# juno181/Ex4DGS

Measured on AMD Instinct MI355X. Metric: fwd+bwd ms/frame @1M Gaussians 1352x1014; achieved HBM GB/s vs peak, lower is better.
Workload: dtype f32; 1 GPU; cfg3: 1.0M static+dynamic (K=35), 1352x1014; P=1000000, HW=1370928, sh_degree=3, step=GaussianRasterizer forward + backward on a resident frame, parallelism=frame-sharded x1

## Files before the change

### ex4dgs_amd/_C.py

```python
import ctypes as C

import torch

from . import _abi
from ._abi import ALLOC_FN, BinningLayout, Ex4dParams, Ex4dSplitSH, GeomLayout, ImgLayout, library_path, load

NUM_CHANNELS = 3
EXPORTS = _abi.exports("ex4d_rasterizer.h")


class PendingFrame:
    __slots__ = ("capacity", "assumed_no_flow", "_status", "_event", "_pool")

    def __init__(self, capacity, assumed_no_flow, status, event, pool):
        self.capacity, self.assumed_no_flow, self._status, self._event, self._pool = int(capacity), bool(assumed_no_flow), status, event, pool

    def done(self):
        return self._event is not None and self._event.query()

    def wait(self):
        if self._event is not None:
            self._event.synchronize()
        else:
            torch.cuda.synchronize()
# ... 40 lines not shown
        except Exception:
            pass


_status_pool = []
_status_parked = []


def _recycle_parked():
    if _status_parked:
        still = []
        for ev, st in _status_parked:
            if ev.query():
                _status_pool.append(st)
            else:
                still.append((ev, st))
        _status_parked[:] = still


def _pinned_status():
    _recycle_parked()
    if not _status_pool:
        if torch.cuda.is_current_stream_capturing():
            raise RuntimeError("no pinned status buffer left during graph capture: run one asynchronous forward before capturing")
        block = torch.zeros(16, 8, dtype=torch.int32).pin_memory()
        _status_pool.extend(block[i] for i in range(16))
    return _status_pool.pop()


class SplitSH(tuple):
    def __new__(cls, dc_static, rest_static, dc_dynamic, rest_dynamic):
        return super().__new__(cls, (dc_static, rest_static, dc_dynamic, rest_dynamic))

    @property
    def n_static(self):
        return self[0].shape[0]

    @property
    def n_dynamic(self):
        return self[2].shape[0]

    def numel(self):
        return sum(t.numel() for t in self)

    def size(self, dim):
        return (self.n_static + self.n_dynamic, 16, 3)[dim]


def _split_struct(split, device, what):
    keep, ptrs = [], []
    for t, shape1 in zip(split, (1, 15, 1, 15)):
        if t.dim() != 3 or t.shape[1] != shape1 or t.shape[2] != 3:
            raise RuntimeError(f"{what}: expected [n,{shape1},3] tensors (dc/rest, static then dynamic)")
        kt, pt = _dev_f32(t, what, device)
        keep.append(kt); ptrs.append(pt)
    if split[0].shape[0] != split[1].shape[0] or split[2].shape[0] != split[3].shape[0]:
        raise RuntimeError(f"{what}: dc and rest must have the same number of rows")
    st = Ex4dSplitSH((C.c_void_p * 2)(ptrs[0], ptrs[2]), (C.c_void_p * 2)(ptrs[1], ptrs[3]), int(split[0].shape[0]))
    return keep, st


def _dev_f32(t, name, device):
    if t is None or t.numel() == 0:
        return None, None
    if t.device != device:
        raise RuntimeError(f"{name} must be on {device}, got {t.device}")
    if t.dtype != torch.float32:
        raise RuntimeError(f"{name} must be float32, got {t.dtype}")
    t = t.contiguous()
    return t, t.data_ptr()


def _rows(t, name, rows, cols=None):
    if t is None or t.numel() == 0:
        return
    if t.size(0) != rows or (cols is not None and t.numel() != rows * cols):
        raise RuntimeError(f"{name} has shape {tuple(t.shape)}, expected {rows} rows" + (f" of {cols} values" if cols else ""))


def _numel(t, name, n):
    if t is not None and t.numel() not in (0, n):
        raise RuntimeError(f"{name} has {t.numel()} elements, expected {n}")


def _require_rocm(t, name):
    if not t.is_cuda:
        raise RuntimeError(f"{name} is on {t.device}: the ex4dgs_amd rasterizer only runs on a ROCm GPU (no CPU fallback)")


def _params(P, D, M, W, H, tanfovx, tanfovy, kernel_size, scale_modifier, min_depth, max_depth, prefiltered, debug, prepare_backward=False,
            instance_capacity=0, assume_no_flow=False):
    return Ex4dParams(P, D, M, W, H, tanfovx, tanfovy, kernel_size, scale_modifier, min_depth, max_depth, int(bool(prefiltered)), int(bool(debug)),
                      int(bool(prepare_backward)), int(instance_capacity), int(bool(assume_no_flow)), 0)


def _resizer(t):
    def fn(_user, nbytes):
        t.resize_(int(nbytes))
        return t.data_ptr()
    return ALLOC_FN(fn)


def rasterize_gaussians(background, means3D, dir3D, colors, opacity, scales, rotations, scale_modifier, cov3D_precomp,
                        viewmatrix, projmatrix, tan_fovx, tan_fovy, kernel_size, subpixel_offset, image_height, image_width,
                        sh, degree, campos, prefiltered, min_depth, max_depth, debug, prepare_backward=False,
                        instance_capacity=0, assume_no_flow=False):
    load()
    if means3D.ndimension() != 2 or means3D.size(1) != 3:
        raise RuntimeError("means3D must have dimensions (num_points, 3)")
    _require_rocm(means3D, "means3D")
    dev = means3D.device
    P, H, W = means3D.size(0), int(image_height), int(image_width)
    f32 = dict(dtype=torch.float32, device=dev)
    i32 = dict(dtype=torch.int32, device=dev)
    geomBuffer = torch.empty(0, dtype=torch.uint8, device=dev)
    binningBuffer = torch.empty(0, dtype=torch.uint8, device=dev)
    imgBuffer = torch.empty(0, dtype=torch.uint8, device=dev)
    if P == 0:
        return (0, torch.zeros(NUM_CHANNELS, H, W, **f32), torch.zeros(P, **i32), geomBuffer, binningBuffer, imgBuffer,
                torch.zeros(1, H, W, **f32), torch.zeros(1, H, W, **f32), torch.zeros(3, H, W, **f32), torch.full((1, H, W), -1, **i32))
    out_color = torch.empty(NUM_CHANNELS, H, W, **f32)
    radii = torch.empty(P, **i32)
    out_depth = torch.empty(1, H, W, **f32)
    out_acc = torch.empty(1, H, W, **f32)
    out_flow = torch.empty(3, H, W, **f32)
    out_idx = torch.empty(1, H, W, **i32)

    split = sh if isinstance(sh, SplitSH) else None
    if split is not None:
        if split.n_static + split.n_dynamic != P:
            raise RuntimeError("SplitSH rows do not add up to the number of Gaussians")
        sh = torch.empty(0, **f32)
    M = 16 if split is not None else (sh.size(1) if sh.numel() != 0 else 0)
    for name, t, cols in (("dir3D", dir3D, 3), ("colors", colors, NUM_CHANNELS), ("opacity", opacity, 1), ("scales", scales, 3),
                          ("rotations", rotations, 4), ("cov3D_precomp", cov3D_precomp, 6), ("sh", sh, 3 * M)):
        _rows(t, name, P, cols)
    _numel(subpixel_offset, "subpixel_offset", 2 * H * W)
    _numel(background, "background", NUM_CHANNELS)
    for name, t in (("viewmatrix", viewmatrix), ("projmatrix", projmatrix)):
        _numel(t, name, 16)
    _numel(campos, "campos", 3)
    keep = []
    ptr = {}
    for name, t in (("background", background), ("means3D", means3D), ("dir3D", dir3D), ("sh", sh), ("colors", colors),
                    ("opacity", opacity), ("scales", scales), ("rotations", rotations), ("cov3D_precomp", cov3D_precomp),
                    ("viewmatrix", viewmatrix), ("projmatrix", projmatrix), ("campos", campos), ("subpixel_offset", subpixel_offset)):
        kt, ptr[name] = _dev_f32(t, name, dev)
        keep.append(kt)
    prm = _params(P, int(degree), M, W, H, tan_fovx, tan_fovy, kernel_size, scale_modifier, min_depth, max_depth, prefiltered, debug, prepare_backward,
                  instance_capacity, assume_no_flow)
    cbs = [_resizer(geomBuffer), _resizer(binningBuffer), _resizer(imgBuffer)]
    num_rendered = C.c_int32(0)
    count_ref = C.byref(num_rendered)
    status = None
    if instance_capacity > 0:
        status = torch.zeros(8, dtype=torch.int32, device=dev) if torch.cuda.is_current_stream_capturing() else _pinned_status()
        count_ref = C.cast(status.data_ptr(), C.POINTER(C.c_int32))
    entry, sh_args = "ex4d_forward", (ptr["sh"], ptr["colors"])
    if split is not None:
        if colors.numel() != 0:
            raise RuntimeError("Please provide excatly one of either SHs or precomputed colors!")
        kp, st = _split_struct(split, dev, "sh")
        keep.append(kp)
        entry, sh_args = "ex4d_forward_split_sh", (C.byref(st),)
    with _abi.stream(dev) as stream:
        _abi.call(entry, C.byref(prm), ptr["background"], ptr["means3D"], ptr["dir3D"], *sh_args, ptr["opacity"],
                  ptr["scales"], ptr["rotations"], ptr["cov3D_precomp"], ptr["viewmatrix"], ptr["projmatrix"], ptr["campos"],
                  ptr["subpixel_offset"], cbs[0], None, cbs[1], None, cbs[2], None,
                  out_color.data_ptr(), radii.data_ptr(), out_depth.data_ptr(), out_acc.data_ptr(), out_flow.data_ptr(), out_idx.data_ptr(),
                  stream, count_ref)
        ev = None
        if status is not None and not torch.cuda.is_current_stream_capturing():
            ev = torch.cuda.Event()
            ev.record(torch.cuda.current_stream())
    if status is not None:
        return (PendingFrame(instance_capacity, assume_no_flow, status, ev, _status_pool), out_color, radii, geomBuffer, binningBuffer, imgBuffer,
                out_depth, out_acc, out_flow, out_idx)
    return (int(num_rendered.value), out_color, radii, geomBuffer, binningBuffer, imgBuffer, out_depth, out_acc, out_flow, out_idx)


def rasterize_gaussians_backward(background, means3D, radii, colors, scales, rotations, acc_depth, acc, min_depth, max_depth,
                                 scale_modifier, cov3D_precomp, viewmatrix, projmatrix, tan_fovx, tan_fovy, kernel_size,
                                 subpixel_offset, dL_dout_color, dL_dout_depth, dL_grad_out_flow, dL_grad_out_acc, sh, degree,
                                 campos, geomBuffer, R, binningBuffer, imageBuffer, debug, need_colors=True, need_cov3D=True, prepared=False):
    lib = load()
    _require_rocm(means3D, "means3D")
    dev = means3D.device
    P = means3D.size(0)
    if isinstance(R, PendingFrame):
        R = R.capacity
    H, W = acc_depth.size(1), acc_depth.size(2)
    f32 = dict(dtype=torch.float32, device=dev)
    split = sh if isinstance(sh, SplitSH) else None
    if split is not None:
        sh = torch.empty(0, **f32)
    M = 16 if split is not None else (sh.size(1) if sh.numel() != 0 else 0)
    shapes = [(P, 3), (P, NUM_CHANNELS), (P, 1), (P, 3), (P, 6), (P, M, 3) if split is None else (0,), (P, 3), (P, 4), (P, 3)]
    for name, t, cols in (("radii", radii, 1), ("colors", colors, NUM_CHANNELS), ("scales", scales, 3), ("rotations", rotations, 4),
                          ("cov3D_precomp", cov3D_precomp, 6), ("sh", sh, 3 * M)):
        _rows(t, name, P, cols)
    if split is not None and split.n_static + split.n_dynamic != P:
        raise RuntimeError("SplitSH rows do not add up to the number of Gaussians")
    _numel(subpixel_offset, "subpixel_offset", 2 * H * W)
    for name, t, n in (("acc", acc, H * W), ("dL_dout_color", dL_dout_color, NUM_CHANNELS * H * W), ("dL_dout_depth", dL_dout_depth, H * W),
                       ("dL_grad_out_flow", dL_grad_out_flow, 3 * H * W), ("dL_grad_out_acc", dL_grad_out_acc, H * W),
                       ("viewmatrix", viewmatrix, 16), ("projmatrix", projmatrix, 16), ("campos", campos, 3)):
        _numel(t, name, n)
    if P == 0:
        outs0 = [torch.zeros(*s, **f32) for s in shapes]
        if split is not None:
            outs0[5] = SplitSH(*[torch.zeros_like(t) for t in split])
        return tuple(outs0)
    outs = [torch.empty(*s, **f32) for s in shapes]
    if not need_colors:
        outs[1] = torch.empty(0, **f32)
    if not need_cov3D:
        outs[4] = torch.empty(0, **f32)
    if split is not None:
        outs[5] = SplitSH(*[torch.empty_like(t, memory_format=torch.contiguous_format) for t in split])
    keep = []
    ptr = {}
    for name, t in (("background", background), ("means3D", means3D), ("sh", sh), ("colors", colors), ("scales", scales),
                    ("rotations", rotations), ("cov3D_precomp", cov3D_precomp), ("viewmatrix", viewmatrix), ("projmatrix", projmatrix),
                    ("campos", campos), ("subpixel_offset", subpixel_offset), ("acc_depth", acc_depth), ("acc", acc),
                    ("dL_dout_color", dL_dout_color), ("dL_dout_depth", dL_dout_depth), ("dL_grad_out_flow", dL_grad_out_flow),
                    ("dL_grad_out_acc", dL_grad_out_acc)):
        kt, ptr[name] = _dev_f32(t, name, dev)
        keep.append(kt)
    radii_c = radii.contiguous()
    scratch = torch.empty(lib.ex4d_backward_scratch_bytes(P), dtype=torch.uint8, device=dev)
    prm = _params(P, int(degree), M, W, H, tan_fovx, tan_fovy, kernel_size, scale_modifier, min_depth, max_depth, False, debug, prepared)
    if split is None:
        entry, sh_args, g_sh = "ex4d_backward", (ptr["sh"], ptr["colors"]), (outs[5].data_ptr() if M > 0 else None)
    else:
        kp, st = _split_struct(split, dev, "sh")
        kg, gst = _split_struct(outs[5], dev, "dL_dsh")
        keep += [kp, kg]
        entry, sh_args, g_sh = "ex4d_backward_split_sh", (C.byref(st),), C.byref(gst)
    with _abi.stream(dev) as stream:
        _abi.call(entry, C.byref(prm), int(R), ptr["background"], ptr["means3D"], radii_c.data_ptr(), *sh_args,
                  ptr["scales"], ptr["rotations"], ptr["cov3D_precomp"], ptr["viewmatrix"], ptr["projmatrix"], ptr["campos"],
                  ptr["subpixel_offset"], ptr["acc_depth"], ptr["acc"],
                  geomBuffer.data_ptr(), binningBuffer.data_ptr(), imageBuffer.data_ptr(),
                  ptr["dL_dout_color"], ptr["dL_dout_depth"], ptr["dL_grad_out_flow"], ptr["dL_grad_out_acc"],
                  outs[0].data_ptr(), _abi.ptr(outs[1]), outs[2].data_ptr(), outs[3].data_ptr(), _abi.ptr(outs[4]),
                  g_sh, outs[6].data_ptr(), outs[7].data_ptr(), outs[8].data_ptr(), scratch.data_ptr(), stream)
    rasterize_gaussians_backward.last_scratch = scratch
    return tuple(outs)


def mark_visible(means3D, viewmatrix, projmatrix, min_depth, max_depth=3.4028234663852886e38):
    load()
    _require_rocm(means3D, "means3D")
    dev = means3D.device
    P = means3D.size(0)
    present = torch.zeros(P, dtype=torch.bool, device=dev)
    if P == 0:
        return present
    if means3D.ndimension() != 2 or means3D.size(1) != 3:
        raise RuntimeError("means3D must have dimensions (num_points, 3)")
    (m, _), (v, _), (p, _) = _dev_f32(means3D, "means3D", dev), _dev_f32(viewmatrix, "viewmatrix", dev), _dev_f32(projmatrix, "projmatrix", dev)
    if v is None or p is None or v.numel() != 16 or p.numel() != 16:
        raise RuntimeError("viewmatrix and projmatrix must be 4x4 float32 tensors")
    with _abi.stream(dev) as stream:
        _abi.call("ex4d_mark_visible", P, m.data_ptr(), v.data_ptr(), p.data_ptr(), min_depth, max_depth, present.data_ptr(), stream)
    return present


def geom_views(geomBuffer, P):
    lay = GeomLayout()
    load().ex4d_geom_layout(P, C.byref(lay))
    g = geomBuffer
    v = lambda off, n, dt: g[off: off + n * torch.empty(0, dtype=dt).element_size()].view(dt)
    rec = v(lay.records, 16 * P, torch.float32).view(P, 16)
    return dict(records=rec, depths=rec[:, 8], means2D=rec[:, 0:2], conic_opacity=rec[:, [2, 3, 4, 15]], rgb=rec[:, 9:12], dir3D=rec[:, 12:15],
                cov3D=v(lay.cov3D, 6 * P, torch.float32).view(P, 6), clamped=v(lay.clamped, P, torch.uint8),
                tiles_touched=v(lay.tiles_touched, P, torch.int32), depth_order=v(lay.depth_order, P, torch.int32),
                rects=v(lay.rects, 2 * P, torch.int32).view(P, 2))


def binning_views(binningBuffer, R, W, H):
    if isinstance(R, PendingFrame):
        R = R.capacity
    lay = BinningLayout()
    load().ex4d_binning_layout(R, W, H, C.byref(lay))
    b = binningBuffer
    T = ((W + 15) // 16) * ((H + 15) // 16)
    return dict(point_list=b[lay.point_list: lay.point_list + 4 * R].view(torch.int32),
                tile_ids=b[lay.tile_ids: lay.tile_ids + 4 * R].view(torch.int32),
                qlist=b[lay.qlist: lay.qlist + 16 * max(R, 1)].view(torch.int32),
                qcount=b[lay.qcount: lay.qcount + 16 * T].view(torch.int32).view(T, 4))


def img_views(imgBuffer, W, H):
    lay = ImgLayout()
    load().ex4d_img_layout(W, H, C.byref(lay))
    T = ((W + 15) // 16) * ((H + 15) // 16)
    i = imgBuffer
    return dict(final_T=i[lay.final_T: lay.final_T + 4 * W * H].view(torch.float32).view(H, W),
                n_contrib=i[lay.n_contrib: lay.n_contrib + 4 * W * H].view(torch.int32).view(H, W),
                ranges=i[lay.ranges: lay.ranges + 8 * T].view(torch.int32).view(T, 2))


def set_option(name, value):
    _abi.call("ex4d_set_option", name.encode(), int(value))


def get_option(name):
    return int(load().ex4d_get_option(name.encode()))


SAMPLE_SORT_STATS = ("empty", "skipped", "packed", "pairs", "memory", "memory_gaussians", "largest", "distinct_splitters")


def sample_sort_stats(reset=True):
    buf = (C.c_ulonglong * 8)()
    _abi.call("ex4d_debug_sample_sort", buf, int(bool(reset)))
    return dict(zip(SAMPLE_SORT_STATS, (int(x) for x in buf)))


def bwd_stats(reset=True, extended=False):
    n = 16 if extended else 8
    buf = (C.c_ulonglong * n)()
    _abi.call("ex4d_debug_bwd_stats16" if extended else "ex4d_debug_bwd_stats", buf, int(bool(reset)))
    return [int(x) for x in buf]


def profile_enable(on=True):
    load().ex4d_profile_enable(int(bool(on)))


def profile_read(which):
    ms = (C.c_float * 16)()
    names = (C.c_char_p * 16)()
    n = load().ex4d_profile_read(int(which), ms, names, 16)
    return [(names[i].decode(), float(ms[i])) for i in range(n)]
```

### ex4dgs_amd/_abi.py

```python
import contextlib
import ctypes as C
import os

import torch

_CSRC = os.path.join(os.path.dirname(os.path.abspath(__file__)), "csrc")
_LIB_PATH = os.environ.get("EX4D_HIP_LIB") or os.path.join(_CSRC, "libex4d_hip.so")
_lib = None

RADAM_MAX_WINDOWS = 8
TRAINER_PARAMS = 15


def _all(ctype, *names):
    return [(n, ctype) for n in names]


i32, i64, f32, f64, vp, cint, size, text = C.c_int32, C.c_int64, C.c_float, C.c_double, C.c_void_p, C.c_int, C.c_size_t, C.c_char_p
P = C.POINTER


class Ex4dParams(C.Structure):
    _fields_ = [*_all(i32, "P", "D", "M", "W", "H"),
                *_all(f32, "tanfovx", "tanfovy", "kernel_size", "scale_modifier", "min_depth", "max_depth"),
                *_all(i32, "prefiltered", "debug", "prepare_backward", "instance_capacity", "assume_no_flow", "reserved")]


ALLOC_FN = C.CFUNCTYPE(vp, vp, size)


class Ex4dSplitSH(C.Structure):
    _fields_ = [("dc", vp * 2), ("rest", vp * 2), ("n_static", i32)]


Ex4dSplitSHGrad = Ex4dSplitSH


class Ex4dGeomLayout(C.Structure):
    _fields_ = _all(size, "records", "cov3D", "clamped", "tiles_touched", "depth_order", "sorted_offsets", "rects", "total")


class Ex4dBinningLayout(C.Structure):
    _fields_ = _all(size, "point_list", "tile_ids", "qlist", "qcount", "total")


class Ex4dImgLayout(C.Structure):
    _fields_ = _all(size, "final_T", "n_contrib", "ranges", "total")


GeomLayout, BinningLayout, ImgLayout = Ex4dGeomLayout, Ex4dBinningLayout, Ex4dImgLayout


class Ex4dAttrParams(C.Structure):
    _fields_ = [*_all(i32, "Ns", "Nd", "K", "k"), *_all(f32, "t", "duration", "delta", "h00", "h10", "h01", "h11", "tau", "var_min")]


class Ex4dRadamTensor(C.Structure):
    _fields_ = [*_all(vp, "param", "grad", "exp_avg", "exp_avg_sq"), ("numel", i64), ("lr", f64), ("step", i64),
                ("nan_to_num", i32), ("reserved", i32)]


class Ex4dRadamSlicedTensor(C.Structure):
    _fields_ = [*_all(vp, "param", "exp_avg", "exp_avg_sq"), ("rows", i64), ("K", i32), ("C", i32), ("lr", f64), ("step", i64),
                ("n_windows", i32), ("first", i32 * RADAM_MAX_WINDOWS), ("count", i32 * RADAM_MAX_WINDOWS),
                ("grad", vp * RADAM_MAX_WINDOWS), ("first_dev", vp)]


class Ex4dRadamSlicedRegTensor(C.Structure):
    _fields_ = [("t", Ex4dRadamSlicedTensor), ("reg_kind", i32), ("reserved", i32), ("reg_weight", f64), ("reg_rows", i64)]


class Ex4dDensifyPlanGroup(C.Structure):
    _fields_ = [("n", i64), *_all(vp, "stats", "scaling", "opacity", "xyz"), ("xyz_width", i32), ("use_screen", i32),
                *_all(f32, "grad_thr", "dense_scale", "big_scale", "screen_size", "min_opacity", "l1_thres", "max_ssim"),
                ("reserved", i32), *_all(vp, "map", "counts", "scratch")]


class Ex4dDensifyTensor(C.Structure):
    _fields_ = [("src", vp), ("dst", vp), ("rows", i64), ("dst_rows", i64), *_all(i32, "width", "planes", "rule", "group"),
                ("aux0", vp), ("aux1", vp), ("value", f32), ("reserved", i32)]


class Ex4dDensifyApplyGroup(C.Structure):
    _fields_ = [("map", vp), ("child_stride", i64), ("n_split", i64), *_all(vp, "split_z", "split_c1", "split_c0", "clone_c1", "clone_c0"),
                *_all(f32, "min_len", "center_lo", "center_hi", "split_div")]


class Ex4dGrowthClassify(C.Structure):
    _fields_ = [("n", i64), *_all(vp, "score", "result", "disp", "stats"), ("motion_abs", f32), ("min_abs", f32),
                *_all(vp, "map", "counts", "selected", "counts_out", "scratch")]


class Ex4dGrowthTensor(C.Structure):
    _fields_ = [*_all(vp, "old", "dst", "src0", "src1"), ("old_rows", i64), ("width", i32), ("rule", i32)]


class Ex4dGrowthAppend(C.Structure):
    _fields_ = [("selected", vp), ("n_new", i64), ("n_static", i64), ("stats", vp), ("K", i32),
                *_all(f32, "interval", "max_dur", "b_scale", "time_shift", "time_pad", "center_lo", "center_hi")]


class Ex4dTrainerConfig(C.Structure):
    _fields_ = [*_all(i32, "Ns", "Nd", "K", "W", "H", "sh_degree"), *_all(f32, "tanfovx", "tanfovy", "kernel_size", "min_depth", "max_depth"),
                *_all(f64, "duration", "interval", "time_shift", "var_pad"), ("lambda_dssim", f32), ("window", f32 * 11),
                ("lr", f64 * TRAINER_PARAMS), *_all(f64, "beta1", "beta2", "eps"), ("optimizer", i32)]


class Ex4dTrainerStepOptions(C.Structure):
    _fields_ = [*_all(i32, "l1_accum", "skip_optimizer", "stats_flags", "nan_census"), *_all(vp, "stats_s", "stats_d")]


class Ex4dTrainerReport(C.Structure):
    _fields_ = [("loss", f32), *_all(i32, "nan_static", "nan_dynamic", "reserved")]


def _status(name, *argtypes):
    return name, cint, argtypes, True


def _value(name, restype, *argtypes):
    return name, restype, argtypes, False


_fwd_tail = (ALLOC_FN, vp) * 3 + (vp,) * 6 + (vp, P(i32))
PROTOTYPES = {
    "ex4d_rasterizer.h": ("ex4d_last_error", (
        _value("ex4d_last_error", text),
        _value("ex4d_abi_version", cint),
        _value("ex4d_target_arch", text),
        _status("ex4d_forward", P(Ex4dParams), *[vp] * 13, *_fwd_tail),
        _status("ex4d_backward", P(Ex4dParams), i32, *[vp] * 32),
        _value("ex4d_backward_scratch_bytes", size, i32),
        _status("ex4d_forward_split_sh", P(Ex4dParams), *[vp] * 3, P(Ex4dSplitSH), *[vp] * 8, *_fwd_tail),
        _status("ex4d_backward_split_sh", P(Ex4dParams), i32, *[vp] * 3, P(Ex4dSplitSH), *[vp] * 21, P(Ex4dSplitSHGrad), *[vp] * 5),
        _status("ex4d_mark_visible", i32, vp, vp, vp, f32, f32, vp, vp),
        _value("ex4d_geom_bytes", size, i32),
        _value("ex4d_binning_bytes", size, i32, i32, i32),
        _value("ex4d_img_bytes", size, i32, i32),
        _value("ex4d_geom_layout", None, i32, P(Ex4dGeomLayout)),
        _value("ex4d_binning_layout", None, i32, i32, i32, P(Ex4dBinningLayout)),
        _value("ex4d_img_layout", None, i32, i32, P(Ex4dImgLayout)),
        _status("ex4d_set_option", text, cint),
        _value("ex4d_get_option", cint, text),
        _status("ex4d_debug_bwd_stats", P(C.c_ulonglong), cint),
        _status("ex4d_debug_bwd_stats16", P(C.c_ulonglong), cint),
        _status("ex4d_debug_rows_prof", P(C.c_ulonglong), cint),
        _status("ex4d_debug_sample_sort", P(C.c_ulonglong), cint),
        _value("ex4d_profile_enable", None, cint),
        _value("ex4d_profile_read", cint, cint, P(f32), P(text), cint))),
    "ex4d_attributes.h": ("ex4d_attributes_last_error", (
        _value("ex4d_attributes_last_error", text),
        _status("ex4d_attributes_forward", P(Ex4dAttrParams), *[vp] * 21),
        _status("ex4d_attributes_backward", P(Ex4dAttrParams), *[vp] * 28),
        _status("ex4d_attributes_backward_sliced", P(Ex4dAttrParams), *[vp] * 27, P(i32), vp),
        _status("ex4d_attr_time_scalars", i32, f64, f64, f64, f64, i32, i32, i32, f64, P(Ex4dAttrParams)),
        _status("ex4d_attributes_forward_ex", P(Ex4dAttrParams), i32, *[vp] * 21),
        _status("ex4d_attributes_backward_ex", P(Ex4dAttrParams), i32, *[vp] * 29),
        _status("ex4d_attributes_backward_sliced_ex", P(Ex4dAttrParams), i32, *[vp] * 28, P(i32), vp))),
    "ex4d_loss.h": ("ex4d_loss_last_error", (
        _value("ex4d_loss_last_error", text),
        _value("ex4d_l1_ssim_scratch_floats", size, i32, i32),
        _status("ex4d_l1_ssim_forward", i32, i32, i32, vp, vp, f32, *[vp] * 7),
        _status("ex4d_l1_ssim_backward", i32, i32, i32, vp, vp, f32, *[vp] * 5),
        _status("ex4d_l1_ssim_forward_u8", i32, i32, vp, vp, i32, vp, f32, *[vp] * 7),
        _status("ex4d_l1_ssim_backward_u8", i32, i32, vp, vp, i32, vp, f32, *[vp] * 5),
        _value("ex4d_frame_metrics_scratch_floats", size, i32, i32),
        _status("ex4d_frame_metrics", i32, i32, vp, vp, vp, i32, *[vp] * 4),
        _status("ex4d_frame_metrics_u8", i32, i32, vp, vp, i32, vp, vp, i32, *[vp] * 4),
        _value("ex4d_resize_u8_table_words", size, i32, i32, i32),
        _status("ex4d_resize_u8_table", i32, i32, i32, vp),
        _value("ex4d_resize_u8_scratch_bytes", size, i32, i32, i32, i32),
        _status("ex4d_resize_u8", i32, i32, i32, i32, i32, *[vp] * 6),
        _value("ex4d_frame_skssim_scratch_floats", size, i32, i32),
        _status("ex4d_frame_skssim", i32, i32, vp, vp, i32, *[vp] * 3),
        _status("ex4d_frame_skssim_u8", i32, i32, vp, vp, i32, vp, i32, *[vp] * 3))),
    "ex4d_optim.h": ("ex4d_optim_last_error", (
        _value("ex4d_optim_last_error", text),
        _status("ex4d_radam_step", P(Ex4dRadamTensor), i32, f64, f64, f64, vp),
        _status("ex4d_radam_step_sliced", P(Ex4dRadamSlicedTensor), i32, f64, f64, f64, vp),
        _status("ex4d_radam_step_sliced_reg", P(Ex4dRadamSlicedRegTensor), i32, f64, f64, f64, vp),
        _value("ex4d_radam_sliced_reg_rows", i32, i32, i32))),
    "ex4d_knn.h": ("ex4d_knn_last_error", (
        _value("ex4d_knn_last_error", text),
        _value("ex4d_dist2_scratch_bytes", size, i32),
        _status("ex4d_dist2", i32, vp, vp, vp, vp))),
    "ex4d_densify.h": ("ex4d_densify_last_error", (
        _status("ex4d_densify_stats", vp, i64, vp, i64, vp, vp, vp, f32, i32, vp),
        _status("ex4d_densify_stats_merge", vp, vp, i32, i64, vp, vp),
        _status("ex4d_nan_any", vp, i64, vp, i64, vp, vp),
        _value("ex4d_densify_scratch_bytes", size, i64),
        _status("ex4d_densify_plan", i32, P(Ex4dDensifyPlanGroup), vp),
        _status("ex4d_densify_apply", P(Ex4dDensifyTensor), i32, P(Ex4dDensifyApplyGroup), vp),
        _value("ex4d_densify_last_error", text),
        _status("ex4d_growth_scores", vp, vp, vp, vp, i64, vp, vp),
        _value("ex4d_growth_select_scratch_bytes", size),
        _status("ex4d_growth_select", vp, i64, f32, vp, vp, vp),
        _status("ex4d_growth_classify", P(Ex4dGrowthClassify), vp),
        _status("ex4d_growth_append", P(Ex4dGrowthTensor), i32, P(Ex4dGrowthAppend), vp),
        _status("ex4d_growth_extrapolate", vp, vp, i64, i32, i32, i32, i32, vp),
        _status("ex4d_growth_expand_opacity", vp, vp, vp, vp, i64, f32, f32, f32, vp),
        _status("ex4d_growth_adjust_opacity", vp, vp, vp, vp, i64, f32, f32, vp))),
    "ex4d_regularizers.h": ("ex4d_reg_last_error", (
        _value("ex4d_reg_last_error", text),
        _value("ex4d_reg_scratch_bytes", size),
        _status("ex4d_reg_forward", vp, i64, vp, vp, i64, i32, f64, f64, f64, vp, vp, vp),
        _status("ex4d_reg_backward", vp, vp, i64, vp, vp, vp, vp, i64, i32, f64, f64, f64, vp, i32, vp),
        _status("ex4d_reg_backward_range", i32, vp, i64, i32, i64, i64, vp, f64, i32, vp))),
    "ex4d_trainer.h": ("ex4d_trainer_last_error", (
        _value("ex4d_trainer_last_error", text),
        _value("ex4d_trainer_create", vp, P(Ex4dTrainerConfig), P(vp)),
        _value("ex4d_trainer_destroy", None, vp),
        _value("ex4d_trainer_time_scalars", None, P(Ex4dTrainerConfig), f64, P(Ex4dAttrParams)),
        _status("ex4d_trainer_step", vp, f64, *[vp] * 6, P(i32)),
        _status("ex4d_trainer_step_ex", vp, f64, *[vp] * 6, P(i32), P(Ex4dTrainerStepOptions)),
        _status("ex4d_trainer_step_u8", vp, f64, *[vp] * 5, i32, vp, vp, P(i32), P(Ex4dTrainerStepOptions)),
        _status("ex4d_trainer_report", vp, P(Ex4dTrainerReport)),
        _status("ex4d_trainer_set_lr", vp, P(f64)),
        _status("ex4d_trainer_set_sh_degree", vp, i32),
        _status("ex4d_trainer_set_async", vp, i32),
        _value("ex4d_trainer_replays", i64, vp),
        _status("ex4d_trainer_set_interp", vp, i32),
        _status("ex4d_trainer_set_regularizers", vp, f64, f64, f64),
        _value("ex4d_trainer_output", vp, vp, i32),
        _value("ex4d_trainer_grad", vp, vp, i32, P(i32)),
        _status("ex4d_trainer_read", vp, i32, vp, size, vp),
        _status("ex4d_trainer_write", vp, i32, vp, size, vp),
        _status("ex4d_trainer_get_step", vp, P(i64)),
        _status("ex4d_trainer_set_step", vp, i64),
        _value("ex4d_trainer_bytes", size, vp))),
}
_LAST_ERROR = {name: err for err, protos in PROTOTYPES.values() for name, _, _, is_status in protos if is_status}


def exports(header):
    return tuple(name for name, _, _, _ in PROTOTYPES[header][1])


def library_path():
    return _LIB_PATH


def load():
    global _lib
    if _lib is not None:
        return _lib
    if not os.path.exists(_LIB_PATH):
        raise RuntimeError(f"{_LIB_PATH} not found: build it with `python -m ex4dgs_amd.build` "
                           "(there is no CPU / PyTorch fallback for the rasterizer)")
    lib = C.CDLL(_LIB_PATH)
    for _, protos in PROTOTYPES.values():
        for name, restype, argtypes, _ in protos:
            fn = getattr(lib, name)
            fn.restype, fn.argtypes = restype, list(argtypes)
    _lib = lib
    return lib


def call(name, *args):
    err = _LAST_ERROR[name]
    lib = load()
    rc = getattr(lib, name)(*args)
    if rc != 0:
        raise RuntimeError(getattr(lib, err)().decode() or f"{name} failed with status {rc}")


def ptr(t):
    return None if t is None or t.numel() == 0 else t.data_ptr()


@contextlib.contextmanager
def stream(device):
    with torch.cuda.device(device):
        yield C.c_void_p(torch.cuda.current_stream().cuda_stream)
```

### ex4dgs_amd/csrc/ex4d_api.hip

```cpp
#include "ex4d_internal.h"
#include <atomic>
#include <cstdarg>
#include <cstdio>
#include <cstdlib>
#include <cstring>
#include <mutex>

namespace {

std::atomic<bool> g_prof_on{false};
std::atomic<int> g_bwd_variant{4};
std::atomic<int> g_tile_ids{0};
std::atomic<int> g_tile_rows{1};
std::atomic<int> g_depth_msd{3};
struct DepthSortWatch {
    std::mutex mu;
    uint32_t *word = nullptr;
    bool tried = false;
    std::atomic<int> hold{0}, backoff{64}, trips{0};
    uint32_t *get()
    {
        std::lock_guard<std::mutex> lock(mu);
        if (!tried) {
            tried = true;
            if (hipHostMalloc((void **)&word, 64, hipHostMallocPortable) != hipSuccess) { (void)hipGetLastError(); word = nullptr; }
            else memset(word, 0, 64);
        }
        return word;
    }
    void reset()
    {
        std::lock_guard<std::mutex> lock(mu);
        hold.store(0); backoff.store(64); trips.store(0);
        if (word) __atomic_store_n(word, 0u, __ATOMIC_RELAXED);
    }
} g_depth_watch;
bool depth_sort_auto_msd(hipStream_t stream, bool async, uint32_t **watch)
{
    *watch = nullptr;
    if (async) {
        hipStreamCaptureStatus st = hipStreamCaptureStatusNone;
        if (hipStreamIsCapturing(stream, &st) != hipSuccess) { (void)hipGetLastError(); return false; }
        if (st != hipStreamCaptureStatusNone) return false;
    }
    uint32_t *w = g_depth_watch.get();
    if (!w) return false;
    if (__atomic_load_n(w, __ATOMIC_RELAXED) != 0u && __atomic_exchange_n(w, 0u, __ATOMIC_RELAXED) != 0u) {
        const int b = g_depth_watch.backoff.load();
        g_depth_watch.hold.store(b);
        g_depth_watch.backoff.store(b < (1 << 20) ? 2 * b : b);
        g_depth_watch.trips.fetch_add(1);
    }
    for (int h = g_depth_watch.hold.load(); h > 0; )
        if (g_depth_watch.hold.compare_exchange_weak(h, h - 1)) return false;
    *watch = w;
    return true;
}
std::atomic<int> g_depth_msd_bits{0};
std::atomic<int> g_readback_side{1};
std::atomic<int> g_depth_local_cap{0};
std::atomic<int> g_depth_local_threads{0};
std::atomic<int> g_depth_sample{0};
std::atomic<int> g_depth_sample_frames{0};
std::atomic<int> g_depth_sample_stats{0};
std::atomic<int> g_geom_debug{0};
thread_local char g_err[512] = "";

int fail(int code, const char *fmt, ...)
{
    va_list ap;
    va_start(ap, fmt);
    vsnprintf(g_err, sizeof(g_err), fmt, ap);
    va_end(ap);
    return code;
}

#define HIP_TRY(expr)                                                                              \
    do {                                                                                           \
        hipError_t e_ = (expr);                                                                    \
        if (e_ != hipSuccess) return fail(EX4D_ERR_HIP, "%s failed: %s", #expr, hipGetErrorString(e_)); \
    } while (0)

#define STAGE(expr, prm, stream)                                                                   \
    do {                                                                                           \
        HIP_TRY(expr);                                                                             \
        if ((prm)->debug) HIP_TRY(hipStreamSynchronize(stream));                                   \
    } while (0)
#define MARK(which, name) g_prof.mark(which, name, stream)

struct StageProfiler {
    static const int kMax = 16;
    hipEvent_t ev[2][kMax + 1];
    const char *names[2][kMax];
    int n[2] = { 0, 0 };
    bool created = false;
    int device = -1;
    std::mutex mu;
    void begin(int which, hipStream_t s)
    {
        if (!g_prof_on.load(std::memory_order_relaxed)) return;
        std::lock_guard<std::mutex> lock(mu);
        int dev = -1;
        (void)hipGetDevice(&dev);
        if (created && dev != device) {
            for (int w = 0; w < 2; w++) for (int i = 0; i <= kMax; i++) (void)hipEventDestroy(ev[w][i]);
            created = false; n[0] = n[1] = 0;
        }
        if (!created) { for (int w = 0; w < 2; w++) for (int i = 0; i <= kMax; i++) (void)hipEventCreate(&ev[w][i]); created = true; device = dev; }
        n[which] = 0;
        (void)hipEventRecord(ev[which][0], s);
    }
    void mark(int which, const char *name, hipStream_t s)
    {
        if (!g_prof_on.load(std::memory_order_relaxed)) return;
        std::lock_guard<std::mutex> lock(mu);
        if (!created || n[which] >= kMax) return;
        names[which][n[which]] = name;
        n[which]++;
        (void)hipEventRecord(ev[which][n[which]], s);
    }
};
StageProfiler g_prof;

struct Readback {
    uint32_t *host = nullptr;
    size_t words = 0;
    hipEvent_t ev;
    hipEvent_t ev_pre;
    hipStream_t side = nullptr;
    bool have_ev = false;
    int device = -1;
    bool init(size_t need_words)
    {
        int dev = -1;
        if (hipGetDevice(&dev) != hipSuccess) return false;
        if (have_ev && dev != device) { (void)hipEventDestroy(ev); (void)hipEventDestroy(ev_pre); (void)hipStreamDestroy(side); side = nullptr; have_ev = false; }
        if (!have_ev) {
            if (hipEventCreateWithFlags(&ev, hipEventDisableTiming) != hipSuccess) return false;
            if (hipEventCreateWithFlags(&ev_pre, hipEventDisableTiming) != hipSuccess) { (void)hipEventDestroy(ev); return false; }
            if (hipStreamCreateWithFlags(&side, hipStreamNonBlocking) != hipSuccess) { (void)hipEventDestroy(ev); (void)hipEventDestroy(ev_pre); side = nullptr; return false; }
            have_ev = true; device = dev;
        }
        if (need_words > words) {
            if (host) (void)hipHostFree(host);
            host = nullptr; words = 0;
            if (hipHostMalloc((void **)&host, need_words * sizeof(uint32_t), hipHostMallocDefault) != hipSuccess) return false;
            words = need_words;
        }
        return true;
    }
};
thread_local Readback g_readback;

struct Carver {
    char *base; size_t off;
    explicit Carver(void *b) : base((char *)b), off(0) {}
    template <typename T> T *take(size_t count)
    {
        T *p = base ? (T *)(base + off) : nullptr;
        off = ex4d_align_up(off + count * sizeof(T));
        return p;
    }
};

GeomState carve_geom(void *buf, int P, Ex4dGeomLayout *lay, size_t *total)
{
    Carver c(buf);
    GeomState g;
    Ex4dGeomLayout l;
    l.records = c.off;        g.records = c.take<float4>(4 * (size_t)P);
    l.cov3D = c.off;          g.cov3D = c.take<float>(6 * (size_t)P);
    l.clamped = c.off;        g.clamped = c.take<uint8_t>(P);
    l.tiles_touched = c.off;  g.tiles_touched = c.take<uint32_t>(P);
    l.rects = c.off;          g.rects = c.take<uint2>(P);
    g.sorted_rects = c.take<uint2>(P);
    g.rects4 = c.take<uint32_t>(P);
    l.depth_order = c.off;    g.depth_order = c.take<uint32_t>(P);
    l.sorted_offsets = c.off; g.sorted_offsets = c.take<uint32_t>(P);
    g.sort_keys_a = c.take<uint32_t>(P);
    g.sort_keys_b = c.take<uint32_t>(P);
    g.sort_vals_b = c.take<uint32_t>(P);
    g.sort_vals_a = c.take<uint32_t>(P);
    g.rects4_b = c.take<uint32_t>(P);
    g.bucket_starts = c.take<uint32_t>((size_t)1 << EX4D_DLS_MSD_BITS);
    g.key_ranges = c.take<uint2>(((size_t)P + 63) / 64);
    g.bucket_sums = c.take<uint32_t>((size_t)1 << EX4D_DLS_MSD_BITS);
    g.scan_block_sums = c.take<uint32_t>((P + SCAN_CHUNK - 1) / SCAN_CHUNK + 1);
    g.sort_hist = c.take<uint32_t>(ex4d_radix_hist_words((uint32_t)P));
    g.total = c.take<uint32_t>(EX4D_FLAG_WORDS);
    g.block_totals = c.take<uint32_t>(2 * (((size_t)P + 63) / 64));
    g.row_hist = c.take<uint32_t>(ex4d_tile_sort_rows_geom_words((uint32_t)P));
    g.sh_dsums = c.take<float>(9 * (size_t)P);
    l.total = c.off;
    if (lay) *lay = l;
    if (total) *total = c.off;
    return g;
}

int tile_bits(int T)
{
    int b = 1;
    while ((1 << b) < T) b++;
    return b;
}

BinState carve_binning(void *buf, uint32_t R, int W, int H, Ex4dBinningLayout *lay, size_t *total)
{
    const int T = ((W + EX4D_TILE - 1) / EX4D_TILE) * ((H + EX4D_TILE - 1) / EX4D_TILE);
    Carver c(buf);
    BinState b;
    Ex4dBinningLayout l;
    const size_t n = R ? R : 1;
    l.point_list = c.off; b.point_list = c.take<uint32_t>(n);
    l.tile_ids = c.off;   b.tile_ids = c.take<uint32_t>(n);
    const int tb = tile_bits(T);
    const int cgx = (W + EX4D_TILE - 1) / EX4D_TILE, cgy = (H + EX4D_TILE - 1) / EX4D_TILE;
    const size_t hw = ex4d_radix_hist_words(R), hw2 = ex4d_tile_sort_hist_words(R, tb);
    const size_t hw3 = (cgx <= 255 && cgy <= 255) ? ex4d_tile_sort_rows_hist_words(R) : 0;
    const size_t hwm = hw > hw2 ? hw : hw2;
    b.sort_hist = c.take<uint32_t>(hwm > hw3 ? hwm : hw3);
    l.qlist = c.off;  b.qlist = c.take<uint32_t>(4 * n);
    b.vals_tmp = b.qlist;
    b.keys_tmp = b.qlist ? b.vals_tmp + ex4d_align_up(n * sizeof(uint32_t)) / sizeof(uint32_t) : nullptr;
    l.qcount = c.off; b.qcount = c.take<uint32_t>(4 * (size_t)T);
    l.total = c.off;
    if (lay) *lay = l;
    if (total) *total = c.off;
    return b;
}

ImgState carve_img(void *buf, int W, int H, Ex4dImgLayout *lay, size_t *total)
{
    Carver c(buf);
    ImgState s;
    Ex4dImgLayout l;
    const size_t HW = (size_t)W * H;
    const int T = ((W + EX4D_TILE - 1) / EX4D_TILE) * ((H + EX4D_TILE - 1) / EX4D_TILE);
    l.final_T = c.off;   s.final_T = c.take<float>(HW);
    l.n_contrib = c.off; s.n_contrib = c.take<uint32_t>(HW);
    l.ranges = c.off;    s.ranges = c.take<uint2>(T);
    l.total = c.off;
    if (lay) *lay = l;
    if (total) *total = c.off;
    return s;
}

}

extern "C" {

const char *ex4d_last_error(void) { return g_err; }
int ex4d_abi_version(void) { return 5; }
const char *ex4d_target_arch(void) { return "gfx950"; }

size_t ex4d_geom_bytes(int32_t P) { size_t t; carve_geom(nullptr, P, nullptr, &t); return t; }
size_t ex4d_binning_bytes(int32_t R, int32_t W, int32_t H) { size_t t; carve_binning(nullptr, (uint32_t)R, W, H, nullptr, &t); return t; }
size_t ex4d_img_bytes(int32_t W, int32_t H) { size_t t; carve_img(nullptr, W, H, nullptr, &t); return t; }
void ex4d_geom_layout(int32_t P, Ex4dGeomLayout *out) { carve_geom(nullptr, P, out, nullptr); }
void ex4d_binning_layout(int32_t R, int32_t W, int32_t H, Ex4dBinningLayout *out) { carve_binning(nullptr, (uint32_t)R, W, H, out, nullptr); }
void ex4d_img_layout(int32_t W, int32_t H, Ex4dImgLayout *out) { carve_img(nullptr, W, H, out, nullptr); }
size_t ex4d_backward_scratch_bytes(int32_t P) { return ex4d_align_up((size_t)P * 16 * sizeof(float)); }

static int forward_impl(
    const Ex4dParams *prm, ShSplit split,
    const float *background, const float *means3D, const float *dir3D, const float *shs, const float *colors_precomp,
    const float *opacities, const float *scales, const float *rotations, const float *cov3D_precomp,
    const float *viewmatrix, const float *projmatrix, const float *campos, const float *subpixel_offset,
    ex4d_alloc_fn geom_alloc, void *geom_user, ex4d_alloc_fn binning_alloc, void *binning_user,
    ex4d_alloc_fn img_alloc, void *img_user,
    float *out_color, int32_t *radii, float *out_depth, float *out_acc, float *out_flow, int32_t *out_idx,
    void *stream_, int32_t *num_rendered)
{
    g_err[0] = 0;
    hipStream_t stream = (hipStream_t)stream_;
    if (!prm || !num_rendered) return fail(EX4D_ERR_ARG, "null params");
    const int P = prm->P, W = prm->W, H = prm->H;
    if (P <= 0 || W <= 0 || H <= 0) return fail(EX4D_ERR_ARG, "P, W, H must be positive (P == 0 is handled by the caller)");
    if (!means3D || !opacities || !background || !viewmatrix || !projmatrix || !campos)
        return fail(EX4D_ERR_ARG, "means3D, opacities, background, viewmatrix, projmatrix, campos are required");
    const bool is_split = split.rest[0] != nullptr || split.rest[1] != nullptr;
    if (((shs != nullptr || is_split) ? 1 : 0) + (colors_precomp != nullptr ? 1 : 0) != 1 || (shs != nullptr && is_split))
        return fail(EX4D_ERR_ARG, "Please provide excatly one of either SHs or precomputed colors!");
    if (is_split && prm->M != 16) return fail(EX4D_ERR_ARG, "split SH needs M == 16 (dc [n,1,3] + rest [n,15,3])");
    if (((scales == nullptr || rotations == nullptr) && cov3D_precomp == nullptr) ||
        ((scales != nullptr || rotations != nullptr) && cov3D_precomp != nullptr))
        return fail(EX4D_ERR_ARG, "Please provide exactly one of either scale/rotation pair or precomputed 3D covariance!");
    if (shs && prm->M < (prm->D + 1) * (prm->D + 1)) return fail(EX4D_ERR_ARG, "sh has fewer coefficients than the active degree needs");
    if (!out_color || !radii || !out_depth || !out_acc || !out_flow || !out_idx) return fail(EX4D_ERR_ARG, "null output");
    const int gx = (W + EX4D_TILE - 1) / EX4D_TILE, gy = (H + EX4D_TILE - 1) / EX4D_TILE;
    const int T = gx * gy;
    const bool async = prm->instance_capacity > 0;
    if (prm->instance_capacity < 0) return fail(EX4D_ERR_ARG, "instance_capacity must be >= 0");
    if (async && prm->debug) return fail(EX4D_ERR_ARG, "debug (synchronise after every stage) and instance_capacity > 0 (asynchronous forward) exclude each other");

    void *geom_buf = geom_alloc(geom_user, ex4d_geom_bytes(P));
    if (!geom_buf) return fail(EX4D_ERR_ALLOC, "geometry buffer allocation failed");
    GeomState g = carve_geom(geom_buf, P, nullptr, nullptr);
    void *img_buf = img_alloc(img_user, ex4d_img_bytes(W, H));
    if (!img_buf) return fail(EX4D_ERR_ALLOC, "image buffer allocation failed");
    ImgState im = carve_img(img_buf, W, H, nullptr, nullptr);

    uint32_t key_base = 0, key_invisible = 0xFFFFFFFFu;
    int key_bits = 32;
    if (prm->min_depth >= 0.0f && prm->max_depth > prm->min_depth && prm->max_depth < 3.0e38f) {
        uint32_t lo, hi;
        memcpy(&lo, &prm->min_depth, 4); memcpy(&hi, &prm->max_depth, 4);
        key_base = lo;
        key_invisible = hi - lo + 1u;
        key_bits = 1;
        while (key_bits < 32 && (key_invisible >> key_bits) != 0u) key_bits++;
    }
    const bool packed_rects = gx <= 255 && gy <= 255;
    int msd_mode = g_depth_msd.load(std::memory_order_relaxed);
    uint32_t *msd_watch = nullptr;
    const bool sample_depth = g_depth_sample.load(std::memory_order_relaxed) != 0 && packed_rects && ex4d_depth_sort_msd_applies((uint32_t)P, key_bits);
    if (!(packed_rects && ex4d_depth_sort_msd_applies((uint32_t)P, key_bits))) msd_mode = 0;
    else if (sample_depth) msd_mode = 1;
    else if (msd_mode == 3) msd_mode = depth_sort_auto_msd(stream, async, &msd_watch) ? 2 : 0;
    const bool msd_depth = msd_mode != 0;
    int msd_bits = ex4d_depth_sort_msd_bits((uint32_t)P, key_bits);
    {
        const int forced = g_depth_msd_bits.load(std::memory_order_relaxed);
        if (forced == EX4D_DLS_MSD_BITS || (forced == EX4D_DLS_MSD_BITS - 1 && ex4d_depth_sort_msd_bits(1u, key_bits) == forced)) msd_bits = forced;
    }
    const bool start_in_b = (ex4d_radix_passes((uint32_t)P, key_bits) & 1) != 0;
    uint32_t *keys0 = start_in_b ? g.sort_keys_b : g.sort_keys_a, *vals0 = start_in_b ? g.sort_vals_b : g.depth_order;
    uint32_t *keys1 = start_in_b ? g.sort_keys_a : g.sort_keys_b, *vals1 = start_in_b ? g.depth_order : g.sort_vals_b;
    if (msd_depth) { keys0 = g.sort_keys_a; vals0 = g.sort_vals_a; }

    HIP_TRY(ex4d_prepare_rank_lds(stream));
    g_prof.begin(0, stream);
    if (async) HIP_TRY(ex4d_launch_zero(g.total, 8 * sizeof(uint32_t), stream));
    GeomState gw = g;
    if (!g_geom_debug.load(std::memory_order_relaxed)) {
        gw.cov3D = nullptr; gw.tiles_touched = nullptr;
        if (packed_rects) gw.rects = nullptr;
    }
    STAGE(ex4d_launch_preprocess_fwd(*prm, means3D, dir3D, scales, rotations, opacities, shs, cov3D_precomp, colors_precomp,
                                     viewmatrix, projmatrix, campos, radii, gw, g.total + 1, split,
                                     keys0, (uint32_t *)nullptr, key_base, key_invisible, packed_rects ? g.rects4 : nullptr, stream,
                                     (msd_depth && !sample_depth) ? reinterpret_cast<uint32_t *>(g.key_ranges) : nullptr, async), prm, stream);
    MARK(0, "preprocess_fwd");
    const size_t nblk = (size_t)(P + 63) / 64;
    const size_t rb_words = (size_t)(g.block_totals - g.total) + 2 * nblk;
    if (!async) {
        if (!g_readback.init(rb_words)) return fail(EX4D_ERR_HIP, "pinned read-back buffer allocation failed");
        if (g_readback_side.load(std::memory_order_relaxed)) {
            HIP_TRY(hipEventRecord(g_readback.ev_pre, stream));
            HIP_TRY(hipStreamWaitEvent(g_readback.side, g_readback.ev_pre, 0));
            HIP_TRY(hipMemcpyAsync(g_readback.host, g.total, rb_words * sizeof(uint32_t), hipMemcpyDeviceToHost, g_readback.side));
            HIP_TRY(hipEventRecord(g_readback.ev, g_readback.side));
        } else {
            HIP_TRY(hipMemcpyAsync(g_readback.host, g.total, rb_words * sizeof(uint32_t), hipMemcpyDeviceToHost, stream));
            HIP_TRY(hipEventRecord(g_readback.ev, stream));
        }
    }
    const bool rows_sort = g_tile_rows.load(std::memory_order_relaxed) != 0 && ex4d_tile_sort_rows_applies(P, gx, gy);
    const bool fused_scan = msd_mode == 2 && !rows_sort;
    const bool lsd_gather = !msd_depth && rows_sort && packed_rects;
    if (msd_depth) {
        if (sample_depth) {
            g_depth_sample_frames.fetch_add(1);
            STAGE(ex4d_depth_sort_sample(g.sort_keys_a, g.sort_vals_a, g.rects4, g.sort_keys_b, g.depth_order, g.rects4_b, (uint32_t)P, key_invisible, key_bits,
                                         g.sort_hist, g.bucket_starts, g.bucket_sums, (uint32_t)g_depth_local_cap.load(std::memory_order_relaxed), stream,
                                         T, rows_sort ? im.ranges : nullptr, g_depth_local_threads.load(std::memory_order_relaxed),
                                         g_depth_sample_stats.load(std::memory_order_relaxed) != 0), prm, stream);
        } else {
            STAGE(ex4d_depth_sort_msd(g.sort_keys_a, g.sort_vals_a, g.rects4, g.sort_keys_b, g.depth_order, g.rects4_b, (uint32_t)P, key_invisible,
                                      g.total, g.key_ranges, g.sort_hist, g.bucket_starts, (uint32_t)g_depth_local_cap.load(std::memory_order_relaxed), stream,
                                      fused_scan ? g.sorted_offsets : nullptr, fused_scan ? g.bucket_sums : nullptr, T, (fused_scan || rows_sort) ? im.ranges : nullptr,
                                      g_depth_local_threads.load(std::memory_order_relaxed), msd_watch, msd_bits), prm, stream);
        }
        MARK(0, "depth_sort");
        if (!fused_scan && !rows_sort) {
            STAGE(ex4d_launch_scan_tiles(P, nullptr, g.rects4_b, nullptr, nullptr, g.sorted_offsets, g.scan_block_sums, T, im.ranges, async ? g.total : nullptr, stream), prm, stream);
            MARK(0, "scan_tiles");
        }
    } else {
        bool in_first = true;
        STAGE(ex4d_radix_sort_pairs(keys0, vals0, keys1, vals1, (uint32_t)P, key_bits, g.sort_hist, &in_first, stream, nullptr, true,
                                    lsd_gather ? g.rects4 : nullptr, lsd_gather ? g.rects4_b : nullptr, lsd_gather ? im.ranges : nullptr, T), prm, stream);
        if (in_first == start_in_b) return fail(EX4D_ERR_HIP, "internal: depth sort ended in the wrong buffer");
        MARK(0, "depth_sort");
        if (!lsd_gather) {
            STAGE(ex4d_launch_scan_tiles(P, g.rects, packed_rects ? g.rects4 : nullptr, g.depth_order, g.sorted_rects, g.sorted_offsets, g.scan_block_sums, T, im.ranges, async ? g.total : nullptr, stream), prm, stream);
            MARK(0, "scan_tiles");
        }
    }
    const uint2 *dup_rects = (msd_depth || lsd_gather) ? nullptr : g.sorted_rects;
    const uint32_t *dup_rects4 = (msd_depth || lsd_gather) ? g.rects4_b : nullptr;
    uint32_t R = 0;
    uint32_t segment_sum = 0;
    const uint32_t *n_dev = nullptr;
    bool has_flow;
    if (async) {
        static_assert(sizeof(Ex4dFrameStatus) == 8 * sizeof(uint32_t), "Ex4dFrameStatus mirrors the first eight frame-flag words");
        const bool count_later = fused_scan || (rows_sort && msd_depth) || lsd_gather;
        if (!count_later) HIP_TRY(hipMemcpyAsync(num_rendered, g.total, sizeof(Ex4dFrameStatus), hipMemcpyDefault, stream));
        R = (uint32_t)prm->instance_capacity;
        segment_sum = 0;
        n_dev = g.total;
        has_flow = prm->assume_no_flow == 0;
    } else {
        {
            static const bool spin = []{ const char *e = getenv("EX4D_READBACK_SPIN"); return e ? atoi(e) != 0 : true; }();
            if (spin) {
                hipError_t q = hipErrorNotReady;
                for (int i = 0; i < 20000 && (q = hipEventQuery(g_readback.ev)) == hipErrorNotReady; i++) { }
                if (q == hipErrorNotReady) q = hipEventSynchronize(g_readback.ev);
                HIP_TRY(q);
            } else HIP_TRY(hipEventSynchronize(g_readback.ev));
        }
        uint32_t instance_sum = 0;
        uint32_t chunk_flags = 0;
        for (size_t i = 0; i < nblk; i++) {
            const uint32_t seg = g_readback.host[(size_t)(g.block_totals - g.total) + 2 * i + 1];
            instance_sum += g_readback.host[(size_t)(g.block_totals - g.total) + 2 * i];
            segment_sum += seg & 0x3FFFFFFFu;
            chunk_flags |= seg;
        }
        has_flow = (chunk_flags & EX4D_CHUNK_FLOW) != 0u;
        if (prm->prefiltered && (chunk_flags & EX4D_CHUNK_FILTERED))
            return fail(EX4D_ERR_PREFILTERED, "Point is filtered although prefiltered is set. This shouldn't happen!");
        R = instance_sum;
        if (R > 0x7FFFFFFFu) return fail(EX4D_ERR_ARG, "more than 2^31-1 tile instances");
        *num_rendered = (int32_t)R;
    }

    void *bin_buf = binning_alloc(binning_user, ex4d_binning_bytes((int32_t)R, W, H));
    if (!bin_buf) return fail(EX4D_ERR_ALLOC, "binning buffer allocation failed");
    BinState b = carve_binning(bin_buf, R, W, H, nullptr, nullptr);

    const int passes = ex4d_radix_passes(R, tile_bits(T));
    uint32_t *k0 = (passes % 2 == 0) ? b.tile_ids : b.keys_tmp;
    uint32_t *v0 = (passes % 2 == 0) ? b.point_list : b.vals_tmp;
    uint32_t *k1 = (passes % 2 == 0) ? b.keys_tmp : b.tile_ids;
    uint32_t *v1 = (passes % 2 == 0) ? b.vals_tmp : b.point_list;
    if (rows_sort) {
        if (R > 0) {
            STAGE(ex4d_tile_sort_rows(P, gx, gy, g.depth_order, dup_rects4, dup_rects, b.keys_tmp, b.point_list,
                                      g_tile_ids.load(std::memory_order_relaxed) ? b.tile_ids : nullptr, R, segment_sum, g.row_hist, b.sort_hist, im.ranges,
                                      (async && (msd_depth || lsd_gather)) ? g.total : nullptr, stream), prm, stream);
        }
        if (async && (msd_depth || lsd_gather)) HIP_TRY(hipMemcpyAsync(num_rendered, g.total, sizeof(Ex4dFrameStatus), hipMemcpyDefault, stream));
        MARK(0, "tile_sort");
    } else if (R > 0 && ex4d_tile_sort_msd_applies(P, tile_bits(T))) {
        STAGE(ex4d_launch_duplicate(P, W, H, g.depth_order, g.sorted_offsets, g.scan_block_sums, dup_rects, dup_rects4, b.tile_ids, b.vals_tmp, R, stream,
                                    fused_scan ? g.sort_keys_b : nullptr, g.total + EX4D_FLAG_DPARAMS, g.bucket_sums, g.total, msd_bits), prm, stream);
        if (async && fused_scan) HIP_TRY(hipMemcpyAsync(num_rendered, g.total, sizeof(Ex4dFrameStatus), hipMemcpyDefault, stream));
        MARK(0, "duplicate");
        STAGE(ex4d_tile_sort_msd(b.tile_ids, b.vals_tmp, b.keys_tmp, b.point_list, g_tile_ids.load(std::memory_order_relaxed) ? b.tile_ids : nullptr,
                                 R, tile_bits(T), b.sort_hist, im.ranges, stream, n_dev), prm, stream);
        MARK(0, "tile_sort");
        MARK(0, "tile_ranges");
    } else {
        if (R > 0) {
            STAGE(ex4d_launch_duplicate(P, W, H, g.depth_order, g.sorted_offsets, g.scan_block_sums, dup_rects, dup_rects4, k0, v0, R, stream,
                                        fused_scan ? g.sort_keys_b : nullptr, g.total + EX4D_FLAG_DPARAMS, g.bucket_sums, g.total, msd_bits), prm, stream);
            if (async && fused_scan) HIP_TRY(hipMemcpyAsync(num_rendered, g.total, sizeof(Ex4dFrameStatus), hipMemcpyDefault, stream));
            MARK(0, "duplicate");
            bool res_a = true;
            STAGE(ex4d_radix_sort_pairs(k0, v0, k1, v1, R, tile_bits(T), b.sort_hist, &res_a, stream, n_dev), prm, stream);
        }
        MARK(0, "tile_sort");
        STAGE(ex4d_launch_tile_ranges(R, T, b.tile_ids, im.ranges, stream, n_dev), prm, stream);
        MARK(0, "tile_ranges");
    }
    STAGE(ex4d_launch_composite_fwd(*prm, im.ranges, b.point_list, subpixel_offset, g.records, background, im.final_T, im.n_contrib,
                                    out_color, out_depth, out_acc, out_flow, out_idx, b.qlist, b.qcount, has_flow, stream), prm, stream);
    MARK(0, "composite_fwd");
    return EX4D_OK;
}

static int backward_impl(
    const Ex4dParams *prm, ShSplit split, ShSplitGrad gsplit, int32_t num_rendered,
    const float *background, const float *means3D, const int32_t *radii,
    const float *shs, const float *colors_precomp, const float *scales, const float *rotations,
    const float *cov3D_precomp, const float *viewmatrix, const float *projmatrix, const float *campos,
    const float *subpixel_offset, const float *out_depth, const float *out_acc,
    const void *geom_buffer, const void *binning_buffer, const void *img_buffer,
    const float *dL_dout_color, const float *dL_dout_depth, const float *dL_dout_flow, const float *dL_dout_acc,
    float *dL_dmeans2D, float *dL_dcolors, float *dL_dopacity, float *dL_dmeans3D, float *dL_dcov3D, float *dL_dsh,
    float *dL_dscales, float *dL_drotations, float *dL_ddir, void *bwd_scratch, void *stream_)
{
    g_err[0] = 0;
    hipStream_t stream = (hipStream_t)stream_;
    if (!prm) return fail(EX4D_ERR_ARG, "null params");
    const int P = prm->P, W = prm->W, H = prm->H;
    if (P <= 0 || W <= 0 || H <= 0) return fail(EX4D_ERR_ARG, "P, W, H must be positive (P == 0 is handled by the caller)");
    if (!geom_buffer || !binning_buffer || !img_buffer || !bwd_scratch) return fail(EX4D_ERR_ARG, "null state buffer");
    if ((size_t)P * 64 > 0xFFFFFFFFull) return fail(EX4D_ERR_ARG, "more than 2^26 Gaussians: the accumulator rows are addressed with 32-bit byte offsets");
    if (!dL_dmeans2D || !dL_dopacity || !dL_dmeans3D || !dL_dscales || !dL_drotations || !dL_ddir || (prm->M > 0 && !dL_dsh && !(gsplit.rest[0] || gsplit.rest[1])))
        return fail(EX4D_ERR_ARG, "null gradient output");
    GeomState g = carve_geom((void *)geom_buffer, P, nullptr, nullptr);
    BinState b = carve_binning((void *)binning_buffer, (uint32_t)num_rendered, W, H, nullptr, nullptr);
    ImgState im = carve_img((void *)img_buffer, W, H, nullptr, nullptr);
    float *acc16 = (float *)bwd_scratch;

    const int variant = g_bwd_variant.load(std::memory_order_relaxed);
    g_prof.begin(1, stream);
    HIP_TRY(ex4d_launch_zero(acc16, (size_t)P * 16 * sizeof(float), stream));
    MARK(1, "zero_accumulators");
    if (num_rendered > 0)
        STAGE(ex4d_launch_composite_bwd(*prm, im.ranges, b.point_list, subpixel_offset, background, g.records,
                                        out_depth, out_acc, im.final_T, im.n_contrib,
                                        dL_dout_color, dL_dout_depth, dL_dout_flow, dL_dout_acc, acc16, b.qlist, b.qcount, variant, stream), prm, stream);
    MARK(1, "composite_bwd");
    const float *cov3D_ptr = cov3D_precomp;
    STAGE(ex4d_launch_preprocess_bwd(*prm, means3D, radii, shs, scales, rotations, cov3D_ptr, viewmatrix, projmatrix, campos, g, acc16,
                                     dL_dmeans2D, dL_dcolors, dL_dopacity, dL_dmeans3D, dL_dcov3D, dL_dsh, dL_dscales, dL_drotations, dL_ddir,
                                     split, gsplit, stream), prm, stream);
    MARK(1, "preprocess_bwd");
    return EX4D_OK;
}

static const ShSplit kNoSplit = { { nullptr, nullptr }, { nullptr, nullptr }, 0 };
static const ShSplitGrad kNoSplitGrad = { { nullptr, nullptr }, { nullptr, nullptr }, 0 };

int ex4d_forward(
    const Ex4dParams *prm,
    const float *background, const float *means3D, const float *dir3D, const float *shs, const float *colors_precomp,
    const float *opacities, const float *scales, const float *rotations, const float *cov3D_precomp,
    const float *viewmatrix, const float *projmatrix, const float *campos, const float *subpixel_offset,
    ex4d_alloc_fn geom_alloc, void *geom_user, ex4d_alloc_fn binning_alloc, void *binning_user,
    ex4d_alloc_fn img_alloc, void *img_user,
    float *out_color, int32_t *radii, float *out_depth, float *out_acc, float *out_flow, int32_t *out_idx,
    void *stream_, int32_t *num_rendered)
{
    return forward_impl(prm, kNoSplit, background, means3D, dir3D, shs, colors_precomp, opacities, scales, rotations, cov3D_precomp,
                        viewmatrix, projmatrix, campos, subpixel_offset, geom_alloc, geom_user, binning_alloc, binning_user,
                        img_alloc, img_user, out_color, radii, out_depth, out_acc, out_flow, out_idx, stream_, num_rendered);
}

static bool split_ok(const Ex4dParams *prm, const float *const dc[2], const float *const rest[2], int n_static)
{
    if (!prm || n_static < 0 || n_static > prm->P) return false;
    if (n_static > 0 && (!dc[0] || !rest[0])) return false;
    if (n_static < prm->P && (!dc[1] || !rest[1])) return false;
    return true;
}

int ex4d_forward_split_sh(
    const Ex4dParams *prm, const float *background, const float *means3D, const float *dir3D, const Ex4dSplitSH *shs,
    const float *opacities, const float *scales, const float *rotations, const float *cov3D_precomp,
    const float *viewmatrix, const float *projmatrix, const float *campos, const float *subpixel_offset,
    ex4d_alloc_fn geom_alloc, void *geom_user, ex4d_alloc_fn binning_alloc, void *binning_user,
    ex4d_alloc_fn img_alloc, void *img_user,
    float *out_color, int32_t *radii, float *out_depth, float *out_acc, float *out_flow, int32_t *out_idx,
    void *stream_, int32_t *num_rendered)
{
    g_err[0] = 0;
    if (!shs || !split_ok(prm, shs->dc, shs->rest, shs->n_static)) return fail(EX4D_ERR_ARG, "split SH: null tensor or n_static outside [0, P]");
    const ShSplit sp = { { shs->dc[0], shs->dc[1] }, { shs->rest[0], shs->rest[1] }, shs->n_static };
    return forward_impl(prm, sp, background, means3D, dir3D, nullptr, nullptr, opacities, scales, rotations, cov3D_precomp,
                        viewmatrix, projmatrix, campos, subpixel_offset, geom_alloc, geom_user, binning_alloc, binning_user,
                        img_alloc, img_user, out_color, radii, out_depth, out_acc, out_flow, out_idx, stream_, num_rendered);
}

int ex4d_backward(
    const Ex4dParams *prm, int32_t num_rendered,
    const float *background, const float *means3D, const int32_t *radii,
    const float *shs, const float *colors_precomp, const float *scales, const float *rotations,
    const float *cov3D_precomp, const float *viewmatrix, const float *projmatrix, const float *campos,
    const float *subpixel_offset, const float *out_depth, const float *out_acc,
    const void *geom_buffer, const void *binning_buffer, const void *img_buffer,
    const float *dL_dout_color, const float *dL_dout_depth, const float *dL_dout_flow, const float *dL_dout_acc,
    float *dL_dmeans2D, float *dL_dcolors, float *dL_dopacity, float *dL_dmeans3D, float *dL_dcov3D, float *dL_dsh,
    float *dL_dscales, float *dL_drotations, float *dL_ddir, void *bwd_scratch, void *stream_)
{
    return backward_impl(prm, kNoSplit, kNoSplitGrad, num_rendered, background, means3D, radii, shs, colors_precomp, scales, rotations,
                         cov3D_precomp, viewmatrix, projmatrix, campos, subpixel_offset, out_depth, out_acc, geom_buffer, binning_buffer,
                         img_buffer, dL_dout_color, dL_dout_depth, dL_dout_flow, dL_dout_acc, dL_dmeans2D, dL_dcolors, dL_dopacity,
                         dL_dmeans3D, dL_dcov3D, dL_dsh, dL_dscales, dL_drotations, dL_ddir, bwd_scratch, stream_);
}

int ex4d_backward_split_sh(
    const Ex4dParams *prm, int32_t num_rendered,
    const float *background, const float *means3D, const int32_t *radii,
    const Ex4dSplitSH *shs, const float *scales, const float *rotations,
    const float *cov3D_precomp, const float *viewmatrix, const float *projmatrix, const float *campos,
    const float *subpixel_offset, const float *out_depth, const float *out_acc,
    const void *geom_buffer, const void *binning_buffer, const void *img_buffer,
    const float *dL_dout_color, const float *dL_dout_depth, const float *dL_dout_flow, const float *dL_dout_acc,
    float *dL_dmeans2D, float *dL_dcolors, float *dL_dopacity, float *dL_dmeans3D, float *dL_dcov3D, const Ex4dSplitSHGrad *dL_dsh,
    float *dL_dscales, float *dL_drotations, float *dL_ddir, void *bwd_scratch, void *stream_)
{
    g_err[0] = 0;
    if (!shs || !dL_dsh || !split_ok(prm, shs->dc, shs->rest, shs->n_static) || dL_dsh->n_static != shs->n_static ||
        !split_ok(prm, (const float *const *)dL_dsh->dc, (const float *const *)dL_dsh->rest, dL_dsh->n_static))
        return fail(EX4D_ERR_ARG, "split SH: null tensor, n_static outside [0, P] or mismatching gradient split");
    if (prm->M != 16) return fail(EX4D_ERR_ARG, "split SH needs M == 16 (dc [n,1,3] + rest [n,15,3])");
    const ShSplit sp = { { shs->dc[0], shs->dc[1] }, { shs->rest[0], shs->rest[1] }, shs->n_static };
    const ShSplitGrad gsp = { { dL_dsh->dc[0], dL_dsh->dc[1] }, { dL_dsh->rest[0], dL_dsh->rest[1] }, dL_dsh->n_static };
    return backward_impl(prm, sp, gsp, num_rendered, background, means3D, radii, nullptr, nullptr, scales, rotations,
                         cov3D_precomp, viewmatrix, projmatrix, campos, subpixel_offset, out_depth, out_acc, geom_buffer, binning_buffer,
                         img_buffer, dL_dout_color, dL_dout_depth, dL_dout_flow, dL_dout_acc, dL_dmeans2D, dL_dcolors, dL_dopacity,
                         dL_dmeans3D, dL_dcov3D, nullptr, dL_dscales, dL_drotations, dL_ddir, bwd_scratch, stream_);
}

int ex4d_set_option(const char *name, int value)
{
    if (name && !strcmp(name, "composite_bwd_variant") && (value == 4 || value == 8)) { g_bwd_variant.store(value); return EX4D_OK; }
    if (name && !strcmp(name, "composite_fwd_asm") && (value == 0 || value == 1)) { ex4d_set_fwd_asm(value); return EX4D_OK; }
    if (name && !strcmp(name, "binning_tile_ids") && (value == 0 || value == 1)) { g_tile_ids.store(value); return EX4D_OK; }
    if (name && !strcmp(name, "composite_clamp_always") && (value == 0 || value == 1)) { ex4d_set_clamp_always(value); return EX4D_OK; }
    if (name && !strcmp(name, "composite_bwd_pairs") && (value == 0 || value == 1)) { ex4d_set_bwd_pairs(value); return EX4D_OK; }
    if (name && !strcmp(name, "tile_sort_rows") && (value == 0 || value == 1)) { g_tile_rows.store(value); return EX4D_OK; }
    if (name && !strcmp(name, "rank_lds_atomics") && value >= -1 && value <= 1) { ex4d_set_rank_lds(value); return EX4D_OK; }
    if (name && !strcmp(name, "rows_probe")) { ex4d_set_rows_probe(value); return EX4D_OK; }
    if (name && !strcmp(name, "preprocess_sh_predicate") && (value == 0 || value == 1)) { ex4d_set_preprocess_tune(value); return EX4D_OK; }
    if (name && !strcmp(name, "geom_debug_arrays") && (value == 0 || value == 1)) { g_geom_debug.store(value); return EX4D_OK; }
    if (name && !strcmp(name, "preprocess_fast_path") && (value == 0 || value == 1)) { ex4d_set_preprocess_fast(value); return EX4D_OK; }
    if (name && !strcmp(name, "depth_sort_msd") && value >= 0 && value <= 3) { g_depth_msd.store(value); g_depth_watch.reset(); return EX4D_OK; }
    if (name && !strcmp(name, "depth_sort_sample") && (value == 0 || value == 1)) { g_depth_sample.store(value); g_depth_sample_frames.store(0); return EX4D_OK; }
    if (name && !strcmp(name, "depth_sort_sample_stats") && (value == 0 || value == 1)) { g_depth_sample_stats.store(value); return EX4D_OK; }
    if (name && !strcmp(name, "depth_sort_local_cap") && value >= 0 && value <= 8192) { g_depth_local_cap.store(value); return EX4D_OK; }
    if (name && !strcmp(name, "readback_side_stream") && (value == 0 || value == 1)) { g_readback_side.store(value); return EX4D_OK; }
    if (name && !strcmp(name, "depth_sort_msd_bits") && (value == 0 || value == EX4D_DLS_MSD_BITS - 1 || value == EX4D_DLS_MSD_BITS)) { g_depth_msd_bits.store(value); return EX4D_OK; }
    if (name && !strcmp(name, "depth_sort_local_threads") && (value == 0 || value == 256 || value == 512)) { g_depth_local_threads.store(value); return EX4D_OK; }
    return fail(EX4D_ERR_ARG, "unknown option or value out of range");
}

int ex4d_debug_bwd_stats(unsigned long long *out8, int reset) { return ex4d_bwd_stats(out8, 8, reset) == hipSuccess ? EX4D_OK : EX4D_ERR_HIP; }
int ex4d_debug_rows_prof(unsigned long long *out8, int reset) { return ex4d_rows_prof(out8, reset) == hipSuccess ? EX4D_OK : EX4D_ERR_HIP; }
int ex4d_debug_sample_sort(unsigned long long *out8, int reset) { return ex4d_sample_sort_stats(out8, reset) == hipSuccess ? EX4D_OK : EX4D_ERR_HIP; }
int ex4d_debug_bwd_stats16(unsigned long long *out16, int reset) { return ex4d_bwd_stats(out16, 16, reset) == hipSuccess ? EX4D_OK : EX4D_ERR_HIP; }

int ex4d_get_option(const char *name)
{
    if (name && !strcmp(name, "composite_bwd_variant")) return g_bwd_variant.load();
    if (name && !strcmp(name, "composite_fwd_asm")) return ex4d_get_fwd_asm();
    if (name && !strcmp(name, "binning_tile_ids")) return g_tile_ids.load();
    if (name && !strcmp(name, "composite_clamp_always")) return ex4d_get_clamp_always();
    if (name && !strcmp(name, "composite_bwd_pairs")) return ex4d_get_bwd_pairs();
    if (name && !strcmp(name, "tile_sort_rows")) return g_tile_rows.load();
    if (name && !strcmp(name, "rank_lds_atomics")) return ex4d_get_rank_lds();
    if (name && !strcmp(name, "rank_lds_atomics_in_use")) return ex4d_rank_lds_in_use();
    if (name && !strcmp(name, "preprocess_sh_predicate")) return ex4d_get_preprocess_tune();
    if (name && !strcmp(name, "geom_debug_arrays")) return g_geom_debug.load();
    if (name && !strcmp(name, "preprocess_fast_path")) return ex4d_get_preprocess_fast();
    if (name && !strcmp(name, "depth_sort_msd")) return g_depth_msd.load();
    if (name && !strcmp(name, "depth_sort_hold")) return g_depth_watch.hold.load();
    if (name && !strcmp(name, "depth_sort_trips")) return g_depth_watch.trips.load();
    if (name && !strcmp(name, "depth_sort_sample")) return g_depth_sample.load();
    if (name && !strcmp(name, "depth_sort_sample_frames")) return g_depth_sample_frames.load();
    if (name && !strcmp(name, "depth_sort_sample_stats")) return g_depth_sample_stats.load();
    if (name && !strcmp(name, "depth_sort_local_cap")) return g_depth_local_cap.load();
    if (name && !strcmp(name, "readback_side_stream")) return g_readback_side.load();
    if (name && !strcmp(name, "depth_sort_msd_bits")) return g_depth_msd_bits.load();
    if (name && !strcmp(name, "depth_sort_local_threads")) return g_depth_local_threads.load();
    return -1;
}

void ex4d_profile_enable(int on) { g_prof_on.store(on != 0); }

int ex4d_profile_read(int which, float *ms, const char **names, int max_stages)
{
    std::lock_guard<std::mutex> lock(g_prof.mu);
    if (which < 0 || which > 1 || !g_prof.created) return 0;
    const int n = g_prof.n[which] < max_stages ? g_prof.n[which] : max_stages;
    if (n == 0) return 0;
    if (hipEventSynchronize(g_prof.ev[which][g_prof.n[which]]) != hipSuccess) return 0;
    for (int i = 0; i < n; i++) {
        float t = 0.f;
        (void)hipEventElapsedTime(&t, g_prof.ev[which][i], g_prof.ev[which][i + 1]);
        ms[i] = t;
        if (names) names[i] = g_prof.names[which][i];
    }
    return n;
}

int ex4d_mark_visible(int32_t P, const float *means3D, const float *viewmatrix, const float *projmatrix,
                      float min_depth, float max_depth, uint8_t *present, void *stream_)
{
    g_err[0] = 0;
    if (P <= 0) return EX4D_OK;
    if (!means3D || !viewmatrix || !projmatrix || !present) return fail(EX4D_ERR_ARG, "null argument");
    HIP_TRY(ex4d_launch_mark_visible(P, means3D, viewmatrix, projmatrix, min_depth, max_depth, present, (hipStream_t)stream_));
    return EX4D_OK;
}

}
```

### ex4dgs_amd/csrc/ex4d_binning.hip

```cpp
#include "ex4d_internal.h"
#include <atomic>
#include <mutex>

__device__ int ex4d_g_rank_lds = 0;

namespace {

__global__ __launch_bounds__(256) void lds_rank_probe_kernel(uint32_t seed, int trials, int ndigits, uint32_t *__restrict__ bad)
{
    __shared__ uint32_t cnt[4][256];
    const int lane = threadIdx.x & 63, wave = threadIdx.x >> 6;
    uint32_t x = seed ^ (blockIdx.x * 0x9E3779B9u) ^ (threadIdx.x * 0x85EBCA6Bu);
    uint32_t nb = 0;
    for (int t = 0; t < trials; t++) {
        for (int i = lane; i < 256; i += 64) cnt[wave][i] = 0;
        __builtin_amdgcn_fence(__ATOMIC_RELEASE, "wavefront"); __builtin_amdgcn_wave_barrier(); __builtin_amdgcn_fence(__ATOMIC_ACQUIRE, "wavefront");
        x = x * 1664525u + 1013904223u;
        const uint32_t d = (x >> 16) % (uint32_t)ndigits;
        uint32_t expect = 0, same = 0;
        for (int l = 0; l < 64; l++) { const uint32_t dl = __shfl(d, l, 64); if (dl == d) { same++; if (l < lane) expect++; } }
        const uint32_t got = atomicAdd(&cnt[wave][d], 1u);
        const uint32_t got2 = atomicAdd(&cnt[wave][d], 1u);
        if (got != expect || got2 != same + expect) nb++;
    }
// ... 295 lines not shown
    }
    __syncthreads();
    {
        constexpr int BPT = BINS / RS_THREADS;
        uint32_t c[BPT][4], tot[BPT], gtot[BPT], pf[BPT];
        uint32_t tsum = 0, gsum = 0;
#pragma unroll
        for (int k = 0; k < BPT; k++) {
            const int d = tid * BPT + k;
            const bool live = d < nbins;
#pragma unroll
            for (int w = 0; w < 4; w++) c[k][w] = live ? wave_cnt[w][d] : 0u;
            tot[k] = c[k][0] + c[k][1] + c[k][2] + c[k][3];
            static_assert(BPT == BPT_PRE, "the prefetched histogram words follow the digit ownership of this phase");
            if (MODE == 2) {
                pf[k] = pre_pf[k];
                gtot[k] = live ? pre_gt[k] - pf[k] : 0u;
            } else {
                pf[k] = 0u;
                gtot[k] = pre_gt[k];
            }
            tsum += tot[k]; gsum += gtot[k];
        }
        uint32_t x = tsum, gx = gsum;
#pragma unroll
        for (int o = 1; o < 64; o <<= 1) {
            const uint32_t y = __shfl_up(x, o, 64), gy = __shfl_up(gx, o, 64);
            if (lane >= o) { x += y; gx += gy; }
        }
        if (lane == 63) { scan_tmp[wave] = x; scan_tmp[4 + wave] = gx; }
        __syncthreads();
        uint32_t ls = x - tsum, gb = gx - gsum;
        for (int w = 0; w < wave; w++) { ls += scan_tmp[w]; gb += scan_tmp[4 + w]; }
        if (MODE == 2) gb += tb.bucket_start;
#pragma unroll
        for (int k = 0; k < BPT; k++) {
            const int d = tid * BPT + k;
            if (d < nbins) {
                local_start[d] = ls;
                global_base[d] = gb + pre_hb[k] - pf[k];
                if (MODE == 2 && blockIdx.x == tb.fb_first && gtot[k] != 0u) {
                    const uint32_t e = gb + gtot[k];
                    ranges[(size_t)bucket * (range_stride ? range_stride : (1u << nbits)) + d] = make_uint2(gb < out_cap ? gb : out_cap, e < out_cap ? e : out_cap);
                }
                if (MODE == 3 && blockIdx.x == 0) bucket_starts[d] = gb;
                wave_cnt[0][d] = ls; wave_cnt[1][d] = ls + c[k][0]; wave_cnt[2][d] = ls + c[k][0] + c[k][1]; wave_cnt[3][d] = ls + c[k][0] + c[k][1] + c[k][2];
            }
            ls += tot[k]; gb += gtot[k];
        }
    }
    __syncthreads();
#pragma unroll
    for (int it = 0; it < ITEMS; it++) {
        const uint32_t i = base + it * 64 + lane;
        if (i < block_end) {
            const uint32_t d = digit_of(key[it]);
            if constexpr (MODE == 2) stage_w[wave_cnt[wave][d] + pos[it]] = key[it];
            else stage[wave_cnt[wave][d] + pos[it]] = make_uint2(key[it], val[it]);
            if constexpr (MODE == 3) stage_r[wave_cnt[wave][d] + pos[it]] = rct[it];
        }
    }
    __syncthreads();
    const uint32_t count = (block_end - block_first) < CHUNK ? (block_end - block_first) : CHUNK;
#pragma unroll 4
    for (uint32_t p = tid; p < count; p += RS_THREADS) {
        uint2 kv;
        if constexpr (MODE == 2) kv = make_uint2(stage_w[p], 0u); else kv = stage[p];
        const uint32_t d = digit_of(kv.x);
        const uint32_t dst = global_base[d] + (p - local_start[d]);
        if (MODE == 0) { keys_out[dst] = kv.x; vals_out[dst] = kv.y; if (rects_in) rects_out[dst] = rects_in[kv.y]; }
        if constexpr (MODE == 3) { keys_out[dst] = kv.x; vals_out[dst] = kv.y; rects_out[dst] = stage_r[p]; }
        if (MODE == 1) keys_out[dst] = ((kv.x & ((1u << low_bits) - 1u)) << (32 - low_bits)) | kv.y;
        if (MODE == 2 && dst < out_cap) {
            vals_out[dst] = kv.x & (0xFFFFFFFFu >> nbits);
            if (keys_out) keys_out[dst] = bucket * (range_stride ? range_stride : (1u << nbits)) + d;
        }
    }
}

__global__ __launch_bounds__(RS_THREADS) void ts_histogram_kernel(const uint32_t *__restrict__ words, const uint32_t *__restrict__ bucket_totals,
    int nbuckets, int shift, uint32_t nblocks, uint32_t *__restrict__ hist, uint32_t cap = 0xFFFFFFFFu, const Ex4dTsBlock *__restrict__ block_table = nullptr)
{
    __shared__ uint32_t h[256];
    __shared__ TsLocateLds loc;
    h[threadIdx.x] = 0;
    TsBlock tb;
    if (block_table) { tb = ts_block_from_table(block_table, blockIdx.x); __syncthreads(); }
    else tb = ts_locate_block(bucket_totals, nbuckets, blockIdx.x, loc);
    if (tb.count != 0) {
        uint32_t k[RS_ITEMS];
#pragma unroll
        for (int it = 0; it < RS_ITEMS; it++) {
            const uint32_t i = it * RS_THREADS + threadIdx.x;
            const uint32_t gi = tb.start + (i < tb.count ? i : tb.count - 1);
            k[it] = words[gi < cap ? gi : cap - 1];
        }
#pragma unroll
        for (int it = 0; it < RS_ITEMS; it++) {
            const uint32_t i = it * RS_THREADS + threadIdx.x;
            if (i < tb.count && tb.start + i < cap) atomicAdd(&h[k[it] >> shift], 1u);
        }
    }
    __syncthreads();
    hist[(size_t)threadIdx.x * nblocks + blockIdx.x] = h[threadIdx.x];
}


#define DLS_ITEMS 16
#define DLS_MAX_CAP 8192
template <int THREADS> struct DlsLds {
    static constexpr int WAVES = THREADS / 64, CAP = THREADS * DLS_ITEMS, IDX_BITS = (THREADS == 512 ? 13 : 12);
    static_assert((1 << IDX_BITS) == CAP, "arrival index bits");
    uint32_t buf[CAP]; uint32_t cnt[WAVES][512]; uint32_t scan_tmp[WAVES];
};
#define DLS_IDX_BITS 13

__device__ __forceinline__ void dls_wave_sync()
{
    __builtin_amdgcn_fence(__ATOMIC_RELEASE, "wavefront");
    __builtin_amdgcn_wave_barrier();
    __builtin_amdgcn_fence(__ATOMIC_ACQUIRE, "wavefront");
}
template <int NBITS>
__device__ __forceinline__ uint64_t dls_peers(uint32_t d, int nbits, bool valid)
{
    const uint64_t vmask = __builtin_amdgcn_ballot_w64(valid);
    uint32_t plo = (uint32_t)vmask, phi = (uint32_t)(vmask >> 32);
    if (NBITS > 0) {
#pragma unroll
        for (int b = 0; b < NBITS; b++) {
            const uint64_t bal = __builtin_amdgcn_ballot_w64((d & (1u << b)) != 0u);
            uint32_t flip;
            asm("v_cndmask_b32_e64 %0, -1, 0, %1" : "=v"(flip) : "s"(bal));
            plo &= (uint32_t)bal ^ flip;
            phi &= (uint32_t)(bal >> 32) ^ flip;
        }
    } else {
        for (int b = 0; b < nbits; b++) {
            const uint32_t bit = (d >> b) & 1u;
            const uint64_t bal = __builtin_amdgcn_ballot_w64(bit != 0u);
            const uint32_t flip = bit - 1u;
            plo &= (uint32_t)bal ^ flip;
            phi &= (uint32_t)(bal >> 32) ^ flip;
        }
    }
    const uint64_t peers = ((uint64_t)phi << 32) | plo;
    return valid ? peers : 0ull;
}
template <int NBITS>
__device__ __forceinline__ uint32_t dls_rank(uint32_t *cnt, uint32_t d, int nbits, bool valid, int lane)
{
    if (ex4d_g_rank_lds != 0) return valid ? atomicAdd(&cnt[d], 1u) : 0u;
    const uint64_t peers = dls_peers<NBITS>(d, nbits, valid);
    const uint32_t rank = __popcll(peers & ((1ull << lane) - 1ull));
    const uint32_t before = cnt[valid ? d : 0u];
    if (valid && rank == 0) cnt[d] = before + (uint32_t)__popcll(peers);
    dls_wave_sync();
    return before + rank;
}
template <int THREADS>
__device__ __forceinline__ void dls_scan_counts(DlsLds<THREADS> &L, int nbits)
{
    constexpr int DLS_WAVES = THREADS / 64;
    const int tid = threadIdx.x, lane = tid & 63, wave = tid >> 6;
    constexpr int PER = 512 / THREADS;
    uint32_t c[PER][DLS_WAVES], tot = 0;
#pragma unroll
    for (int q = 0; q < PER; q++) {
        const bool live = tid * PER + q < (1 << nbits);
#pragma unroll
        for (int w = 0; w < DLS_WAVES; w++) { c[q][w] = live ? L.cnt[w][tid * PER + q] : 0u; tot += c[q][w]; }
    }
    uint32_t x = tot;
#pragma unroll
    for (int o = 1; o < 64; o <<= 1) { const uint32_t y = __shfl_up(x, o, 64); if (lane >= o) x += y; }
    if (lane == 63) L.scan_tmp[wave] = x;
    __syncthreads();
    uint32_t run = x - tot;
    for (int w = 0; w < wave; w++) run += L.scan_tmp[w];
#pragma unroll
    for (int q = 0; q < PER; q++) {
        if (tid * PER + q < (1 << nbits)) {
#pragma unroll
            for (int w = 0; w < DLS_WAVES; w++) { L.cnt[w][tid * PER + q] = run; run += c[q][w]; }
        }
    }
    __syncthreads();
}
__device__ __forceinline__ int dls_pass_bits(int rem, int lo, int npass, int pass) { return (rem - lo + (npass - pass) - 1) / (npass - pass); }

template <int THREADS>
__device__ __forceinline__ void dls_sort_through_memory(DlsLds<THREADS> &L, uint32_t *xk, uint32_t *xv, uint32_t *xr, uint32_t *yk, uint32_t *yv, uint32_t *yr,
    uint32_t n, int rem, uint32_t kmin)
{
    constexpr int DLS_WAVES = THREADS / 64, DLS_THREADS = THREADS;
    const int tid = threadIdx.x, lane = tid & 63, wave = tid >> 6;
    const int npass = (rem + 8) / 9;
    const uint32_t m = ((n + DLS_WAVES * 64 - 1) / (DLS_WAVES * 64)) * 64;
    const uint32_t wbase = wave * m < n ? wave * m : n, wend = (wbase + m) < n ? (wbase + m) : n;
    uint32_t *sk = xk, *sv = xv, *sr = xr, *dk = yk, *dv = yv, *dr = yr;
    for (int pass = 0, lo = 0; pass < npass; pass++) {
        const int nbits = dls_pass_bits(rem, lo, npass, pass);
        const uint32_t mask = (1u << nbits) - 1u;
        for (int i = lane; i < 512; i += 64) L.cnt[wave][i] = 0;
        dls_wave_sync();
        for (uint32_t i = wbase + lane; i < wend; i += 64) atomicAdd(&L.cnt[wave][((sk[i] - kmin) >> lo) & mask], 1u);
        __syncthreads();
        dls_scan_counts(L, nbits);
        for (uint32_t base = wbase; base < wend; base += 64) {
            const uint32_t i = base + lane;
            const bool valid = i < wend;
            const uint32_t k = valid ? sk[i] : 0u, v = valid ? sv[i] : 0u, r = valid ? sr[i] : 0u;
            const uint32_t d = ((k - kmin) >> lo) & mask;
            const uint32_t dst = dls_rank<0>(L.cnt[wave], d, nbits, valid, lane);
            if (valid) { dk[dst] = k; dv[dst] = v; dr[dst] = r; }
        }
        __threadfence();
        __syncthreads();
        uint32_t *t;
        t = sk; sk = dk; dk = t; t = sv; sv = dv; dv = t; t = sr; sr = dr; dr = t;
        lo += nbits;
    }
    if (sv != xv) {
        for (uint32_t i = tid; i < n; i += DLS_THREADS) { xv[i] = sv[i]; xr[i] = sr[i]; }
    }
}

__device__ __forceinline__ uint32_t rect4_count(uint32_t r) { return ((r >> 16) & 0xFFu) * (r >> 24); }
template <int THREADS>
__device__ __forceinline__ uint32_t dls_scan_chunk(DlsLds<THREADS> &L, uint32_t cn, uint32_t carry)
{
    constexpr int DLS_WAVES = THREADS / 64;
    const int tid = threadIdx.x, lane = tid & 63, wave = tid >> 6;
    uint32_t v[DLS_ITEMS], run = 0;
#pragma unroll
    for (int q = 0; q < DLS_ITEMS; q++) { const uint32_t i = tid * DLS_ITEMS + q; run += (i < cn) ? L.buf[i] : 0u; v[q] = run; }
    uint32_t x = run;
#pragma unroll
    for (int o = 1; o < 64; o <<= 1) { const uint32_t y = __shfl_up(x, o, 64); if (lane >= o) x += y; }
    if (lane == 63) L.scan_tmp[wave] = x;
    __syncthreads();
    uint32_t excl = carry + x - run, total = 0;
    for (int w = 0; w < DLS_WAVES; w++) { const uint32_t t = L.scan_tmp[w]; if (w < wave) excl += t; total += t; }
#pragma unroll
    for (int q = 0; q < DLS_ITEMS; q++) { const uint32_t i = tid * DLS_ITEMS + q; if (i < cn) L.buf[i] = excl + v[q]; }
    __syncthreads();
    return total;
}
template <int THREADS>
__device__ __forceinline__ uint32_t dls_scan_from_memory(DlsLds<THREADS> &L, const uint32_t *rects, uint32_t *local_incl, uint32_t n)
{
    constexpr int DLS_THREADS = THREADS, DLS_CAP = THREADS * DLS_ITEMS;
    const int tid = threadIdx.x;
    uint32_t carry = 0;
    for (uint32_t c0 = 0; c0 < n; c0 += DLS_CAP) {
        const uint32_t cn = (n - c0) < DLS_CAP ? (n - c0) : DLS_CAP;
        uint32_t r[DLS_ITEMS];
#pragma unroll
        for (int j = 0; j < DLS_ITEMS; j++) { const uint32_t p = tid + j * DLS_THREADS; r[j] = p < cn ? rects[c0 + p] : 0u; }
#pragma unroll
        for (int j = 0; j < DLS_ITEMS; j++) { const uint32_t p = tid + j * DLS_THREADS; if (p < cn) L.buf[p] = rect4_count(r[j]); }
        __syncthreads();
        carry += dls_scan_chunk(L, cn, carry);
#pragma unroll
        for (int j = 0; j < DLS_ITEMS; j++) { const uint32_t p = tid + j * DLS_THREADS; if (p < cn) local_incl[c0 + p] = L.buf[p]; }
        __syncthreads();
    }
    return carry;
}

template <int THREADS, int NBITS>
__device__ __forceinline__ void dls_lds_pass(DlsLds<THREADS> &L, uint32_t n, uint32_t m, int sh, int nbits)
{
    const int tid = threadIdx.x, lane = tid & 63, wave = tid >> 6;
    if (NBITS > 0) nbits = NBITS;
    const uint32_t mask = (1u << nbits) - 1u;
    const uint32_t wbase = wave * m;
    for (int i = lane; i < (1 << nbits); i += 64) L.cnt[wave][i] = 0;
    dls_wave_sync();
    uint32_t word[DLS_ITEMS], pos[DLS_ITEMS];
#pragma unroll
    for (int it = 0; it < DLS_ITEMS; it++) {
        word[it] = 0u; pos[it] = 0u;
        if ((uint32_t)(it * 64) < m) {
            const uint32_t i = wbase + it * 64 + lane;
            const bool valid = i < n;
            word[it] = valid ? L.buf[i] : 0u;
            pos[it] = dls_rank<NBITS>(L.cnt[wave], (word[it] >> sh) & mask, nbits, valid, lane);
        }
    }
    __syncthreads();
    dls_scan_counts(L, nbits);
#pragma unroll
    for (int it = 0; it < DLS_ITEMS; it++) {
        if ((uint32_t)(it * 64) < m) {
            const uint32_t i = wbase + it * 64 + lane;
            if (i < n) L.buf[L.cnt[wave][(word[it] >> sh) & mask] + pos[it]] = word[it];
        }
    }
    __syncthreads();
}

template <int THREADS>
__global__ __launch_bounds__(THREADS, THREADS == 512 ? 4 : 5) void depth_local_sort_kernel(uint32_t *kb, uint32_t *vb, uint32_t *rb, uint32_t *ka, uint32_t *va, uint32_t *ra,
    const uint32_t *__restrict__ starts, const uint32_t *__restrict__ totals, const uint32_t *__restrict__ dparams, uint32_t cap,
    uint32_t *__restrict__ local_incl, uint32_t *__restrict__ bucket_sums, int T, uint2 *__restrict__ ranges, uint32_t *__restrict__ watch)
{
    constexpr int DLS_THREADS = THREADS, DLS_WAVES = THREADS / 64, DLS_CAP = THREADS * DLS_ITEMS, IDX_BITS = DlsLds<THREADS>::IDX_BITS;
    __shared__ DlsLds<THREADS> L;
    const uint32_t b = blockIdx.x;
    const int tid = threadIdx.x;
    if (ranges) for (int i = b * DLS_THREADS + tid; i < T; i += gridDim.x * DLS_THREADS) ranges[i] = make_uint2(0u, 0u);
    const uint32_t n = totals[b], s = starts[b];
    const DlsParams dq = dls_params(dparams);
    const int rem = (int)dq.shift;
    const uint32_t inv_digit = gridDim.x - 1u;
    if (b == inv_digit || n == 0u) {
        if (bucket_sums && tid == 0) bucket_sums[b] = 0u;
        return;
    }
    const bool sorted_already = n < 2u || rem == 0;
    if (sorted_already || n > cap) {
        if (n > cap && watch && tid == 0) __hip_atomic_store(watch, 1u, __ATOMIC_RELAXED, __HIP_MEMORY_SCOPE_SYSTEM);
        if (!sorted_already) {
            dls_sort_through_memory(L, kb + s, vb + s, rb + s, ka + s, va + s, ra + s, n, rem, dq.kmin); __threadfence(); __syncthreads();
        }
        if (local_incl) {
            const uint32_t sum = dls_scan_from_memory(L, rb + s, local_incl + s, n);
            if (tid == 0) bucket_sums[b] = sum;
        }
        return;
    }
    const uint32_t remmask = (1u << rem) - 1u;
    {
        uint32_t k[DLS_ITEMS];
#pragma unroll
        for (int j = 0; j < DLS_ITEMS; j++) { const uint32_t p = tid + j * DLS_THREADS; k[j] = p < n ? kb[s + p] : 0u; }
#pragma unroll
        for (int j = 0; j < DLS_ITEMS; j++) { const uint32_t p = tid + j * DLS_THREADS; if (p < n) L.buf[p] = (((k[j] - dq.kmin) & remmask) << IDX_BITS) | p; }
    }
    __syncthreads();
    const int npass = (rem + 8) / 9;
    const uint32_t m = ((n + DLS_WAVES * 64 - 1) / (DLS_WAVES * 64)) * 64;
    if (rem == 16) { dls_lds_pass<THREADS, 8>(L, n, m, IDX_BITS, 8); dls_lds_pass<THREADS, 8>(L, n, m, IDX_BITS + 8, 8); }
    else if (rem == 17) { dls_lds_pass<THREADS, 9>(L, n, m, IDX_BITS, 9); dls_lds_pass<THREADS, 8>(L, n, m, IDX_BITS + 9, 8); }
    else {
        for (int pass = 0, lo = 0; pass < npass; pass++) {
            const int nbits = dls_pass_bits(rem, lo, npass, pass);
            dls_lds_pass<THREADS, 0>(L, n, m, IDX_BITS + lo, nbits);
            lo += nbits;
        }
    }
    uint32_t v[DLS_ITEMS], r[DLS_ITEMS];
#pragma unroll
    for (int j = 0; j < DLS_ITEMS; j++) {
        const uint32_t p = tid + j * DLS_THREADS;
        v[j] = 0u; r[j] = 0u;
        if (p < n) { const uint32_t idx = L.buf[p] & (DLS_CAP - 1u); v[j] = vb[s + idx]; r[j] = rb[s + idx]; }
    }
    asm volatile("s_waitcnt vmcnt(0)" ::: "memory");
    __syncthreads();
#pragma unroll
    for (int j = 0; j < DLS_ITEMS; j++) {
        const uint32_t p = tid + j * DLS_THREADS;
        if (p < n) { vb[s + p] = v[j]; rb[s + p] = r[j]; if (local_incl) L.buf[p] = rect4_count(r[j]); }
    }
    if (local_incl) {
        __syncthreads();
        const uint32_t sum = dls_scan_chunk(L, n, 0u);
#pragma unroll
        for (int j = 0; j < DLS_ITEMS; j++) { const uint32_t p = tid + j * DLS_THREADS; if (p < n) local_incl[s + p] = L.buf[p]; }
        if (tid == 0) bucket_sums[b] = sum;
    }
}

__device__ __forceinline__ uint2 unpack_rect(uint32_t p) { return make_uint2((p & 0xFFu) | (((p >> 8) & 0xFFu) << 16), ((p >> 16) & 0xFFu) | ((p >> 24) << 16)); }
__global__ __launch_bounds__(256) void scan_tiles_local_kernel(int P, const uint2 *__restrict__ rects, const uint32_t *__restrict__ rects4,
    const uint32_t *__restrict__ order, uint2 *__restrict__ sorted_rects, uint32_t *__restrict__ out, uint32_t *__restrict__ block_sums,
    int T, uint2 *__restrict__ ranges, uint32_t *__restrict__ frame_total)
{
    for (int i = blockIdx.x * 256 + threadIdx.x; i < T; i += gridDim.x * 256) ranges[i] = make_uint2(0u, 0u);
    __shared__ uint32_t cnt[SCAN_CHUNK];
    __shared__ uint32_t wave_sums[4];
    const int lane = threadIdx.x & 63, wave = threadIdx.x >> 6;
    const int block_first = blockIdx.x * SCAN_CHUNK;
#pragma unroll
    for (int it = 0; it < SCAN_CHUNK / 256; it++) {
        const int i = block_first + it * 256 + threadIdx.x;
        uint2 rc = make_uint2(0u, 0u);
        if (i < P) { rc = rects4 ? unpack_rect(rects4[order ? order[i] : (uint32_t)i]) : rects[order[i]]; if (sorted_rects) sorted_rects[i] = rc; }
        cnt[it * 256 + threadIdx.x] = (rc.y & 0xFFFFu) * (rc.y >> 16);
    }
    __syncthreads();
    uint32_t v[8];
    uint32_t run = 0;
#pragma unroll
    for (int k = 0; k < 8; k++) { run += cnt[threadIdx.x * 8 + k]; v[k] = run; }
    uint32_t x = run;
#pragma unroll
    for (int o = 1; o < 64; o <<= 1) { uint32_t y = __shfl_up(x, o, 64); if (lane >= o) x += y; }
    if (lane == 63) wave_sums[wave] = x;
    __syncthreads();
    uint32_t woff = 0;
    for (int w = 0; w < wave; w++) woff += wave_sums[w];
    const uint32_t excl = woff + x - run;
#pragma unroll
    for (int k = 0; k < 8; k++) cnt[threadIdx.x * 8 + k] = excl + v[k];
    __syncthreads();
#pragma unroll
    for (int it = 0; it < SCAN_CHUNK / 256; it++) {
        const int i = block_first + it * 256 + threadIdx.x;
        if (i < P) out[i] = cnt[it * 256 + threadIdx.x];
    }
    if (threadIdx.x == 255) {
        block_sums[blockIdx.x] = woff + x;
        if (frame_total) atomicAdd(frame_total, woff + x);
    }
}

template <int CTRL, int ROW_MASK>
__device__ __forceinline__ uint32_t dpp_max_u32(uint32_t x)
{
    const uint32_t y = (uint32_t)__builtin_amdgcn_update_dpp((int)x, (int)x, CTRL, ROW_MASK, 0xf, false);
    return y > x ? y : x;
}
__device__ __forceinline__ uint32_t wave_inclusive_max_u32(uint32_t x)
{
    x = dpp_max_u32<0x111, 0xf>(x);
    x = dpp_max_u32<0x112, 0xf>(x);
    x = dpp_max_u32<0x114, 0xf>(x);
    x = dpp_max_u32<0x118, 0xf>(x);
    x = dpp_max_u32<0x142, 0xa>(x);
    x = dpp_max_u32<0x143, 0xc>(x);
    return x;
}
struct DupRec { uint32_t off, gid, xy, w, magic; };
__global__ __launch_bounds__(256) void duplicate_kernel(int P, int gx, int gy, const uint32_t *__restrict__ order,
    const uint32_t *__restrict__ sorted_offsets, const uint32_t *__restrict__ block_sums,
    const uint2 *__restrict__ sorted_rects, const uint32_t *__restrict__ sorted_rects4,
    uint32_t *__restrict__ tile_keys, uint32_t *__restrict__ vals, uint32_t cap,
    const uint32_t *__restrict__ bucket_keys, const uint32_t *__restrict__ dparams, const uint32_t *__restrict__ bucket_sums, int nbuckets, uint32_t *__restrict__ frame_total)
{
    __shared__ DupRec s_rec[4][64];
    __shared__ uint32_t s_mark[4][64];
    __shared__ uint32_t s_base[1024];
    __shared__ uint32_t s_wsum[4];
    const int k = blockIdx.x * 256 + threadIdx.x;
    const int lane = threadIdx.x & 63, wave = threadIdx.x >> 6;
    if (bucket_keys) {
        const int per = nbuckets >> 8;
        uint32_t c[4], run = 0;
#pragma unroll
        for (int q = 0; q < 4; q++) { c[q] = q < per ? bucket_sums[threadIdx.x * per + q] : 0u; }
#pragma unroll
        for (int q = 0; q < 4; q++) { const uint32_t t = c[q]; c[q] = run; run += t; }
        uint32_t x = run;
#pragma unroll
        for (int o = 1; o < 64; o <<= 1) { const uint32_t y = __shfl_up(x, o, 64); if (lane >= o) x += y; }
        if (lane == 63) s_wsum[wave] = x;
        __syncthreads();
        uint32_t excl = x - run;
        for (int wv = 0; wv < wave; wv++) excl += s_wsum[wv];
#pragma unroll
        for (int q = 0; q < 4; q++) if (q < per) s_base[threadIdx.x * per + q] = excl + c[q];
        if (blockIdx.x == 0 && threadIdx.x == 255) *frame_total = excl + run;
        __syncthreads();
    }
    uint32_t gid = 0, off = 0, count = 0;
    int x0 = 0, y0 = 0, w = 1;
    if (k < P) {
        gid = order[k];
        const uint2 rc = sorted_rects4 ? unpack_rect(sorted_rects4[k]) : sorted_rects[k];
        x0 = (int)(rc.x & 0xFFFFu); y0 = (int)(rc.x >> 16);
        w = (int)(rc.y & 0xFFFFu);
        count = (uint32_t)w * (rc.y >> 16);
        if (w <= 0) w = 1;
        if (!bucket_keys) off = (k == 0) ? 0u : sorted_offsets[k - 1];
        else if (count != 0u) off = s_base[dls_digit(bucket_keys[k], dls_params(dparams), (uint32_t)nbuckets)] + sorted_offsets[k] - count;
    }
    if (!bucket_keys) {
        const int kf = blockIdx.x * 256 + (threadIdx.x & ~63) - 1;
        const int c0 = kf < 0 ? 0 : kf / SCAN_CHUNK;
        uint32_t part = 0;
        for (int j = lane; j < c0; j += 64) part += block_sums[j];
#pragma unroll
        for (int o = 32; o > 0; o >>= 1) part += __shfl_xor(part, o, 64);
        if (k > 0 && k < P) {
            const int c = (k - 1) / SCAN_CHUNK;
            off += part + (c > c0 ? block_sums[c0] : 0u);
        }
    }
    const uint32_t magic = 0xFFFFFFFFu / (uint32_t)w + 1u;
    uint32_t start = count != 0u ? off : 0xFFFFFFFFu, end = count != 0u ? off + count : 0u;
#pragma unroll
    for (int o = 32; o > 0; o >>= 1) {
        const uint32_t t = __shfl_xor(end, o, 64), u = __shfl_xor(start, o, 64);
        end = t > end ? t : end; start = u < start ? u : start;
    }
    s_rec[wave][lane] = { off, gid, (uint32_t)x0 | ((uint32_t)y0 << 16), (uint32_t)w, magic };
    uint32_t carry = 0;
    for (uint32_t tb = start; tb < end; tb += 64) {
        const uint32_t t = tb + lane;
        s_mark[wave][lane] = 0u;
        __builtin_amdgcn_fence(__ATOMIC_RELEASE, "wavefront"); __builtin_amdgcn_wave_barrier(); __builtin_amdgcn_fence(__ATOMIC_ACQUIRE, "wavefront");
        if (count != 0u && off - tb < 64u) s_mark[wave][off - tb] = (uint32_t)lane + 1u;
        __builtin_amdgcn_fence(__ATOMIC_RELEASE, "wavefront"); __builtin_amdgcn_wave_barrier(); __builtin_amdgcn_fence(__ATOMIC_ACQUIRE, "wavefront");
        uint32_t owner = wave_inclusive_max_u32(s_mark[wave][lane]);
        owner = owner > carry ? owner : carry;
        carry = (uint32_t)__builtin_amdgcn_readlane((int)owner, 63);
        if (t < end && t < cap) {
            const DupRec r = s_rec[wave][owner - 1u];
            const uint32_t local = t - r.off;
            uint32_t row = (r.w == 1u) ? local : __umulhi(local, r.magic);
            if (gx * gy > 65535) row = local / r.w;
            const uint32_t ty = (r.xy >> 16) + row, tx = (r.xy & 0xFFFFu) + (local - row * r.w);
            tile_keys[t] = ty * (uint32_t)gx + tx;
            vals[t] = r.gid;
        }
    }
}

__global__ __launch_bounds__(256) void zero_fill_kernel(uint4 *__restrict__ p, size_t n16, uint32_t tail_words)
{
    const uint4 z = make_uint4(0u, 0u, 0u, 0u);
    for (size_t i = (size_t)blockIdx.x * 256 + threadIdx.x; i < n16; i += (size_t)gridDim.x * 256) p[i] = z;
    if (blockIdx.x == 0 && threadIdx.x < tail_words) reinterpret_cast<uint32_t *>(p + n16)[threadIdx.x] = 0u;
}

__global__ __launch_bounds__(256) void tile_ranges_kernel(uint32_t R, const uint32_t *__restrict__ tile_ids, uint2 *__restrict__ ranges,
    const uint32_t *__restrict__ n_dev)
{
    if (n_dev) { const uint32_t nd = *n_dev; R = nd < R ? nd : R; }
    const uint32_t i = blockIdx.x * 256 + threadIdx.x;
    if (i >= R) return;
    const uint32_t cur = tile_ids[i];
    if (i == 0) ranges[cur].x = 0;
    else {
        const uint32_t prev = tile_ids[i - 1];
        if (cur != prev) { ranges[prev].y = i; ranges[cur].x = i; }
    }
    if (i == R - 1) ranges[cur].y = R;
}

#define SS_SAMPLE 8192
__device__ unsigned long long g_ss_stats[8];

template <int BINS>
__device__ __forceinline__ uint32_t ss_bucket_of(const uint32_t *ub, uint32_t key)
{
    const uint32_t K = 2u * key + 1u;
    uint32_t i = 0;
#pragma unroll
    for (uint32_t step = BINS / 2; step > 0; step >>= 1) if (ub[i + step - 1u] < K) i += step;
    return i;
}

template <int BINS>
__global__ __launch_bounds__(512) void ss_splitter_kernel(const uint32_t *__restrict__ keys, uint32_t n, uint32_t inv_key, int key_bits,
    uint32_t *__restrict__ table, unsigned long long *__restrict__ stats)
{
    __shared__ DlsLds<512> L;
    __shared__ uint32_t spl[BINS];
    const int tid = threadIdx.x, lane = tid & 63, wave = tid >> 6;
    const uint32_t stride = (n + SS_SAMPLE - 1u) / SS_SAMPLE;
    const uint32_t ns = (n + stride - 1u) / stride;
    {
        uint32_t k[DLS_ITEMS];
#pragma unroll
        for (int j = 0; j < DLS_ITEMS; j++) { const uint32_t p = tid + j * 512; k[j] = p < ns ? keys[p * stride] : 0u; }
#pragma unroll
        for (int j = 0; j < DLS_ITEMS; j++) { const uint32_t p = tid + j * 512; if (p < ns) L.buf[p] = k[j]; }
    }
    __syncthreads();
    const int npass = (key_bits + 8) / 9;
    const uint32_t m = ((ns + 8 * 64 - 1) / (8 * 64)) * 64;
    for (int pass = 0, lo = 0; pass < npass; pass++) {
        const int nbits = dls_pass_bits(key_bits, lo, npass, pass);
        dls_lds_pass<512, 0>(L, ns, m, lo, nbits);
        lo += nbits;
    }
    constexpr uint32_t NSPL = BINS - 2;
    for (uint32_t j = tid; j < (uint32_t)BINS; j += 512) spl[j] = j < NSPL ? L.buf[((j + 1u) * ns) / (NSPL + 1u)] : inv_key;
    __syncthreads();
    constexpr int PER = BINS / 512;
    uint32_t v[PER], c[PER], x = 0;
#pragma unroll
    for (int q = 0; q < PER; q++) {
        const uint32_t j = tid * PER + q;
        v[q] = spl[j];
        const bool first = j == 0u || spl[j - 1u] != v[q];
        const bool rep = first && j + 1u < (uint32_t)BINS && spl[j + 1u] == v[q];
        c[q] = first ? (rep ? 2u : 1u) : 0u;
        x += c[q] + (first ? 0x10000u : 0u);
    }
    const uint32_t own = x;
#pragma unroll
    for (int o = 1; o < 64; o <<= 1) { const uint32_t y = __shfl_up(x, o, 64); if (lane >= o) x += y; }
    if (lane == 63) L.scan_tmp[wave] = x;
    __syncthreads();
    uint32_t excl = x - own, total = 0;
    for (int w = 0; w < 8; w++) { const uint32_t t = L.scan_tmp[w]; if (w < wave) excl += t; total += t; }
    uint32_t off = excl & 0xFFFFu;
#pragma unroll
    for (int q = 0; q < PER; q++) {
        if (c[q] == 2u) { table[off] = 2u * v[q]; table[off + 1u] = 2u * v[q] + 1u; }
        else if (c[q] == 1u) table[off] = 2u * v[q] + 1u;
        off += c[q];
    }
    for (uint32_t j = (total & 0xFFFFu) + tid; j < (uint32_t)BINS; j += 512) table[j] = 0xFFFFFFFFu;
    if (stats && tid == 0) atomicAdd(&stats[7], (unsigned long long)(total >> 16));
}

template <int ITEMS, int BINS>
__global__ __launch_bounds__(RS_THREADS) void ss_histogram_kernel(const uint32_t *__restrict__ keys, uint32_t n, uint32_t nblocks,
    uint32_t *__restrict__ hist, const uint32_t *__restrict__ table)
{
    __shared__ uint32_t h[BINS];
    __shared__ uint32_t ub[BINS];
    for (int b = threadIdx.x; b < BINS; b += RS_THREADS) { h[b] = 0; ub[b] = table[b]; }
    const uint32_t base = blockIdx.x * (RS_THREADS * ITEMS);
    uint32_t k[ITEMS];
    if (base < n) {
#pragma unroll
        for (int it = 0; it < ITEMS; it++) {
            const uint32_t i = base + it * RS_THREADS + threadIdx.x;
            k[it] = keys[i < n ? i : n - 1];
        }
    }
    __syncthreads();
    if (base < n) {
#pragma unroll
        for (int it = 0; it < ITEMS; it++) {
            const uint32_t i = base + it * RS_THREADS + threadIdx.x;
            if (i < n) atomicAdd(&h[ss_bucket_of<BINS>(ub, k[it])], 1u);
        }
    }
    __syncthreads();
    for (int b = threadIdx.x; b < BINS; b += RS_THREADS) hist[(size_t)b * nblocks + blockIdx.x] = h[b];
}

template <int ITEMS, int BINS>
__global__ __launch_bounds__(RS_THREADS) void ss_scatter_kernel(const uint32_t *__restrict__ keys_in, const uint32_t *__restrict__ rects_in,
    uint32_t *__restrict__ keys_out, uint32_t *__restrict__ vals_out, uint32_t *__restrict__ rects_out, uint32_t n, uint32_t nblocks,
    const uint32_t *__restrict__ hist, const uint32_t *__restrict__ table, uint32_t *__restrict__ bucket_starts)
{
    constexpr uint32_t CHUNK = RS_THREADS * ITEMS;
    constexpr int NBITS = BINS == 512 ? 9 : 10, BPT = BINS / RS_THREADS;
    static_assert(BINS == 512 || BINS == 1024, "bucket counts of the sample sort");
    if (blockIdx.x * CHUNK >= n) return;
    __shared__ uint32_t wave_cnt[4][BINS];
    __shared__ uint32_t local_start[BINS];
    __shared__ uint32_t global_base[BINS];
    __shared__ uint32_t ub[BINS];
    __shared__ uint32_t scan_tmp[4];
    __shared__ uint2 stage[CHUNK];
    __shared__ uint32_t stage_r[CHUNK];
    static_assert(sizeof(uint32_t) * (7 * BINS + 4) + sizeof(uint32_t) * 3 * CHUNK <= 80 * 1024, "ss_scatter_kernel: static LDS beyond 80 KB");
    const int tid = threadIdx.x, lane = tid & 63, wave = tid >> 6;
    for (int i = tid; i < BINS; i += RS_THREADS) { ub[i] = table[i]; wave_cnt[0][i] = 0; wave_cnt[1][i] = 0; wave_cnt[2][i] = 0; wave_cnt[3][i] = 0; }
    const uint32_t block_first = blockIdx.x * CHUNK, block_end = n;
    const uint32_t base = block_first + wave * (CHUNK / 4);
    uint32_t pre_gt[BPT], pre_hb[BPT];
#pragma unroll
    for (int k = 0; k < BPT; k++) {
        const int d = tid * BPT + k;
        pre_gt[k] = hist[(size_t)BINS * nblocks + d];
        pre_hb[k] = hist[(size_t)d * nblocks + blockIdx.x];
    }
    uint32_t key[ITEMS], pos[ITEMS], rct[ITEMS], dig[ITEMS];
#pragma unroll
    for (int it = 0; it < ITEMS; it++) {
        const uint32_t i = base + it * 64 + lane;
        const uint32_t ic = i < block_end ? i : block_end - 1;
        key[it] = keys_in[ic];
        rct[it] = rects_in[ic];
    }
    __syncthreads();
#pragma unroll
    for (int it = 0; it < ITEMS; it++) {
        const uint32_t i = base + it * 64 + lane;
        dig[it] = ss_bucket_of<BINS>(ub, key[it]);
        pos[it] = dls_rank<NBITS>(wave_cnt[wave], dig[it], NBITS, i < block_end, lane);
    }
    __syncthreads();
    {
        uint32_t c[BPT][4], tot[BPT];
        uint32_t tsum = 0, gsum = 0;
#pragma unroll
        for (int k = 0; k < BPT; k++) {
            const int d = tid * BPT + k;
#pragma unroll
            for (int w = 0; w < 4; w++) c[k][w] = wave_cnt[w][d];
            tot[k] = c[k][0] + c[k][1] + c[k][2] + c[k][3];
            tsum += tot[k]; gsum += pre_gt[k];
        }
        uint32_t x = tsum, gx = gsum;
#pragma unroll
        for (int o = 1; o < 64; o <<= 1) {
            const uint32_t y = __shfl_up(x, o, 64), gy = __shfl_up(gx, o, 64);
            if (lane >= o) { x += y; gx += gy; }
        }
        if (lane == 63) { scan_tmp[wave] = x; local_start[wave] = gx; }
        __syncthreads();
        uint32_t ls = x - tsum, gb = gx - gsum;
        for (int w = 0; w < wave; w++) { ls += scan_tmp[w]; gb += local_start[w]; }
        __syncthreads();
#pragma unroll
        for (int k = 0; k < BPT; k++) {
            const int d = tid * BPT + k;
            local_start[d] = ls;
            global_base[d] = gb + pre_hb[k];
            if (blockIdx.x == 0) bucket_starts[d] = gb;
            wave_cnt[0][d] = ls; wave_cnt[1][d] = ls + c[k][0]; wave_cnt[2][d] = ls + c[k][0] + c[k][1]; wave_cnt[3][d] = ls + c[k][0] + c[k][1] + c[k][2];
            ls += tot[k]; gb += pre_gt[k];
        }
    }
    __syncthreads();
#pragma unroll
    for (int it = 0; it < ITEMS; it++) {
        const uint32_t i = base + it * 64 + lane;
        if (i < block_end) {
            const uint32_t slot = wave_cnt[wave][dig[it]] + pos[it];
            stage[slot] = make_uint2(key[it], i);
            stage_r[slot] = rct[it];
        }
    }
    __syncthreads();
    const uint32_t count = (block_end - block_first) < CHUNK ? (block_end - block_first) : CHUNK;
#pragma unroll 4
    for (uint32_t p = tid; p < count; p += RS_THREADS) {
        const uint2 kv = stage[p];
        const uint32_t d = ss_bucket_of<BINS>(ub, kv.x);
        const uint32_t dst = global_base[d] + (p - local_start[d]);
        keys_out[dst] = kv.x; vals_out[dst] = kv.y; rects_out[dst] = stage_r[p];
    }
}

template <int THREADS> struct SsLds { DlsLds<THREADS> L; uint16_t idx[THREADS * DLS_ITEMS]; };

template <int THREADS>
__device__ __forceinline__ void ss_pair_pass(SsLds<THREADS> &S, uint32_t n, uint32_t m, int lo, int nbits)
{
    DlsLds<THREADS> &L = S.L;
    const int tid = threadIdx.x, lane = tid & 63, wave = tid >> 6;
    const uint32_t mask = (1u << nbits) - 1u;
    const uint32_t wbase = wave * m;
    for (int i = lane; i < (1 << nbits); i += 64) L.cnt[wave][i] = 0;
    dls_wave_sync();
    uint32_t word[DLS_ITEMS], idx[DLS_ITEMS], pos[DLS_ITEMS];
#pragma unroll
    for (int it = 0; it < DLS_ITEMS; it++) {
        word[it] = 0u; idx[it] = 0u; pos[it] = 0u;
        if ((uint32_t)(it * 64) < m) {
            const uint32_t i = wbase + it * 64 + lane;
            const bool valid = i < n;
            word[it] = valid ? L.buf[i] : 0u;
            idx[it] = valid ? S.idx[i] : 0u;
            pos[it] = dls_rank<0>(L.cnt[wave], (word[it] >> lo) & mask, nbits, valid, lane);
        }
    }
    __syncthreads();
    dls_scan_counts(L, nbits);
#pragma unroll
    for (int it = 0; it < DLS_ITEMS; it++) {
        if ((uint32_t)(it * 64) < m) {
            const uint32_t i = wbase + it * 64 + lane;
            if (i < n) { const uint32_t dst = L.cnt[wave][(word[it] >> lo) & mask] + pos[it]; L.buf[dst] = word[it]; S.idx[dst] = (uint16_t)idx[it]; }
        }
    }
    __syncthreads();
}

template <int THREADS>
__global__ __launch_bounds__(THREADS) void ss_bucket_kernel(uint32_t *kb, uint32_t *vb, uint32_t *rb, uint32_t *ka, uint32_t *va, uint32_t *ra,
    const uint32_t *__restrict__ starts, const uint32_t *__restrict__ totals, const uint32_t *__restrict__ table, uint32_t cap,
    int T, uint2 *__restrict__ ranges, unsigned long long *__restrict__ stats)
{
    constexpr int DLS_THREADS = THREADS, DLS_WAVES = THREADS / 64, DLS_CAP = THREADS * DLS_ITEMS, IDX_BITS = DlsLds<THREADS>::IDX_BITS;
    __shared__ SsLds<THREADS> S;
    DlsLds<THREADS> &L = S.L;
    const uint32_t b = blockIdx.x;
    const int tid = threadIdx.x;
    if (ranges) for (int i = b * DLS_THREADS + tid; i < T; i += gridDim.x * DLS_THREADS) ranges[i] = make_uint2(0u, 0u);
    const uint32_t n = totals[b], s = starts[b];
    if (n == 0u) { if (stats && tid == 0) atomicAdd(&stats[0], 1ull); return; }
    const uint32_t ub_prev = b ? table[b - 1u] : 0u, ub_cur = table[b];
    const uint32_t klo = (ub_prev + 1u) >> 1, khi = (ub_cur - 1u) >> 1;
    const uint32_t span = khi - klo;
    const int rem = span ? 32 - __builtin_clz(span) : 0;
    if (stats && tid == 0 && span) atomicMax(&stats[6], (unsigned long long)n);
    if (n < 2u || span == 0u) { if (stats && tid == 0) atomicAdd(&stats[1], 1ull); return; }
    if (n > cap) {
        if (stats && tid == 0) { atomicAdd(&stats[4], 1ull); atomicAdd(&stats[5], (unsigned long long)n); }
        dls_sort_through_memory(L, kb + s, vb + s, rb + s, ka + s, va + s, ra + s, n, rem, klo);
        return;
    }
    const bool packed = rem + IDX_BITS <= 32;
    if (stats && tid == 0) atomicAdd(&stats[packed ? 2 : 3], 1ull);
    {
        uint32_t k[DLS_ITEMS];
#pragma unroll
        for (int j = 0; j < DLS_ITEMS; j++) { const uint32_t p = tid + j * DLS_THREADS; k[j] = p < n ? kb[s + p] : 0u; }
#pragma unroll
        for (int j = 0; j < DLS_ITEMS; j++) {
            const uint32_t p = tid + j * DLS_THREADS;
            if (p < n) { if (packed) L.buf[p] = ((k[j] - klo) << IDX_BITS) | p; else { L.buf[p] = k[j] - klo; S.idx[p] = (uint16_t)p; } }
        }
    }
    __syncthreads();
    const int npass = (rem + 8) / 9;
    const uint32_t m = ((n + DLS_WAVES * 64 - 1) / (DLS_WAVES * 64)) * 64;
    for (int pass = 0, lo = 0; pass < npass; pass++) {
        const int nbits = dls_pass_bits(rem, lo, npass, pass);
        if (packed) dls_lds_pass<THREADS, 0>(L, n, m, IDX_BITS + lo, nbits);
        else ss_pair_pass<THREADS>(S, n, m, lo, nbits);
        lo += nbits;
    }
    uint32_t v[DLS_ITEMS], r[DLS_ITEMS];
#pragma unroll
    for (int j = 0; j < DLS_ITEMS; j++) {
        const uint32_t p = tid + j * DLS_THREADS;
        v[j] = 0u; r[j] = 0u;
        if (p < n) { const uint32_t idx = packed ? (L.buf[p] & (DLS_CAP - 1u)) : S.idx[p]; v[j] = vb[s + idx]; r[j] = rb[s + idx]; }
    }
    asm volatile("s_waitcnt vmcnt(0)" ::: "memory");
    __syncthreads();
#pragma unroll
    for (int j = 0; j < DLS_ITEMS; j++) {
        const uint32_t p = tid + j * DLS_THREADS;
        if (p < n) { vb[s + p] = v[j]; rb[s + p] = r[j]; }
    }
}

}

static std::atomic<int> g_rank_lds_option{-1};
static std::mutex g_rank_lds_mu;
static int g_rank_lds_device = -1, g_rank_lds_value = 0;
void ex4d_set_rank_lds(int v) { std::lock_guard<std::mutex> lock(g_rank_lds_mu); g_rank_lds_option.store(v); g_rank_lds_device = -1; }
int ex4d_get_rank_lds() { return g_rank_lds_option.load(); }
int ex4d_rank_lds_in_use() { return g_rank_lds_value; }
hipError_t ex4d_prepare_rank_lds(hipStream_t stream)
{
    int dev = -1;
    if (hipGetDevice(&dev) != hipSuccess) return hipGetLastError();
    std::lock_guard<std::mutex> lock(g_rank_lds_mu);
    if (dev == g_rank_lds_device) return hipSuccess;
    hipStreamCaptureStatus st = hipStreamCaptureStatusNone;
    if (hipStreamIsCapturing(stream, &st) == hipSuccess && st != hipStreamCaptureStatusNone) return hipSuccess;
    (void)hipGetLastError();
    int want = g_rank_lds_option.load();
    if (want < 0) {
        uint32_t *bad = nullptr, h = 1;
        hipError_t e = hipMalloc((void **)&bad, sizeof(uint32_t));
        if (e != hipSuccess) return e;
        (void)hipMemset(bad, 0, sizeof(uint32_t));
        for (int nd : { 1, 3, 17, 64, 256 })
            hipLaunchKernelGGL(lds_rank_probe_kernel, dim3(256), dim3(256), 0, 0, 0x5EEDu + nd, 200, nd, bad);
        e = hipMemcpy(&h, bad, sizeof(uint32_t), hipMemcpyDeviceToHost);
        (void)hipFree(bad);
        if (e != hipSuccess) return e;
        want = h == 0u ? 1 : 0;
    }
    hipError_t e = hipMemcpyToSymbol(HIP_SYMBOL(ex4d_g_rank_lds), &want, sizeof(int));
    if (e != hipSuccess) return e;
    g_rank_lds_device = dev; g_rank_lds_value = want;
    return hipSuccess;
}

#define RS_SMALL_ITEMS 8
static inline int rs_items_for(uint32_t n) { return n <= (2u << 20) ? RS_SMALL_ITEMS : RS_ITEMS; }
static inline uint32_t rs_blocks_for(uint32_t n) { const uint32_t c = RS_THREADS * rs_items_for(n); return (n + c - 1) / c; }
static inline int rs_max_bits_for(uint32_t n) { return rs_items_for(n) == RS_SMALL_ITEMS ? 9 : 8; }
size_t ex4d_radix_hist_words(uint32_t n) { return (size_t)1024 * rs_blocks_for(n) + 1024; }
int ex4d_radix_passes(uint32_t n, int end_bit) { const int mb = rs_max_bits_for(n); return (end_bit + mb - 1) / mb; }

hipError_t ex4d_radix_sort_pairs(uint32_t *keys_a, uint32_t *vals_a, uint32_t *keys_b, uint32_t *vals_b,
    uint32_t n, int end_bit, uint32_t *hist, bool *result_in_a, hipStream_t stream, const uint32_t *n_dev, bool iota_values,
    const uint32_t *gather_in, uint32_t *gather_out, uint2 *zero_ranges, int num_ranges)
{
    *result_in_a = true;
    if (n == 0) return hipSuccess;
    const uint32_t nb = rs_blocks_for(n);
    const bool small = rs_items_for(n) == RS_SMALL_ITEMS;
    uint32_t *kin = keys_a, *vin = iota_values ? nullptr : vals_a, *kout = keys_b, *vout = vals_b;
    uint32_t *vnext = vals_a;
    const int npass = ex4d_radix_passes(n, end_bit);
    for (int pass = 0, shift = 0; pass < npass; pass++) {
        const int nbits = (end_bit - shift + (npass - pass) - 1) / (npass - pass);
        const uint32_t mask = (1u << nbits) - 1u;
        if (small) {
            hipLaunchKernelGGL((rs_histogram_kernel<RS_SMALL_ITEMS, 512, 1>), dim3(nb), dim3(RS_THREADS), 0, stream, kin, n, shift, mask, nb, hist, n_dev);
            hipLaunchKernelGGL(rs_scan_rows_kernel, dim3(1u << nbits), dim3(256), 0, stream, nb, hist, 512u);
            const bool last = pass == npass - 1;
#define RS_SMALL_SCATTER(NB) hipLaunchKernelGGL((rs_scatter_kernel<RS_SMALL_ITEMS, 512, 0, NB>), dim3(nb), dim3(RS_THREADS), 0, stream, kin, vin, kout, vout, n, shift, nbits, nb, hist, 0, nullptr, 0, \
                last ? zero_ranges : (uint2 *)nullptr, n_dev, last ? gather_in : (const uint32_t *)nullptr, last ? gather_out : (uint32_t *)nullptr, (uint32_t *)nullptr, (const uint32_t *)nullptr, (uint32_t)num_ranges)
            if (nbits == 9) RS_SMALL_SCATTER(9); else if (nbits == 8) RS_SMALL_SCATTER(8); else RS_SMALL_SCATTER(0);
#undef RS_SMALL_SCATTER
        } else {
            hipLaunchKernelGGL((rs_histogram_kernel<RS_ITEMS, 256, 1>), dim3(nb), dim3(RS_THREADS), 0, stream, kin, n, shift, mask, nb, hist, n_dev);
            hipLaunchKernelGGL(rs_scan_rows_kernel, dim3(1u << nbits), dim3(256), 0, stream, nb, hist, 256u);
            const bool last = pass == npass - 1;
            hipLaunchKernelGGL((rs_scatter_kernel<RS_ITEMS, 256, 0, 0>), dim3(nb), dim3(RS_THREADS), 0, stream, kin, vin, kout, vout, n, shift, nbits, nb, hist, 0, nullptr, 0,
                last ? zero_ranges : (uint2 *)nullptr, n_dev, last ? gather_in : (const uint32_t *)nullptr, last ? gather_out : (uint32_t *)nullptr, (uint32_t *)nullptr, (const uint32_t *)nullptr, (uint32_t)num_ranges);
        }
        uint32_t *t = kin; kin = kout; kout = t;
        t = (pass == 0) ? vnext : vin; vin = vout; vout = t;
        *result_in_a = !*result_in_a;
        shift += nbits;
    }
    return hipGetLastError();
}

bool ex4d_depth_sort_msd_applies(uint32_t n, int key_bits) { return n <= (1u << 26) && key_bits - (EX4D_DLS_MSD_BITS - 1) + DLS_IDX_BITS <= 32; }
int ex4d_depth_sort_msd_bits(uint32_t n, int key_bits)
{
    const int narrow = EX4D_DLS_MSD_BITS - 1;
    return (n <= 1300000u && key_bits - (narrow - 1) + DLS_IDX_BITS <= 32) ? narrow : EX4D_DLS_MSD_BITS;
}
template <int MB>
static hipError_t depth_sort_msd_launch(uint32_t *ka, uint32_t *va, uint32_t *ra, uint32_t *kb, uint32_t *vb, uint32_t *rb, uint32_t n, uint32_t inv_key,
    uint32_t *flags, const uint2 *wave_ranges, uint32_t *hist, uint32_t *starts, uint32_t local_cap, hipStream_t stream,
    uint32_t *local_incl, uint32_t *bucket_sums, int T, uint2 *ranges, int local_threads, uint32_t *watch)
{
    if (n == 0) return hipSuccess;
    constexpr int BINS = 1 << MB;
    const uint32_t nb = rs_blocks_for(n);
    const bool small = rs_items_for(n) == RS_SMALL_ITEMS;
    uint32_t *dparams = flags + EX4D_FLAG_DPARAMS;
    const uint32_t nranges = (n + 255u) / 256u;
    if (local_threads != 256 && local_threads != 512) local_threads = (MB < EX4D_DLS_MSD_BITS || n > 1200000u) ? 512 : 256;
    const uint32_t kcap = (uint32_t)local_threads * DLS_ITEMS;
    if (local_cap == 0 || local_cap > kcap) local_cap = kcap;
    if (small) {
        hipLaunchKernelGGL((dls_histogram_kernel<RS_SMALL_ITEMS, BINS>), dim3(nb), dim3(RS_THREADS), 0, stream, ka, n, nb, hist, dparams, wave_ranges, nranges, inv_key);
        hipLaunchKernelGGL(rs_scan_rows_kernel, dim3(BINS), dim3(256), 0, stream, nb, hist, (uint32_t)BINS);
        hipLaunchKernelGGL((rs_scatter_kernel<RS_SMALL_ITEMS, BINS, 3, MB>), dim3(nb), dim3(RS_THREADS), 0, stream, ka, (const uint32_t *)nullptr, kb, vb, n, 0, MB, nb, hist,
            0, (const uint32_t *)nullptr, 0, (uint2 *)nullptr, (const uint32_t *)nullptr, ra, rb, starts, (const uint32_t *)dparams);
    } else {
        hipLaunchKernelGGL((dls_histogram_kernel<RS_ITEMS, BINS>), dim3(nb), dim3(RS_THREADS), 0, stream, ka, n, nb, hist, dparams, wave_ranges, nranges, inv_key);
        hipLaunchKernelGGL(rs_scan_rows_kernel, dim3(BINS), dim3(256), 0, stream, nb, hist, (uint32_t)BINS);
        hipLaunchKernelGGL((rs_scatter_kernel<RS_ITEMS, BINS, 3, MB>), dim3(nb), dim3(RS_THREADS), 0, stream, ka, (const uint32_t *)nullptr, kb, vb, n, 0, MB, nb, hist,
            0, (const uint32_t *)nullptr, 0, (uint2 *)nullptr, (const uint32_t *)nullptr, ra, rb, starts, (const uint32_t *)dparams);
    }
    if (local_threads == 256)
        hipLaunchKernelGGL(depth_local_sort_kernel<256>, dim3(BINS), dim3(256), 0, stream, kb, vb, rb, ka, va, ra, starts, hist + (size_t)BINS * nb, (const uint32_t *)dparams, local_cap,
            local_incl, bucket_sums, T, ranges, watch);
    else
        hipLaunchKernelGGL(depth_local_sort_kernel<512>, dim3(BINS), dim3(512), 0, stream, kb, vb, rb, ka, va, ra, starts, hist + (size_t)BINS * nb, (const uint32_t *)dparams, local_cap,
            local_incl, bucket_sums, T, ranges, watch);
    return hipGetLastError();
}

hipError_t ex4d_depth_sort_msd(uint32_t *ka, uint32_t *va, uint32_t *ra, uint32_t *kb, uint32_t *vb, uint32_t *rb, uint32_t n, uint32_t inv_key,
    uint32_t *flags, const uint2 *wave_ranges, uint32_t *hist, uint32_t *starts, uint32_t local_cap, hipStream_t stream,
    uint32_t *local_incl, uint32_t *bucket_sums, int T, uint2 *ranges, int local_threads, uint32_t *watch, int msd_bits)
{
    if (msd_bits == EX4D_DLS_MSD_BITS - 1)
        return depth_sort_msd_launch<EX4D_DLS_MSD_BITS - 1>(ka, va, ra, kb, vb, rb, n, inv_key, flags, wave_ranges, hist, starts, local_cap, stream, local_incl, bucket_sums, T, ranges, local_threads, watch);
    return depth_sort_msd_launch<EX4D_DLS_MSD_BITS>(ka, va, ra, kb, vb, rb, n, inv_key, flags, wave_ranges, hist, starts, local_cap, stream, local_incl, bucket_sums, T, ranges, local_threads, watch);
}

template <int BINS>
static hipError_t depth_sort_sample_launch(uint32_t *ka, uint32_t *va, uint32_t *ra, uint32_t *kb, uint32_t *vb, uint32_t *rb, uint32_t n, uint32_t inv_key, int key_bits,
    uint32_t *hist, uint32_t *starts, uint32_t *table, uint32_t local_cap, hipStream_t stream, int T, uint2 *ranges, int local_threads, unsigned long long *stats)
{
    const uint32_t nb = rs_blocks_for(n);
    if (local_threads != 256 && local_threads != 512) local_threads = 512;
    const uint32_t kcap = (uint32_t)local_threads * DLS_ITEMS;
    if (local_cap == 0 || local_cap > kcap) local_cap = kcap;
    hipLaunchKernelGGL(ss_splitter_kernel<BINS>, dim3(1), dim3(512), 0, stream, (const uint32_t *)ka, n, inv_key, key_bits, table, stats);
    if (rs_items_for(n) == RS_SMALL_ITEMS) {
        hipLaunchKernelGGL((ss_histogram_kernel<RS_SMALL_ITEMS, BINS>), dim3(nb), dim3(RS_THREADS), 0, stream, (const uint32_t *)ka, n, nb, hist, (const uint32_t *)table);
        hipLaunchKernelGGL(rs_scan_rows_kernel, dim3(BINS), dim3(256), 0, stream, nb, hist, (uint32_t)BINS);
        hipLaunchKernelGGL((ss_scatter_kernel<RS_SMALL_ITEMS, BINS>), dim3(nb), dim3(RS_THREADS), 0, stream, (const uint32_t *)ka, (const uint32_t *)ra, kb, vb, rb, n, nb,
            (const uint32_t *)hist, (const uint32_t *)table, starts);
    } else {
        hipLaunchKernelGGL((ss_histogram_kernel<RS_ITEMS, BINS>), dim3(nb), dim3(RS_THREADS), 0, stream, (const uint32_t *)ka, n, nb, hist, (const uint32_t *)table);
        hipLaunchKernelGGL(rs_scan_rows_kernel, dim3(BINS), dim3(256), 0, stream, nb, hist, (uint32_t)BINS);
        hipLaunchKernelGGL((ss_scatter_kernel<RS_ITEMS, BINS>), dim3(nb), dim3(RS_THREADS), 0, stream, (const uint32_t *)ka, (const uint32_t *)ra, kb, vb, rb, n, nb,
            (const uint32_t *)hist, (const uint32_t *)table, starts);
    }
    if (local_threads == 256)
        hipLaunchKernelGGL(ss_bucket_kernel<256>, dim3(BINS), dim3(256), 0, stream, kb, vb, rb, ka, va, ra, (const uint32_t *)starts, (const uint32_t *)(hist + (size_t)BINS * nb),
            (const uint32_t *)table, local_cap, T, ranges, stats);
    else
        hipLaunchKernelGGL(ss_bucket_kernel<512>, dim3(BINS), dim3(512), 0, stream, kb, vb, rb, ka, va, ra, (const uint32_t *)starts, (const uint32_t *)(hist + (size_t)BINS * nb),
            (const uint32_t *)table, local_cap, T, ranges, stats);
    return hipGetLastError();
}

int ex4d_depth_sort_sample_bins(uint32_t n) { return n <= 1300000u ? 512 : 1024; }
hipError_t ex4d_depth_sort_sample(uint32_t *ka, uint32_t *va, uint32_t *ra, uint32_t *kb, uint32_t *vb, uint32_t *rb, uint32_t n, uint32_t inv_key, int key_bits,
    uint32_t *hist, uint32_t *starts, uint32_t *table, uint32_t local_cap, hipStream_t stream, int T, uint2 *ranges, int local_threads, bool census)
{
    if (n == 0) return hipSuccess;
    unsigned long long *stats = nullptr;
    if (census) { hipError_t e = hipGetSymbolAddress((void **)&stats, HIP_SYMBOL(g_ss_stats)); if (e != hipSuccess) return e; }
    if (ex4d_depth_sort_sample_bins(n) == 512)
        return depth_sort_sample_launch<512>(ka, va, ra, kb, vb, rb, n, inv_key, key_bits, hist, starts, table, local_cap, stream, T, ranges, local_threads, stats);
    return depth_sort_sample_launch<1024>(ka, va, ra, kb, vb, rb, n, inv_key, key_bits, hist, starts, table, local_cap, stream, T, ranges, local_threads, stats);
}
hipError_t ex4d_sample_sort_stats(unsigned long long *out8, int reset)
{
    hipError_t e = hipMemcpyFromSymbol(out8, HIP_SYMBOL(g_ss_stats), 8 * sizeof(unsigned long long));
    if (e == hipSuccess && reset) { unsigned long long z[8] = { 0 }; e = hipMemcpyToSymbol(HIP_SYMBOL(g_ss_stats), z, sizeof(z)); }
    return e;
}

bool ex4d_tile_sort_msd_applies(int P, int tile_bits)
{
    if (tile_bits < 9 || tile_bits > 16) return false;
    const int low_bits = (tile_bits + 1) / 2;
    return (uint64_t)P <= (1ull << (32 - low_bits));
}
static inline int ts_clamp_bits(int tile_bits) { return tile_bits > 16 ? 16 : (tile_bits < 2 ? 2 : tile_bits); }
static inline uint32_t ts_max_blocks(uint32_t R, int tile_bits) { return rs_num_blocks(R) + (1u << (tile_bits - (tile_bits + 1) / 2)) + 1u; }
size_t ex4d_tile_sort_hist_words(uint32_t R, int tile_bits) { return (size_t)256 * (rs_num_blocks(R) + 1) + (size_t)256 * (ts_max_blocks(R, ts_clamp_bits(tile_bits)) + 1); }

hipError_t ex4d_tile_sort_msd(const uint32_t *keys, const uint32_t *vals, uint32_t *packed, uint32_t *point_list, uint32_t *tile_ids_out,
    uint32_t R, int tile_bits, uint32_t *hist, uint2 *ranges, hipStream_t stream, const uint32_t *n_dev)
{
    if (R == 0) return hipSuccess;
    const int low_bits = (tile_bits + 1) / 2, high_bits = tile_bits - low_bits;
    const uint32_t nbA = rs_num_blocks(R), nbB = ts_max_blocks(R, tile_bits);
    uint32_t *histB = hist + (size_t)256 * (nbA + 1);
    const uint32_t *totals = hist + (size_t)256 * nbA;
    hipLaunchKernelGGL((rs_histogram_kernel<RS_ITEMS, 256, 8>), dim3(nbA), dim3(RS_THREADS), 0, stream, keys, R, low_bits, (1u << high_bits) - 1u, nbA, hist, n_dev);
    hipLaunchKernelGGL(rs_scan_rows_kernel, dim3(1u << high_bits), dim3(256), 0, stream, nbA, hist, 256u);
#define TS_SCATTER_A(NB) hipLaunchKernelGGL((rs_scatter_kernel<RS_ITEMS, 256, 1, NB>), dim3(nbA), dim3(RS_THREADS), 0, stream, keys, vals, packed, (uint32_t *)nullptr, \
        R, low_bits, high_bits, nbA, hist, low_bits, (const uint32_t *)nullptr, 0, (uint2 *)nullptr, n_dev)
    if (high_bits == 6) TS_SCATTER_A(6); else if (high_bits == 7) TS_SCATTER_A(7); else if (high_bits == 8) TS_SCATTER_A(8); else TS_SCATTER_A(0);
#undef TS_SCATTER_A
    hipLaunchKernelGGL(ts_histogram_kernel, dim3(nbB), dim3(RS_THREADS), 0, stream, packed, totals, 1 << high_bits, 32 - low_bits, nbB, histB);
    hipLaunchKernelGGL(rs_scan_rows_kernel, dim3(1u << low_bits), dim3(256), 0, stream, nbB, histB, 256u);
#define TS_SCATTER_B(NB) hipLaunchKernelGGL((rs_scatter_kernel<RS_ITEMS, 256, 2, NB>), dim3(nbB), dim3(RS_THREADS), 0, stream, packed, (const uint32_t *)nullptr, tile_ids_out, point_list, \
        R, 32 - low_bits, low_bits, nbB, histB, low_bits, totals, 1 << high_bits, ranges, (const uint32_t *)nullptr)
    if (low_bits == 7) TS_SCATTER_B(7); else if (low_bits == 8) TS_SCATTER_B(8); else TS_SCATTER_B(0);
#undef TS_SCATTER_B
    return hipGetLastError();
}

size_t ex4d_tile_sort_pass_b_hist_words(uint32_t R) { return (size_t)256 * (rs_num_blocks(R) + 258) + (size_t)6 * (rs_num_blocks(R) + 258); }
size_t ex4d_tile_sort_pass_b_table_offset(uint32_t R) { return (size_t)256 * (rs_num_blocks(R) + 258); }
hipError_t ex4d_tile_sort_pass_b(const uint32_t *packed, const uint32_t *totals, int nbuckets, int low_bits, uint32_t stride, uint32_t R, uint32_t cap,
    uint32_t *histB, uint32_t *point_list, uint32_t *tile_ids_out, uint2 *ranges, hipStream_t stream, const Ex4dTsBlock *block_table)
{
    if (R == 0) return hipSuccess;
    const uint32_t nbB = ex4d_tile_sort_pass_b_blocks(R, nbuckets);
    hipLaunchKernelGGL(ts_histogram_kernel, dim3(nbB), dim3(RS_THREADS), 0, stream, packed, totals, nbuckets, 32 - low_bits, nbB, histB, cap, block_table);
    hipLaunchKernelGGL(rs_scan_rows_kernel, dim3(1u << low_bits), dim3(256), 0, stream, nbB, histB, 256u);
#define TS_SCATTER_B(NB) hipLaunchKernelGGL((rs_scatter_kernel<RS_ITEMS, 256, 2, NB>), dim3(nbB), dim3(RS_THREADS), 0, stream, packed, (const uint32_t *)nullptr, tile_ids_out, point_list, \
        R, 32 - low_bits, low_bits, nbB, histB, low_bits, totals, nbuckets, ranges, (const uint32_t *)nullptr, (const uint32_t *)nullptr, (uint32_t *)nullptr, (uint32_t *)nullptr, \
        (const uint32_t *)nullptr, stride, cap, block_table)
    if (low_bits == 7) TS_SCATTER_B(7); else if (low_bits == 8) TS_SCATTER_B(8); else TS_SCATTER_B(0);
#undef TS_SCATTER_B
    return hipGetLastError();
}

hipError_t ex4d_launch_scan_tiles(int P, const uint2 *rects, const uint32_t *rects4, const uint32_t *order, uint2 *sorted_rects, uint32_t *sorted_offsets,
    uint32_t *block_sums, int T, uint2 *ranges, uint32_t *frame_total, hipStream_t stream)
{
    const int nb = (P + SCAN_CHUNK - 1) / SCAN_CHUNK;
    hipLaunchKernelGGL(scan_tiles_local_kernel, dim3(nb), dim3(256), 0, stream, P, rects, rects4, order, sorted_rects, sorted_offsets, block_sums, T, ranges, frame_total);
    return hipGetLastError();
}

hipError_t ex4d_launch_duplicate(int P, int W, int H, const uint32_t *order, const uint32_t *sorted_offsets,
    const uint32_t *block_sums, const uint2 *sorted_rects, const uint32_t *sorted_rects4, uint32_t *tile_keys, uint32_t *vals, uint32_t cap, hipStream_t stream,
    const uint32_t *bucket_keys, const uint32_t *dparams, const uint32_t *bucket_sums, uint32_t *frame_total, int msd_bits)
{
    const int gx = (W + EX4D_TILE - 1) / EX4D_TILE, gy = (H + EX4D_TILE - 1) / EX4D_TILE;
    hipLaunchKernelGGL(duplicate_kernel, dim3((P + 255) / 256), dim3(256), 0, stream, P, gx, gy, order, sorted_offsets, block_sums,
        sorted_rects, sorted_rects4, tile_keys, vals, cap, bucket_keys, dparams, bucket_sums, 1 << msd_bits, frame_total);
    return hipGetLastError();
}

hipError_t ex4d_launch_zero(void *ptr, size_t bytes, hipStream_t stream)
{
    const size_t n16 = bytes / 16;
    const uint32_t tail_words = (uint32_t)((bytes % 16) / 4);
    if (bytes == 0) return hipSuccess;
    size_t blocks = (n16 + 1023) / 1024;
    if (blocks > 8192) blocks = 8192;
    if (blocks == 0) blocks = 1;
    hipLaunchKernelGGL(zero_fill_kernel, dim3((unsigned)blocks), dim3(256), 0, stream, (uint4 *)ptr, n16, tail_words);
    return hipGetLastError();
}

hipError_t ex4d_launch_tile_ranges(uint32_t R, int T, const uint32_t *tile_ids, uint2 *ranges, hipStream_t stream, const uint32_t *n_dev)
{
    (void)T;
    if (R > 0)
        hipLaunchKernelGGL(tile_ranges_kernel, dim3((R + 255) / 256), dim3(256), 0, stream, R, tile_ids, ranges, n_dev);
    return hipGetLastError();
}
```

### ex4dgs_amd/csrc/ex4d_internal.h

```cpp
#pragma once
#include <hip/hip_runtime.h>
#include <stdint.h>
#include <stddef.h>
#include "../../include/ex4d_rasterizer.h"
#include "../../include/ex4d_attributes.h"

#define EX4D_ALIGN 256

static inline size_t ex4d_align_up(size_t x) { return (x + (EX4D_ALIGN - 1)) & ~(size_t)(EX4D_ALIGN - 1); }

#define EX4D_RECORD_FLOATS 16
#define EX4D_DLS_MSD_BITS 10
#define EX4D_CHUNK_FLOW 0x80000000u
#define EX4D_CHUNK_FILTERED 0x40000000u
#define EX4D_DSUMS_MARK 0x44535553u

struct GeomState {
    float4 *records;
    float *cov3D;
    uint8_t *clamped;
    uint32_t *tiles_touched;
    uint2 *rects;
    uint2 *sorted_rects;
    uint32_t *rects4;
    uint32_t *depth_order;
    uint32_t *sorted_offsets;
    uint32_t *sort_keys_a, *sort_keys_b, *sort_vals_b;
    uint32_t *bucket_sums;
    uint2 *key_ranges;
    uint32_t *sort_vals_a, *rects4_b, *bucket_starts;
    uint32_t *scan_block_sums;
    uint32_t *sort_hist;
    uint32_t *total;
    uint32_t *block_totals;
    uint32_t *row_hist;
    float *sh_dsums;
};
struct BinState {
    uint32_t *point_list;
    uint32_t *tile_ids;
    uint32_t *vals_tmp, *keys_tmp;
    uint32_t *sort_hist;
    uint32_t *qlist;
    uint32_t *qcount;
};
struct ImgState {
    float *final_T;
    uint32_t *n_contrib;
    uint2 *ranges;
};

#define RS_THREADS 256
#define RS_ITEMS 16
#define RS_CHUNK (RS_THREADS * RS_ITEMS)
#define RS_BINS 256
#define SCAN_CHUNK 2048

static inline uint32_t rs_num_blocks(uint32_t n) { return (n + RS_CHUNK - 1) / RS_CHUNK; }
struct Ex4dTsBlock { uint32_t start, count, bucket, fb_first, fb_next, bucket_start; };
static inline uint32_t ex4d_tile_sort_pass_b_blocks(uint32_t R, int nbuckets) { return rs_num_blocks(R) + (uint32_t)nbuckets + 1u; }

struct ShSplit { const float *dc[2]; const float *rest[2]; int n_static; };
struct ShSplitGrad { float *dc[2]; float *rest[2]; int n_static; };

hipError_t ex4d_launch_preprocess_fwd(const Ex4dParams &prm, const float *means3D, const float *dir3D, const float *scales,
    const float *rotations, const float *opacities, const float *shs, const float *cov3D_precomp,
    const float *colors_precomp, const float *viewmatrix, const float *projmatrix, const float *campos,
    int32_t *radii, GeomState g, uint32_t *prefilter_violation, ShSplit split,
    uint32_t *depth_keys, uint32_t *depth_vals, uint32_t depth_key_base, uint32_t depth_key_invisible, uint32_t *rects4, hipStream_t stream,
    uint32_t *key_range_slots = nullptr, bool global_flags = true);

hipError_t ex4d_launch_mark_visible(int P, const float *means3D, const float *viewmatrix, const float *projmatrix,
    float min_depth, float max_depth, uint8_t *present, hipStream_t stream);

hipError_t ex4d_launch_preprocess_bwd(const Ex4dParams &prm, const float *means3D, const int32_t *radii,
    const float *shs, const float *scales, const float *rotations, const float *cov3D_ptr,
    const float *viewmatrix, const float *projmatrix, const float *campos, GeomState g, const float *acc16,
    float *dL_dmeans2D, float *dL_dcolors, float *dL_dopacity, float *dL_dmeans3D, float *dL_dcov3D, float *dL_dsh,
    float *dL_dscales, float *dL_drotations, float *dL_ddir, ShSplit split, ShSplitGrad gsplit, hipStream_t stream);

hipError_t ex4d_radix_sort_pairs(uint32_t *keys_a, uint32_t *vals_a, uint32_t *keys_b, uint32_t *vals_b,
    uint32_t n, int end_bit, uint32_t *hist, bool *result_in_a, hipStream_t stream, const uint32_t *n_dev = nullptr, bool iota_values = false,
    const uint32_t *gather_in = nullptr, uint32_t *gather_out = nullptr, uint2 *zero_ranges = nullptr, int num_ranges = 0);
size_t ex4d_radix_hist_words(uint32_t n);
int ex4d_radix_passes(uint32_t n, int end_bit);

bool ex4d_tile_sort_msd_applies(int P, int tile_bits);
size_t ex4d_tile_sort_hist_words(uint32_t R, int tile_bits);
hipError_t ex4d_tile_sort_msd(const uint32_t *keys, const uint32_t *vals, uint32_t *packed, uint32_t *point_list, uint32_t *tile_ids_out,
    uint32_t R, int tile_bits, uint32_t *hist, uint2 *ranges, hipStream_t stream, const uint32_t *n_dev = nullptr);

bool ex4d_tile_sort_rows_applies(int P, int gx, int gy);
size_t ex4d_tile_sort_rows_geom_words(uint32_t P);
size_t ex4d_tile_sort_rows_hist_words(uint32_t R);
void ex4d_set_rows_probe(int v);
hipError_t ex4d_rows_prof(unsigned long long *out8, int reset);
hipError_t ex4d_tile_sort_rows(int P, int gx, int gy, const uint32_t *order, const uint32_t *r4, const uint2 *r8, uint32_t *words,
    uint32_t *point_list, uint32_t *tile_ids_out, uint32_t cap, uint32_t S, uint32_t *histA, uint32_t *histB, uint2 *ranges, uint32_t *frame_total, hipStream_t stream);

hipError_t ex4d_launch_scan_tiles(int P, const uint2 *rects, const uint32_t *rects4, const uint32_t *order, uint2 *sorted_rects, uint32_t *sorted_offsets,
    uint32_t *block_sums, int T, uint2 *ranges, uint32_t *frame_total, hipStream_t stream);
hipError_t ex4d_launch_duplicate(int P, int W, int H, const uint32_t *order, const uint32_t *sorted_offsets,
    const uint32_t *block_sums, const uint2 *sorted_rects, const uint32_t *sorted_rects4, uint32_t *tile_keys, uint32_t *vals, uint32_t cap, hipStream_t stream,
    const uint32_t *bucket_keys = nullptr, const uint32_t *dparams = nullptr, const uint32_t *bucket_sums = nullptr, uint32_t *frame_total = nullptr,
    int msd_bits = EX4D_DLS_MSD_BITS);

#define EX4D_FLAG_DPARAMS 8
#define EX4D_FLAG_WORDS 64
bool ex4d_depth_sort_msd_applies(uint32_t n, int key_bits);
hipError_t ex4d_depth_sort_msd(uint32_t *ka, uint32_t *va, uint32_t *ra, uint32_t *kb, uint32_t *vb, uint32_t *rb, uint32_t n, uint32_t inv_key,
    uint32_t *flags, const uint2 *wave_ranges, uint32_t *hist, uint32_t *starts, uint32_t local_cap, hipStream_t stream,
    uint32_t *local_incl, uint32_t *bucket_sums, int T, uint2 *ranges, int local_threads,
    uint32_t *watch = nullptr,
    int msd_bits = EX4D_DLS_MSD_BITS);
int ex4d_depth_sort_msd_bits(uint32_t n, int key_bits);
hipError_t ex4d_depth_sort_sample(uint32_t *ka, uint32_t *va, uint32_t *ra, uint32_t *kb, uint32_t *vb, uint32_t *rb, uint32_t n, uint32_t inv_key, int key_bits,
    uint32_t *hist, uint32_t *starts, uint32_t *table, uint32_t local_cap, hipStream_t stream, int T, uint2 *ranges, int local_threads, bool census);
int ex4d_depth_sort_sample_bins(uint32_t n);
hipError_t ex4d_sample_sort_stats(unsigned long long *out8, int reset);
void ex4d_set_rank_lds(int v);
int ex4d_get_rank_lds();
int ex4d_rank_lds_in_use();
hipError_t ex4d_prepare_rank_lds(hipStream_t stream);
hipError_t ex4d_launch_zero(void *ptr, size_t bytes, hipStream_t stream);
hipError_t ex4d_launch_tile_ranges(uint32_t R, int T, const uint32_t *tile_ids, uint2 *ranges, hipStream_t stream, const uint32_t *n_dev = nullptr);

void ex4d_set_preprocess_tune(int v);
int ex4d_get_preprocess_tune();
void ex4d_set_preprocess_fast(int v);
int ex4d_get_preprocess_fast();
void ex4d_set_fwd_asm(int on);
int ex4d_get_fwd_asm();
void ex4d_set_clamp_always(int on);
int ex4d_get_clamp_always();
void ex4d_set_bwd_pairs(int on);
int ex4d_get_bwd_pairs();
hipError_t ex4d_launch_composite_fwd(const Ex4dParams &prm, const uint2 *ranges, const uint32_t *point_list,
    const float *subpixel_offset, const float4 *records, const float *bg, float *final_T, uint32_t *n_contrib,
    float *out_color, float *out_depth, float *out_acc, float *out_flow, int32_t *out_idx, uint32_t *qlist, uint32_t *qcount,
    bool has_flow, hipStream_t stream);

hipError_t ex4d_launch_composite_bwd(const Ex4dParams &prm, const uint2 *ranges, const uint32_t *point_list,
    const float *subpixel_offset, const float *bg, const float4 *records, const float *out_depth, const float *out_acc,
    const float *final_T, const uint32_t *n_contrib, const float *dL_dpix, const float *dL_ddepth,
    const float *dL_dflow, const float *dL_dacc, float *acc16, const uint32_t *qlist, const uint32_t *qcount,
    int variant, hipStream_t stream);

hipError_t ex4d_bwd_stats(unsigned long long *out, int count, int reset);
```

### ex4dgs_amd/csrc/ex4d_rowsort.hip

```cpp
#include "ex4d_internal.h"

namespace {

#define ROW_THREADS 256
#define ROWA_GAUSS 256
#define ROWA_HINTS 1024
#define ROW_PAD 260

__device__ __forceinline__ void wsync()
{
    __builtin_amdgcn_fence(__ATOMIC_RELEASE, "wavefront");
    __builtin_amdgcn_wave_barrier();
    __builtin_amdgcn_fence(__ATOMIC_ACQUIRE, "wavefront");
}

struct RectU { uint32_t x0, y0, w, h; };
__device__ __forceinline__ RectU rect_at(const uint32_t *__restrict__ r4, const uint2 *__restrict__ r8, uint32_t k)
{
    if (r4) { const uint32_t p = r4[k]; return { p & 0xFFu, (p >> 8) & 0xFFu, (p >> 16) & 0xFFu, p >> 24 }; }
    const uint2 rc = r8[k];
    return { rc.x & 0xFFFFu, rc.x >> 16, rc.y & 0xFFFFu, rc.y >> 16 };
}

__device__ __forceinline__ uint32_t wave_incl_scan(uint32_t x, int lane)
{
#pragma unroll
    for (int o = 1; o < 64; o <<= 1) { const uint32_t y = __shfl_up(x, o, 64); if (lane >= o) x += y; }
    return x;
}
__device__ __forceinline__ uint32_t block_excl_scan(uint32_t v, uint32_t *tmp, uint32_t &total)
{
    const int lane = threadIdx.x & 63, wave = threadIdx.x >> 6;
    const uint32_t x = wave_incl_scan(v, lane);
    if (lane == 63) tmp[wave] = x;
    __syncthreads();
    uint32_t excl = x - v;
    total = 0;
#pragma unroll
    for (int w = 0; w < 4; w++) { const uint32_t t = tmp[w]; if (w < wave) excl += t; total += t; }
    __syncthreads();
    return excl;
}

__device__ __forceinline__ void block_excl_scan2(uint32_t a, uint32_t b, uint32_t *tmp, uint32_t &ea, uint32_t &eb, uint32_t &ta, uint32_t &tb)
{
    const int lane = threadIdx.x & 63, wave = threadIdx.x >> 6;
    const uint32_t xa = wave_incl_scan(a, lane), xb = wave_incl_scan(b, lane);
    if (lane == 63) { tmp[wave] = xa; tmp[4 + wave] = xb; }
    __syncthreads();
    ea = xa - a; eb = xb - b; ta = 0; tb = 0;
#pragma unroll
    for (int w = 0; w < 4; w++) { const uint32_t t = tmp[w], u = tmp[4 + w]; if (w < wave) { ea += t; eb += u; } ta += t; tb += u; }
    __syncthreads();
}

template <int NDIG>
__device__ __forceinline__ void wave_diff_to_counts(uint32_t *cnt, int lane)
{
    constexpr int PER = NDIG / 64;
    uint32_t v[PER], run = 0;
#pragma unroll
    for (int q = 0; q < PER; q++) { run += cnt[PER * lane + q]; v[q] = run; }
    const uint32_t excl = wave_incl_scan(run, lane) - run;
#pragma unroll
    for (int q = 0; q < PER; q++) cnt[PER * lane + q] = v[q] + excl;
}

__global__ __launch_bounds__(ROW_THREADS) void rows_seg_hist_kernel(uint32_t P, int NR, const uint32_t *__restrict__ r4, const uint2 *__restrict__ r8,
    uint32_t *__restrict__ hist, uint32_t nblocks, uint32_t *__restrict__ frame_total)
{
    __shared__ __attribute__((aligned(16))) uint32_t d_seg[4][ROW_PAD], d_inst[4][ROW_PAD];
    const int tid = threadIdx.x, lane = tid & 63, wave = tid >> 6;
    const uint32_t blk = blockIdx.x * 4 + wave;
    if (blk >= nblocks) return;
    uint32_t *ds = d_seg[wave], *di = d_inst[wave];
    RectU r[ROWA_GAUSS / 64];
#pragma unroll
    for (int it = 0; it < ROWA_GAUSS / 64; it++) {
        const uint32_t k = blk * ROWA_GAUSS + it * 64 + lane;
        r[it] = { 0u, 0u, 0u, 0u };
        if (k < P) r[it] = rect_at(r4, r8, k);
    }
    for (int i = lane; i < ROW_PAD; i += 64) { ds[i] = 0u; di[i] = 0u; }
    wsync();
    uint32_t inst = 0;
#pragma unroll
    for (int it = 0; it < ROWA_GAUSS / 64; it++) {
        if (r[it].w * r[it].h != 0u) {
            atomicAdd(&ds[r[it].y0], 1u); atomicAdd(&ds[r[it].y0 + r[it].h], 0xFFFFFFFFu);
            atomicAdd(&di[r[it].y0], r[it].w); atomicAdd(&di[r[it].y0 + r[it].h], 0u - r[it].w);
            inst += r[it].w * r[it].h;
        }
    }
    wsync();
    wave_diff_to_counts<256>(ds, lane);
    wave_diff_to_counts<256>(di, lane);
    wsync();
    for (int row = lane; row < NR; row += 64) {
        hist[(size_t)row * nblocks + blk] = ds[row];
        hist[(size_t)(NR + row) * nblocks + blk] = di[row];
    }
    (void)inst; (void)frame_total;
}

__global__ __launch_bounds__(256) void rows_scan_kernel(uint32_t len, uint32_t *__restrict__ hist, uint32_t nrows, uint32_t *__restrict__ frame_total, uint32_t first_total_row)
{
    __shared__ uint32_t wave_sums[4];
    __shared__ uint32_t carry_s;
    uint32_t *row = hist + (size_t)blockIdx.x * len;
    const int lane = threadIdx.x & 63, wave = threadIdx.x >> 6;
    const bool vec = ((((uintptr_t)row) & 15) == 0);
    if (threadIdx.x == 0) carry_s = 0;
    __syncthreads();
    for (uint32_t base = 0; base < len; base += 2048) {
        const uint32_t i0 = base + 8 * threadIdx.x;
        uint32_t v[8];
        if (vec && i0 + 8 <= len) {
            const uint4 a = *reinterpret_cast<const uint4 *>(row + i0), b = *reinterpret_cast<const uint4 *>(row + i0 + 4);
            v[0] = a.x; v[1] = a.y; v[2] = a.z; v[3] = a.w; v[4] = b.x; v[5] = b.y; v[6] = b.z; v[7] = b.w;
        } else {
#pragma unroll
            for (int k = 0; k < 8; k++) v[k] = (i0 + k < len) ? row[i0 + k] : 0u;
        }
        uint32_t run = 0;
#pragma unroll
        for (int k = 0; k < 8; k++) { const uint32_t t = v[k]; v[k] = run; run += t; }
        const uint32_t x = wave_incl_scan(run, lane);
        if (lane == 63) wave_sums[wave] = x;
        __syncthreads();
        uint32_t woff = carry_s + x - run;
        for (int w = 0; w < wave; w++) woff += wave_sums[w];
        if (vec && i0 + 8 <= len) {
            *reinterpret_cast<uint4 *>(row + i0) = make_uint4(woff + v[0], woff + v[1], woff + v[2], woff + v[3]);
            *reinterpret_cast<uint4 *>(row + i0 + 4) = make_uint4(woff + v[4], woff + v[5], woff + v[6], woff + v[7]);
        } else {
#pragma unroll
            for (int k = 0; k < 8; k++) if (i0 + k < len) row[i0 + k] = woff + v[k];
        }

        __syncthreads();
        if (threadIdx.x == 255) carry_s = woff + run;
        __syncthreads();
    }
    if (threadIdx.x == 0) {
        hist[(size_t)nrows * len + blockIdx.x] = carry_s;
        if (frame_total && blockIdx.x >= first_total_row && carry_s != 0u) atomicAdd(frame_total, carry_s);
    }
}

struct CovLds { uint2 cov[4][ROW_PAD]; };
struct LaneBits { uint32_t bit_lo, bit_hi, lt_lo, lt_hi; };
__device__ __forceinline__ LaneBits lane_bits(int lane)
{
    LaneBits b;
    const uint32_t one = 1u << (lane & 31);
    b.bit_lo = lane < 32 ? one : 0u; b.bit_hi = lane < 32 ? 0u : one;
    b.lt_lo = lane < 32 ? one - 1u : 0xFFFFFFFFu; b.lt_hi = lane < 32 ? 0u : one - 1u;
    return b;
}
__device__ __forceinline__ void cov_publish(uint2 *cov, uint32_t d0, uint32_t len, const LaneBits &lb)
{
    for (uint32_t j = 0; __builtin_amdgcn_ballot_w64(j < len) != 0ull; j++)
        if (j < len) { if (lb.bit_lo) atomicOr(&cov[d0 + j].x, lb.bit_lo); else atomicOr(&cov[d0 + j].y, lb.bit_hi); }
    wsync();
}
__device__ __forceinline__ void cov_retire(uint2 *cov, uint32_t *cnt, int ndig, int lane)
{
    wsync();
    for (int c = lane; c < ndig; c += 64) {
        const uint2 m = cov[c];
        const uint32_t k = __popc(m.x) + __popc(m.y);
        if (k != 0u) { cnt[c] += k; cov[c] = make_uint2(0u, 0u); }
    }
    wsync();
}

__device__ unsigned long long g_rows_prof[8];
template <int NRP, int CAP>
__global__ __launch_bounds__(ROW_THREADS) void rows_seg_scatter_kernel(uint32_t P, int NR, const uint32_t *__restrict__ order,
    const uint32_t *__restrict__ r4, const uint2 *__restrict__ r8, const uint32_t *__restrict__ hist, uint32_t nblocks,
    uint32_t *__restrict__ words, uint32_t cap, int shift, int probe, Ex4dTsBlock *__restrict__ block_table, uint32_t table_blocks)
{
    constexpr int PAD = NRP + 4;
    __shared__ __attribute__((aligned(16))) uint32_t wave_cnt[4][PAD];
    __shared__ __attribute__((aligned(16))) uint2 wave_cov[4][PAD];
    __shared__ uint32_t local_start[NRP], inst_base[NRP], row_word[NRP];
    __shared__ uint32_t tmp[8];
    __shared__ uint32_t s_total, s_words;
    __shared__ uint2 stage[CAP];
    __shared__ uint32_t winc[CAP + 256];
    __shared__ uint16_t hint[ROWA_HINTS];
    const int tid = threadIdx.x, lane = tid & 63, wave = tid >> 6;
    unsigned long long ts[8];
#define ROWS_TS(i) do { if (probe) ts[i] = __builtin_amdgcn_s_memtime(); } while (0)
    ROWS_TS(0);
    const uint32_t k = blockIdx.x * ROWA_GAUSS + tid;
    RectU rc = { 0u, 0u, 0u, 0u };
    uint32_t id = 0u;
    if (k < P) { rc = rect_at(r4, r8, k); id = order[k]; }
    if (rc.w * rc.h == 0u) rc.h = 0u;
    const uint32_t it = tid < NR ? hist[(size_t)2 * NR * nblocks + NR + tid] : 0u;
    const uint32_t ipre = tid < NR ? hist[(size_t)(NR + tid) * nblocks + blockIdx.x] : 0u;
    uint32_t *cnt = wave_cnt[wave];
    uint2 *cov = wave_cov[wave];
    for (int i = lane; i < PAD; i += 64) { cnt[i] = 0u; cov[i] = make_uint2(0u, 0u); }
    wsync();
    if (rc.h != 0u) { atomicAdd(&cnt[rc.y0], 1u); atomicAdd(&cnt[rc.y0 + rc.h], 0xFFFFFFFFu); }
    wsync();
    wave_diff_to_counts<NRP>(cnt, lane);
    ROWS_TS(1);
    __syncthreads();
    {
        uint32_t c[4], tot = 0;
#pragma unroll
        for (int w = 0; w < 4; w++) { c[w] = tid < NR ? wave_cnt[w][tid] : 0u; tot += c[w]; }
        uint32_t total, itotal, ls, is;
        block_excl_scan2(tot, it, tmp, ls, is, total, itotal);
        if (block_table && blockIdx.x == 0) {
            const uint32_t nblk = tid < NR ? (it + RS_CHUNK - 1u) / RS_CHUNK : 0u;
            uint32_t fb_total;
            const uint32_t fb = block_excl_scan(nblk, tmp, fb_total);
            for (uint32_t j = 0; j < nblk; j++) {
                const uint32_t within = j * RS_CHUNK;
                if (fb + j < table_blocks)
                    block_table[fb + j] = { is + within, (it - within) < RS_CHUNK ? (it - within) : (uint32_t)RS_CHUNK, (uint32_t)tid, fb, fb + nblk, is };
            }
            for (uint32_t e = fb_total + tid; e < table_blocks; e += ROW_THREADS) block_table[e] = { 0u, 0u, 0u, 0u, 0u, 0u };
        }
        if (tid < NRP) { local_start[tid] = ls; inst_base[tid] = is + ipre; }
        if (tid < NR) { wave_cnt[0][tid] = ls; wave_cnt[1][tid] = ls + c[0]; wave_cnt[2][tid] = ls + c[0] + c[1]; wave_cnt[3][tid] = ls + c[0] + c[1] + c[2]; }
        if (tid == 0) s_total = total;
    }
    __syncthreads();
    const uint32_t total = s_total;
    ROWS_TS(2);
    if (total == 0u) return;
    if (total > CAP) {
        stage[tid] = make_uint2(rc.x0 | (rc.y0 << 8) | (rc.w << 16) | (rc.h << 24), id);
        __syncthreads();
        if (tid < NR) {
            uint32_t pos = inst_base[tid];
            for (int kk = 0; kk < ROWA_GAUSS; kk++) {
                const uint2 e = stage[kk];
                const uint32_t x0 = e.x & 0xFFu, y0 = (e.x >> 8) & 0xFFu, w = (e.x >> 16) & 0xFFu, h = e.x >> 24;
                if ((uint32_t)tid - y0 < h) {
                    for (uint32_t j = 0; j < w; j++) if (pos + j < cap) words[pos + j] = ((x0 + j) << shift) | e.y;
                    pos += w;
                }
            }
        }
        return;
    }
    {
        const LaneBits lb = lane_bits(lane);
        const uint32_t h = rc.h, y0 = rc.y0;
        if (__builtin_amdgcn_ballot_w64(h != 0u) != 0ull) {
            cov_publish(cov, y0, h, lb);
            const uint32_t xw = rc.x0 | (rc.w << 8);
            for (uint32_t j0 = 0; __builtin_amdgcn_ballot_w64(j0 < h) != 0ull; j0 += 2) {
                uint2 m[2]; uint32_t c[2];
#pragma unroll
                for (int u = 0; u < 2; u++) { const uint32_t i = j0 + u < h ? y0 + j0 + u : 0u; m[u] = cov[i]; c[u] = cnt[i]; }
#pragma unroll
                for (int u = 0; u < 2; u++) {
                    if (j0 + u < h) {
                        const uint32_t ty = y0 + j0 + u;
                        const uint32_t slot = c[u] + __popc(m[u].x & lb.lt_lo) + __popc(m[u].y & lb.lt_hi);
                        stage[slot] = make_uint2(id, xw | (ty << 16));
                    }
                }
            }
        }
    }
    ROWS_TS(3);
    __syncthreads();
    {
        constexpr int KP = CAP / ROW_THREADS;
        uint32_t wv[KP], sum = 0;
#pragma unroll
        for (int q = 0; q < KP; q++) { const uint32_t p = tid * KP + q; wv[q] = p < total ? (stage[p].y >> 8) & 0xFFu : 0u; sum += wv[q]; }
        uint32_t all;
        uint32_t run = block_excl_scan(sum, tmp, all);
        int sh = 3;
        while (((all - 1u) >> sh) >= ROWA_HINTS) sh++;
#pragma unroll
        for (int q = 0; q < KP; q++) {
            const uint32_t p = tid * KP + q;
            winc[p] = p < total ? run : 0xFFFFFFFFu;
            if (wv[q] != 0u) for (uint32_t bkt = (run + (1u << sh) - 1u) >> sh; bkt <= (run + wv[q] - 1u) >> sh; bkt++) hint[bkt] = (uint16_t)p;
            run += wv[q];
        }
        winc[CAP + tid] = 0xFFFFFFFFu;
        if (tid == 0) s_words = all;
    }
    __syncthreads();
    const uint32_t nwords = s_words;
    ROWS_TS(4);
    if (tid < NRP) { const uint32_t ls = local_start[tid]; row_word[tid] = ls < total ? winc[ls] : nwords; }
    __syncthreads();
    ROWS_TS(5);
    int sh = 3;
    while (((nwords - 1u) >> sh) >= ROWA_HINTS) sh++;
    for (uint32_t q0 = tid; q0 < nwords; q0 += 4 * ROW_THREADS) {
        uint32_t q[4], p[4];
#pragma unroll
        for (int u = 0; u < 4; u++) { q[u] = q0 + u * ROW_THREADS; p[u] = hint[(q[u] < nwords ? q[u] : q0) >> sh]; }
        for (uint32_t step = 1u << (sh - 1); step > 0; step >>= 1) {
            uint32_t wv[4];
#pragma unroll
            for (int u = 0; u < 4; u++) wv[u] = winc[p[u] + step];
#pragma unroll
            for (int u = 0; u < 4; u++) if (wv[u] <= q[u]) p[u] += step;
        }
        uint2 seg[4]; uint32_t w0[4];
#pragma unroll
        for (int u = 0; u < 4; u++) { seg[u] = stage[p[u]]; w0[u] = winc[p[u]]; }
        uint32_t ib[4], rw[4];
#pragma unroll
        for (int u = 0; u < 4; u++) { const uint32_t ty = seg[u].y >> 16; ib[u] = inst_base[ty]; rw[u] = row_word[ty]; }
#pragma unroll
        for (int u = 0; u < 4; u++) {
            const uint32_t dst = ib[u] + (q[u] - rw[u]);
            if (q[u] < nwords && dst < cap) words[dst] = (((seg[u].y & 0xFFu) + (q[u] - w0[u])) << shift) | seg[u].x;
        }
    }
    ROWS_TS(6);
    if (probe && tid == 0) { for (int i = 0; i < 6; i++) atomicAdd(&g_rows_prof[i], ts[i + 1] - ts[i]); atomicAdd(&g_rows_prof[7], 1ull); }
#undef ROWS_TS
}

static inline int bits_for(int n) { int b = 1; while ((1 << b) < n) b++; return b; }

}

hipError_t ex4d_tile_sort_pass_b(const uint32_t *packed, const uint32_t *totals, int nbuckets, int low_bits, uint32_t stride, uint32_t R, uint32_t cap,
    uint32_t *histB, uint32_t *point_list, uint32_t *tile_ids_out, uint2 *ranges, hipStream_t stream, const Ex4dTsBlock *block_table);
size_t ex4d_tile_sort_pass_b_hist_words(uint32_t R);
size_t ex4d_tile_sort_pass_b_table_offset(uint32_t R);

static int g_rows_probe = 0;
void ex4d_set_rows_probe(int v) { g_rows_probe = v; }
hipError_t ex4d_rows_prof(unsigned long long *out8, int reset)
{
    hipError_t e = hipMemcpyFromSymbol(out8, HIP_SYMBOL(g_rows_prof), 8 * sizeof(unsigned long long));
    if (e == hipSuccess && reset) { unsigned long long z[8] = { 0 }; e = hipMemcpyToSymbol(HIP_SYMBOL(g_rows_prof), z, sizeof(z)); }
    return e;
}
bool ex4d_tile_sort_rows_applies(int P, int gx, int gy) { return gx <= 255 && gy <= 255 && (uint32_t)P <= (1u << 24); }
size_t ex4d_tile_sort_rows_geom_words(uint32_t P) { return (size_t)2 * 255 * ((P + 255) / 256 + 1) + 64; }
size_t ex4d_tile_sort_rows_hist_words(uint32_t R) { return ex4d_tile_sort_pass_b_hist_words(R); }

hipError_t ex4d_tile_sort_rows(int P, int gx, int gy, const uint32_t *order, const uint32_t *r4, const uint2 *r8, uint32_t *words,
    uint32_t *point_list, uint32_t *tile_ids_out, uint32_t cap, uint32_t S, uint32_t *histA, uint32_t *histB, uint2 *ranges, uint32_t *frame_total, hipStream_t stream)
{
    if (P <= 0 || cap == 0) return hipSuccess;
    const uint32_t nbA = ((uint32_t)P + ROWA_GAUSS - 1) / ROWA_GAUSS;
    uint32_t *totA = histA + (size_t)2 * gy * nbA;
    const int bx = bits_for(gx);
    hipLaunchKernelGGL(rows_seg_hist_kernel, dim3((nbA + 3) / 4), dim3(ROW_THREADS), 0, stream, (uint32_t)P, gy, r4, r8, histA, nbA, frame_total);
    hipLaunchKernelGGL(rows_scan_kernel, dim3(2 * gy), dim3(256), 0, stream, nbA, histA, (uint32_t)(2 * gy), frame_total, (uint32_t)gy);
    const bool big = S == 0 ? (uint64_t)cap > 20ull * (uint32_t)P : 2ull * S > 7ull * (uint32_t)P;
    Ex4dTsBlock *block_table = reinterpret_cast<Ex4dTsBlock *>(histB + ex4d_tile_sort_pass_b_table_offset(cap));
    const uint32_t table_blocks = ex4d_tile_sort_pass_b_blocks(cap, gy);
#define ROWS_A(NRP, CAP) hipLaunchKernelGGL((rows_seg_scatter_kernel<NRP, CAP>), dim3(nbA), dim3(ROW_THREADS), 0, stream, (uint32_t)P, gy, order, r4, r8, (const uint32_t *)histA, nbA, \
        words, cap, 32 - bx, g_rows_probe, block_table, table_blocks)
    if (gy <= 64) { if (big) ROWS_A(64, 2048); else ROWS_A(64, 1024); }
    else if (gy <= 128) { if (big) ROWS_A(128, 2048); else ROWS_A(128, 1024); }
    else { if (big) ROWS_A(256, 2048); else ROWS_A(256, 1024); }
#undef ROWS_A
    hipError_t e = hipGetLastError();
    if (e != hipSuccess) return e;
    return ex4d_tile_sort_pass_b(words, totA + gy, gy, bx, (uint32_t)gx, cap, cap, histB, point_list, tile_ids_out, ranges, stream, block_table);
}
```

### include/ex4d_rasterizer.h

```cpp
#ifndef EX4D_RASTERIZER_H_INCLUDED
#define EX4D_RASTERIZER_H_INCLUDED

#include <stddef.h>
#include <stdint.h>

#ifdef __cplusplus
extern "C" {
#endif

#define EX4D_TILE 16
#define EX4D_CHANNELS 3

typedef struct Ex4dParams {
    int32_t P;
    int32_t D;
    int32_t M;
    int32_t W, H;
    float tanfovx, tanfovy;
    float kernel_size;
    float scale_modifier;
    float min_depth, max_depth;
    int32_t prefiltered;
    int32_t debug;
    int32_t prepare_backward;
    int32_t instance_capacity;
    int32_t assume_no_flow;
    int32_t reserved;
} Ex4dParams;

typedef struct Ex4dFrameStatus {
    uint32_t num_rendered;
    uint32_t prefilter_violation;
    uint32_t has_flow;
    uint32_t reserved[5];
} Ex4dFrameStatus;

typedef void *(*ex4d_alloc_fn)(void *user, size_t bytes);

enum {
    EX4D_OK = 0,
    EX4D_ERR_ARG = 1,
    EX4D_ERR_HIP = 2,
    EX4D_ERR_ALLOC = 3,
    EX4D_ERR_PREFILTERED = 4
};

const char *ex4d_last_error(void);

int ex4d_abi_version(void);
const char *ex4d_target_arch(void);

int ex4d_forward(
    const Ex4dParams *prm,
    const float *background,
    const float *means3D,
    const float *dir3D,
    const float *shs,
    const float *colors_precomp,
    const float *opacities,
    const float *scales,
    const float *rotations,
    const float *cov3D_precomp,
    const float *viewmatrix,
    const float *projmatrix,
    const float *campos,
    const float *subpixel_offset,
    ex4d_alloc_fn geom_alloc, void *geom_user,
    ex4d_alloc_fn binning_alloc, void *binning_user,
    ex4d_alloc_fn img_alloc, void *img_user,
    float *out_color, int32_t *radii, float *out_depth, float *out_acc, float *out_flow, int32_t *out_idx,
    void *stream,
    int32_t *num_rendered);

int ex4d_backward(
    const Ex4dParams *prm, int32_t num_rendered,
    const float *background, const float *means3D, const int32_t *radii,
    const float *shs, const float *colors_precomp, const float *scales, const float *rotations,
    const float *cov3D_precomp, const float *viewmatrix, const float *projmatrix, const float *campos,
    const float *subpixel_offset,
    const float *out_depth, const float *out_acc,
    const void *geom_buffer, const void *binning_buffer, const void *img_buffer,
    const float *dL_dout_color , const float *dL_dout_depth ,
    const float *dL_dout_flow , const float *dL_dout_acc ,
    float *dL_dmeans2D , float *dL_dcolors , float *dL_dopacity ,
    float *dL_dmeans3D , float *dL_dcov3D , float *dL_dsh ,
    float *dL_dscales , float *dL_drotations , float *dL_ddir ,
    void *bwd_scratch,
    void *stream);

size_t ex4d_backward_scratch_bytes(int32_t P);

typedef struct Ex4dSplitSH { const float *dc[2]; const float *rest[2]; int32_t n_static; } Ex4dSplitSH;
typedef struct Ex4dSplitSHGrad { float *dc[2]; float *rest[2]; int32_t n_static; } Ex4dSplitSHGrad;

int ex4d_forward_split_sh(
    const Ex4dParams *prm, const float *background, const float *means3D, const float *dir3D, const Ex4dSplitSH *shs,
    const float *opacities, const float *scales, const float *rotations, const float *cov3D_precomp,
    const float *viewmatrix, const float *projmatrix, const float *campos, const float *subpixel_offset,
    ex4d_alloc_fn geom_alloc, void *geom_user, ex4d_alloc_fn binning_alloc, void *binning_user,
    ex4d_alloc_fn img_alloc, void *img_user,
    float *out_color, int32_t *radii, float *out_depth, float *out_acc, float *out_flow, int32_t *out_idx,
    void *stream, int32_t *num_rendered);

int ex4d_backward_split_sh(
    const Ex4dParams *prm, int32_t num_rendered,
    const float *background, const float *means3D, const int32_t *radii,
    const Ex4dSplitSH *shs, const float *scales, const float *rotations,
    const float *cov3D_precomp, const float *viewmatrix, const float *projmatrix, const float *campos,
    const float *subpixel_offset, const float *out_depth, const float *out_acc,
    const void *geom_buffer, const void *binning_buffer, const void *img_buffer,
    const float *dL_dout_color, const float *dL_dout_depth, const float *dL_dout_flow, const float *dL_dout_acc,
    float *dL_dmeans2D, float *dL_dcolors, float *dL_dopacity, float *dL_dmeans3D, float *dL_dcov3D, const Ex4dSplitSHGrad *dL_dsh,
    float *dL_dscales, float *dL_drotations, float *dL_ddir, void *bwd_scratch, void *stream);

int ex4d_mark_visible(int32_t P, const float *means3D, const float *viewmatrix, const float *projmatrix,
                      float min_depth, float max_depth, uint8_t *present, void *stream);

size_t ex4d_geom_bytes(int32_t P);
size_t ex4d_binning_bytes(int32_t num_rendered, int32_t W, int32_t H);
size_t ex4d_img_bytes(int32_t W, int32_t H);

typedef struct Ex4dGeomLayout {
    size_t records;
    size_t cov3D;
    size_t clamped;
    size_t tiles_touched;
    size_t depth_order;
    size_t sorted_offsets;
    size_t rects;
    size_t total;
} Ex4dGeomLayout;
typedef struct Ex4dBinningLayout {
    size_t point_list;
    size_t tile_ids;
    size_t qlist;
    size_t qcount;
    size_t total;
} Ex4dBinningLayout;
typedef struct Ex4dImgLayout {
    size_t final_T;
    size_t n_contrib;
    size_t ranges;
    size_t total;
} Ex4dImgLayout;
void ex4d_geom_layout(int32_t P, Ex4dGeomLayout *out);
void ex4d_binning_layout(int32_t num_rendered, int32_t W, int32_t H, Ex4dBinningLayout *out);
void ex4d_img_layout(int32_t W, int32_t H, Ex4dImgLayout *out);

int ex4d_set_option(const char *name, int value);
int ex4d_get_option(const char *name);
int ex4d_debug_bwd_stats(unsigned long long *out8, int reset);
int ex4d_debug_bwd_stats16(unsigned long long *out16, int reset);
int ex4d_debug_rows_prof(unsigned long long *out8, int reset);
int ex4d_debug_sample_sort(unsigned long long *out8, int reset);

void ex4d_profile_enable(int on);
int ex4d_profile_read(int which, float *ms, const char **names, int max_stages);

#ifdef __cplusplus
}
#endif
#endif
```

Before: 0.6503 ms/frame.

## Fuse tile-row histogram into depth local sort buckets

```diff
diff --git a/ex4dgs_amd/_C.py b/ex4dgs_amd/_C.py
--- a/ex4dgs_amd/_C.py
+++ b/ex4dgs_amd/_C.py
@@ -366,6 +366,13 @@
                 ranges=i[lay.ranges: lay.ranges + 8 * T].view(torch.int32).view(T, 2))
 
 
+def rows_fused_views(geomBuffer, P):
+    out = (C.c_size_t * 4)()
+    _abi.call("ex4d_debug_rows_fused_layout", int(P), out)
+    hist, table, path, words = (int(x) for x in out)
+    return dict(hist=geomBuffer[hist: table].view(torch.int32), table=geomBuffer[table: table + 4 * words].view(torch.int32), path_offset=path)
+
+
 def set_option(name, value):
     _abi.call("ex4d_set_option", name.encode(), int(value))
 
diff --git a/ex4dgs_amd/_abi.py b/ex4dgs_amd/_abi.py
--- a/ex4dgs_amd/_abi.py
+++ b/ex4dgs_amd/_abi.py
@@ -146,6 +146,7 @@
         _status("ex4d_debug_bwd_stats16", P(C.c_ulonglong), cint),
         _status("ex4d_debug_rows_prof", P(C.c_ulonglong), cint),
         _status("ex4d_debug_sample_sort", P(C.c_ulonglong), cint),
+        _status("ex4d_debug_rows_fused_layout", i32, P(size)),
         _value("ex4d_profile_enable", None, cint),
         _value("ex4d_profile_read", cint, cint, P(f32), P(text), cint))),
     "ex4d_attributes.h": ("ex4d_attributes_last_error", (
diff --git a/ex4dgs_amd/csrc/ex4d_api.hip b/ex4dgs_amd/csrc/ex4d_api.hip
--- a/ex4dgs_amd/csrc/ex4d_api.hip
+++ b/ex4dgs_amd/csrc/ex4d_api.hip
@@ -12,6 +12,8 @@
 std::atomic<int> g_bwd_variant{4};
 std::atomic<int> g_tile_ids{0};
 std::atomic<int> g_tile_rows{1};
+std::atomic<int> g_rows_fused{1};
+std::atomic<int> g_rows_fused_frames{0};
 std::atomic<int> g_depth_msd{3};
 struct DepthSortWatch {
     std::mutex mu;
@@ -190,6 +192,7 @@
     g.total = c.take<uint32_t>(EX4D_FLAG_WORDS);
     g.block_totals = c.take<uint32_t>(2 * (((size_t)P + 63) / 64));
     g.row_hist = c.take<uint32_t>(ex4d_tile_sort_rows_geom_words((uint32_t)P));
+    g.row_blocks = c.take<uint32_t>(ex4d_rows_fused_table_words((uint32_t)P));
     g.sh_dsums = c.take<float>(9 * (size_t)P);
     l.total = c.off;
     if (lay) *lay = l;
@@ -358,6 +361,8 @@
     const bool rows_sort = g_tile_rows.load(std::memory_order_relaxed) != 0 && ex4d_tile_sort_rows_applies(P, gx, gy);
     const bool fused_scan = msd_mode == 2 && !rows_sort;
     const bool lsd_gather = !msd_depth && rows_sort && packed_rects;
+    const bool rows_fused = g_rows_fused.load(std::memory_order_relaxed) != 0 && msd_mode == 2 && rows_sort;
+    const Ex4dRowsFused rows_hist = { g.row_hist, g.row_blocks, ex4d_rows_fused_blocks((uint32_t)P, msd_bits), (uint32_t)ex4d_rows_fused_path_offset((uint32_t)P), gy };
     if (msd_depth) {
         if (sample_depth) {
             g_depth_sample_frames.fetch_add(1);
@@ -369,7 +374,8 @@
             STAGE(ex4d_depth_sort_msd(g.sort_keys_a, g.sort_vals_a, g.rects4, g.sort_keys_b, g.depth_order, g.rects4_b, (uint32_t)P, key_invisible,
                                       g.total, g.key_ranges, g.sort_hist, g.bucket_starts, (uint32_t)g_depth_local_cap.load(std::memory_order_relaxed), stream,
                                       fused_scan ? g.sorted_offsets : nullptr, fused_scan ? g.bucket_sums : nullptr, T, (fused_scan || rows_sort) ? im.ranges : nullptr,
-                                      g_depth_local_threads.load(std::memory_order_relaxed), msd_watch, msd_bits), prm, stream);
+                                      g_depth_local_threads.load(std::memory_order_relaxed), msd_watch, msd_bits, rows_fused ? &rows_hist : nullptr), prm, stream);
+            if (rows_fused) g_rows_fused_frames.fetch_add(1);
         }
         MARK(0, "depth_sort");
         if (!fused_scan && !rows_sort) {
@@ -440,7 +446,8 @@
         if (R > 0) {
             STAGE(ex4d_tile_sort_rows(P, gx, gy, g.depth_order, dup_rects4, dup_rects, b.keys_tmp, b.point_list,
                                       g_tile_ids.load(std::memory_order_relaxed) ? b.tile_ids : nullptr, R, segment_sum, g.row_hist, b.sort_hist, im.ranges,
-                                      (async && (msd_depth || lsd_gather)) ? g.total : nullptr, stream), prm, stream);
+                                      (async && (msd_depth || lsd_gather)) ? g.total : nullptr, stream,
+                                      rows_fused ? g.row_blocks : nullptr, rows_hist.nblocks), prm, stream);
         }
         if (async && (msd_depth || lsd_gather)) HIP_TRY(hipMemcpyAsync(num_rendered, g.total, sizeof(Ex4dFrameStatus), hipMemcpyDefault, stream));
         MARK(0, "tile_sort");
@@ -606,6 +613,7 @@
     if (name && !strcmp(name, "composite_clamp_always") && (value == 0 || value == 1)) { ex4d_set_clamp_always(value); return EX4D_OK; }
     if (name && !strcmp(name, "composite_bwd_pairs") && (value == 0 || value == 1)) { ex4d_set_bwd_pairs(value); return EX4D_OK; }
     if (name && !strcmp(name, "tile_sort_rows") && (value == 0 || value == 1)) { g_tile_rows.store(value); return EX4D_OK; }
+    if (name && !strcmp(name, "rows_hist_fused") && (value == 0 || value == 1)) { g_rows_fused.store(value); g_rows_fused_frames.store(0); return EX4D_OK; }
     if (name && !strcmp(name, "rank_lds_atomics") && value >= -1 && value <= 1) { ex4d_set_rank_lds(value); return EX4D_OK; }
     if (name && !strcmp(name, "rows_probe")) { ex4d_set_rows_probe(value); return EX4D_OK; }
     if (name && !strcmp(name, "preprocess_sh_predicate") && (value == 0 || value == 1)) { ex4d_set_preprocess_tune(value); return EX4D_OK; }
@@ -624,6 +632,15 @@
 int ex4d_debug_bwd_stats(unsigned long long *out8, int reset) { return ex4d_bwd_stats(out8, 8, reset) == hipSuccess ? EX4D_OK : EX4D_ERR_HIP; }
 int ex4d_debug_rows_prof(unsigned long long *out8, int reset) { return ex4d_rows_prof(out8, reset) == hipSuccess ? EX4D_OK : EX4D_ERR_HIP; }
 int ex4d_debug_sample_sort(unsigned long long *out8, int reset) { return ex4d_sample_sort_stats(out8, reset) == hipSuccess ? EX4D_OK : EX4D_ERR_HIP; }
+int ex4d_debug_rows_fused_layout(int32_t P, size_t *out4)
+{
+    if (P <= 0 || !out4) return EX4D_ERR_ARG;
+    const uintptr_t base = EX4D_ALIGN;
+    const GeomState g = carve_geom((void *)base, P, nullptr, nullptr);
+    out4[0] = (size_t)((uintptr_t)g.row_hist - base); out4[1] = (size_t)((uintptr_t)g.row_blocks - base);
+    out4[2] = ex4d_rows_fused_path_offset((uint32_t)P); out4[3] = ex4d_rows_fused_table_words((uint32_t)P);
+    return EX4D_OK;
+}
 int ex4d_debug_bwd_stats16(unsigned long long *out16, int reset) { return ex4d_bwd_stats(out16, 16, reset) == hipSuccess ? EX4D_OK : EX4D_ERR_HIP; }
 
 int ex4d_get_option(const char *name)
@@ -634,6 +651,8 @@
     if (name && !strcmp(name, "composite_clamp_always")) return ex4d_get_clamp_always();
     if (name && !strcmp(name, "composite_bwd_pairs")) return ex4d_get_bwd_pairs();
     if (name && !strcmp(name, "tile_sort_rows")) return g_tile_rows.load();
+    if (name && !strcmp(name, "rows_hist_fused")) return g_rows_fused.load();
+    if (name && !strcmp(name, "rows_hist_fused_frames")) return g_rows_fused_frames.load();
     if (name && !strcmp(name, "rank_lds_atomics")) return ex4d_get_rank_lds();
     if (name && !strcmp(name, "rank_lds_atomics_in_use")) return ex4d_rank_lds_in_use();
     if (name && !strcmp(name, "preprocess_sh_predicate")) return ex4d_get_preprocess_tune();
diff --git a/ex4dgs_amd/csrc/ex4d_binning.hip b/ex4dgs_amd/csrc/ex4d_binning.hip
--- a/ex4dgs_amd/csrc/ex4d_binning.hip
+++ b/ex4dgs_amd/csrc/ex4d_binning.hip
@@ -621,11 +621,106 @@
 }
 
 template <int THREADS>
+__device__ __forceinline__ uint32_t dls_blocks_before_part(const uint32_t *__restrict__ totals, uint32_t b)
+{
+    uint32_t part = 0;
+    for (uint32_t i = threadIdx.x; i < b; i += THREADS) part += (totals[i] + 255u) >> 8;
+    return part;
+}
+template <int THREADS>
+__device__ __forceinline__ void dls_part_to_lds(DlsLds<THREADS> &L, uint32_t part)
+{
+#pragma unroll
+    for (int o = 32; o > 0; o >>= 1) part += __shfl_xor(part, o, 64);
+    if ((threadIdx.x & 63) == 0) L.scan_tmp[threadIdx.x >> 6] = part;
+}
+template <int THREADS>
+__device__ __forceinline__ uint32_t dls_parts_sum(const DlsLds<THREADS> &L)
+{
+    uint32_t sum = 0;
+#pragma unroll
+    for (int w = 0; w < THREADS / 64; w++) sum += L.scan_tmp[w];
+    return sum;
+}
+__device__ __forceinline__ void dls_rows_count_blocks(uint32_t *d, const uint32_t (&r)[2][4], int lane)
+{
+    for (int i = lane; i < 512; i += 64) d[i] = 0u;
+    dls_wave_sync();
+#pragma unroll
+    for (int u = 0; u < 2; u++) {
+#pragma unroll
+        for (int it = 0; it < 4; it++) {
+            const uint32_t y0 = (r[u][it] >> 8) & 0xFFu, w = (r[u][it] >> 16) & 0xFFu, h = r[u][it] >> 24;
+            if (w * h != 0u && y0 + h < 256u) {
+                atomicAdd(&d[256 * u + y0], (1u << 16) | w); atomicAdd(&d[256 * u + y0 + h], 0u - ((1u << 16) | w));
+            }
+        }
+    }
+    dls_wave_sync();
+    uint32_t v[2][4], run[2] = { 0u, 0u }, x[2];
+#pragma unroll
+    for (int u = 0; u < 2; u++) {
+#pragma unroll
+        for (int q = 0; q < 4; q++) { run[u] += d[256 * u + 4 * lane + q]; v[u][q] = run[u]; }
+        x[u] = run[u];
+    }
+#pragma unroll
+    for (int o = 1; o < 64; o <<= 1) {
+        const uint32_t y0 = __shfl_up(x[0], o, 64), y1 = __shfl_up(x[1], o, 64);
+        if (lane >= o) { x[0] += y0; x[1] += y1; }
+    }
+#pragma unroll
+    for (int u = 0; u < 2; u++) {
+#pragma unroll
+        for (int q = 0; q < 4; q++) d[256 * u + 4 * lane + q] = v[u][q] + (x[u] - run[u]);
+    }
+}
+template <int THREADS, typename Rect>
+__device__ __forceinline__ void dls_rows_hist_bucket(DlsLds<THREADS> &L, const Ex4dRowsFused &rh, uint32_t base, uint32_t n, Rect rect)
+{
+    constexpr uint32_t WAVES = THREADS / 64, COLS = 2 * WAVES;
+    const uint32_t tid = threadIdx.x, lane = tid & 63u, wave = tid >> 6;
+    const uint32_t nblk = (n + 255u) >> 8, NR = (uint32_t)rh.NR;
+    for (uint32_t q0 = 0; q0 < nblk; q0 += COLS) {
+        if (q0 + wave < nblk) {
+            uint32_t rr[2][4];
+#pragma unroll
+            for (int u = 0; u < 2; u++) {
+#pragma unroll
+                for (int it = 0; it < 4; it++) { const uint32_t p = 256u * (q0 + WAVES * u + wave) + 64u * it + lane; rr[u][it] = p < n ? rect(p) : 0u; }
+            }
+            dls_rows_count_blocks(L.cnt[wave], rr, (int)lane);
+        }
+        __syncthreads();
+        const uint32_t nq = (nblk - q0) < COLS ? (nblk - q0) : COLS;
+        for (uint32_t i = tid; i < 2u * NR * COLS; i += THREADS) {
+            const uint32_t c = i % COLS, row = i / COLS;
+            if (c < nq && base + q0 + c < rh.nblocks) {
+                const uint32_t word = L.cnt[c % WAVES][256u * (c / WAVES) + (row < NR ? row : row - NR)];
+                rh.hist[(size_t)row * rh.nblocks + base + q0 + c] = row < NR ? word >> 16 : word & 0xFFFFu;
+            }
+        }
+        __syncthreads();
+    }
+}
+template <int THREADS>
+__device__ __forceinline__ void dls_rows_records(const Ex4dRowsFused &rh, uint32_t b, uint32_t base, uint32_t s, uint32_t n, uint32_t path)
+{
+    uint2 *rec = reinterpret_cast<uint2 *>(rh.table) + 1;
+    const uint32_t nblk = (n + 255u) >> 8;
+    for (uint32_t q = threadIdx.x; q < nblk; q += THREADS)
+        if (base + q < rh.nblocks) rec[base + q] = make_uint2(s + 256u * q, (n - 256u * q) < 256u ? (n - 256u * q) : 256u);
+    if (threadIdx.x == 0) rh.table[rh.path_offset + b] = path;
+}
+
+template <int THREADS, bool ROWS>
 __global__ __launch_bounds__(THREADS, THREADS == 512 ? 4 : 5) void depth_local_sort_kernel(uint32_t *kb, uint32_t *vb, uint32_t *rb, uint32_t *ka, uint32_t *va, uint32_t *ra,
     const uint32_t *__restrict__ starts, const uint32_t *__restrict__ totals, const uint32_t *__restrict__ dparams, uint32_t cap,
-    uint32_t *__restrict__ local_incl, uint32_t *__restrict__ bucket_sums, int T, uint2 *__restrict__ ranges, uint32_t *__restrict__ watch)
+    uint32_t *__restrict__ local_incl, uint32_t *__restrict__ bucket_sums, int T, uint2 *__restrict__ ranges, uint32_t *__restrict__ watch, Ex4dRowsFused rh)
 {
     constexpr int DLS_THREADS = THREADS, DLS_WAVES = THREADS / 64, DLS_CAP = THREADS * DLS_ITEMS, IDX_BITS = DlsLds<THREADS>::IDX_BITS;
+    static_assert(sizeof(DlsLds<THREADS>) <= 64 * 1024, "the bucket kernel's LDS (two workgroups of 512 per CU and more): the row histogram gets none of its own");
+    static_assert(sizeof(DlsLds<THREADS>::cnt) == sizeof(uint32_t) * DLS_WAVES * 2 * 256, "a wave's counter row holds its two difference arrays over 256 tile rows");
     __shared__ DlsLds<THREADS> L;
     const uint32_t b = blockIdx.x;
     const int tid = threadIdx.x;
@@ -634,8 +729,21 @@
     const DlsParams dq = dls_params(dparams);
     const int rem = (int)dq.shift;
     const uint32_t inv_digit = gridDim.x - 1u;
+    uint32_t blocks_part = 0;
+    if (ROWS) blocks_part = dls_blocks_before_part<THREADS>(totals, b);
     if (b == inv_digit || n == 0u) {
         if (bucket_sums && tid == 0) bucket_sums[b] = 0u;
+        if (ROWS) {
+            if (tid == 0) rh.table[rh.path_offset + b] = EX4D_ROWS_PATH_NONE;
+            if (b == inv_digit) {
+                dls_part_to_lds(L, blocks_part);
+                __syncthreads();
+                const uint32_t used = dls_parts_sum(L);
+                uint2 *rec = reinterpret_cast<uint2 *>(rh.table) + 1;
+                if (tid == 0) { rh.table[0] = used < rh.nblocks ? used : rh.nblocks; rh.table[1] = 0u; }
+                for (uint32_t e = used + tid; e < rh.nblocks; e += DLS_THREADS) rec[e] = make_uint2(0u, 0u);
+            }
+        }
         return;
     }
     const bool sorted_already = n < 2u || rem == 0;
@@ -648,6 +756,14 @@
             const uint32_t sum = dls_scan_from_memory(L, rb + s, local_incl + s, n);
             if (tid == 0) bucket_sums[b] = sum;
         }
+        if (ROWS) {
+            dls_part_to_lds(L, blocks_part);
+            __syncthreads();
+            const uint32_t base = dls_parts_sum(L);
+            const uint32_t *sorted = rb + s;
+            dls_rows_hist_bucket(L, rh, base, n, [sorted](uint32_t p) { return sorted[p]; });
+            dls_rows_records<THREADS>(rh, b, base, s, n, EX4D_ROWS_PATH_MEMORY);
+        }
         return;
     }
     const uint32_t remmask = (1u << rem) - 1u;
@@ -658,7 +774,10 @@
 #pragma unroll
         for (int j = 0; j < DLS_ITEMS; j++) { const uint32_t p = tid + j * DLS_THREADS; if (p < n) L.buf[p] = (((k[j] - dq.kmin) & remmask) << IDX_BITS) | p; }
     }
-    __syncthreads();
+    if (ROWS) dls_part_to_lds(L, blocks_part);
+    __syncthreads();
+    uint32_t first_block = 0;
+    if (ROWS) first_block = dls_parts_sum(L);
     const int npass = (rem + 8) / 9;
     const uint32_t m = ((n + DLS_WAVES * 64 - 1) / (DLS_WAVES * 64)) * 64;
     if (rem == 16) { dls_lds_pass<THREADS, 8>(L, n, m, IDX_BITS, 8); dls_lds_pass<THREADS, 8>(L, n, m, IDX_BITS + 8, 8); }
@@ -682,7 +801,13 @@
 #pragma unroll
     for (int j = 0; j < DLS_ITEMS; j++) {
         const uint32_t p = tid + j * DLS_THREADS;
-        if (p < n) { vb[s + p] = v[j]; rb[s + p] = r[j]; if (local_incl) L.buf[p] = rect4_count(r[j]); }
+        if (p < n) { vb[s + p] = v[j]; rb[s + p] = r[j]; if (local_incl) L.buf[p] = rect4_count(r[j]); if (ROWS) L.buf[p] = r[j]; }
+    }
+    if (ROWS) {
+        __syncthreads();
+        const uint32_t *sorted = L.buf;
+        dls_rows_hist_bucket(L, rh, first_block, n, [sorted](uint32_t p) { return sorted[p]; });
+        dls_rows_records<THREADS>(rh, b, first_block, s, n, EX4D_ROWS_PATH_LDS);
     }
     if (local_incl) {
         __syncthreads();
@@ -1240,7 +1365,7 @@
 template <int MB>
 static hipError_t depth_sort_msd_launch(uint32_t *ka, uint32_t *va, uint32_t *ra, uint32_t *kb, uint32_t *vb, uint32_t *rb, uint32_t n, uint32_t inv_key,
     uint32_t *flags, const uint2 *wave_ranges, uint32_t *hist, uint32_t *starts, uint32_t local_cap, hipStream_t stream,
-    uint32_t *local_incl, uint32_t *bucket_sums, int T, uint2 *ranges, int local_threads, uint32_t *watch)
+    uint32_t *local_incl, uint32_t *bucket_sums, int T, uint2 *ranges, int local_threads, uint32_t *watch, const Ex4dRowsFused *rows)
 {
     if (n == 0) return hipSuccess;
     constexpr int BINS = 1 << MB;
@@ -1262,22 +1387,23 @@
         hipLaunchKernelGGL((rs_scatter_kernel<RS_ITEMS, BINS, 3, MB>), dim3(nb), dim3(RS_THREADS), 0, stream, ka, (const uint32_t *)nullptr, kb, vb, n, 0, MB, nb, hist,
             0, (const uint32_t *)nullptr, 0, (uint2 *)nullptr, (const uint32_t *)nullptr, ra, rb, starts, (const uint32_t *)dparams);
     }
-    if (local_threads == 256)
-        hipLaunchKernelGGL(depth_local_sort_kernel<256>, dim3(BINS), dim3(256), 0, stream, kb, vb, rb, ka, va, ra, starts, hist + (size_t)BINS * nb, (const uint32_t *)dparams, local_cap,
-            local_incl, bucket_sums, T, ranges, watch);
-    else
-        hipLaunchKernelGGL(depth_local_sort_kernel<512>, dim3(BINS), dim3(512), 0, stream, kb, vb, rb, ka, va, ra, starts, hist + (size_t)BINS * nb, (const uint32_t *)dparams, local_cap,
-            local_incl, bucket_sums, T, ranges, watch);
+    const bool fill_rows = rows != nullptr && local_incl == nullptr;
+    const Ex4dRowsFused rh = fill_rows ? *rows : Ex4dRowsFused{ nullptr, nullptr, 0u, 0u, 0 };
+#define DLS_LOCAL(TH, ROWS) hipLaunchKernelGGL((depth_local_sort_kernel<TH, ROWS>), dim3(BINS), dim3(TH), 0, stream, kb, vb, rb, ka, va, ra, starts, hist + (size_t)BINS * nb, \
+        (const uint32_t *)dparams, local_cap, local_incl, bucket_sums, T, ranges, watch, rh)
+    if (local_threads == 256) { if (fill_rows) DLS_LOCAL(256, true); else DLS_LOCAL(256, false); }
+    else { if (fill_rows) DLS_LOCAL(512, true); else DLS_LOCAL(512, false); }
+#undef DLS_LOCAL
     return hipGetLastError();
 }
 
 hipError_t ex4d_depth_sort_msd(uint32_t *ka, uint32_t *va, uint32_t *ra, uint32_t *kb, uint32_t *vb, uint32_t *rb, uint32_t n, uint32_t inv_key,
     uint32_t *flags, const uint2 *wave_ranges, uint32_t *hist, uint32_t *starts, uint32_t local_cap, hipStream_t stream,
-    uint32_t *local_incl, uint32_t *bucket_sums, int T, uint2 *ranges, int local_threads, uint32_t *watch, int msd_bits)
+    uint32_t *local_incl, uint32_t *bucket_sums, int T, uint2 *ranges, int local_threads, uint32_t *watch, int msd_bits, const Ex4dRowsFused *rows)
 {
     if (msd_bits == EX4D_DLS_MSD_BITS - 1)
-        return depth_sort_msd_launch<EX4D_DLS_MSD_BITS - 1>(ka, va, ra, kb, vb, rb, n, inv_key, flags, wave_ranges, hist, starts, local_cap, stream, local_incl, bucket_sums, T, ranges, local_threads, watch);
-    return depth_sort_msd_launch<EX4D_DLS_MSD_BITS>(ka, va, ra, kb, vb, rb, n, inv_key, flags, wave_ranges, hist, starts, local_cap, stream, local_incl, bucket_sums, T, ranges, local_threads, watch);
+        return depth_sort_msd_launch<EX4D_DLS_MSD_BITS - 1>(ka, va, ra, kb, vb, rb, n, inv_key, flags, wave_ranges, hist, starts, local_cap, stream, local_incl, bucket_sums, T, ranges, local_threads, watch, rows);
+    return depth_sort_msd_launch<EX4D_DLS_MSD_BITS>(ka, va, ra, kb, vb, rb, n, inv_key, flags, wave_ranges, hist, starts, local_cap, stream, local_incl, bucket_sums, T, ranges, local_threads, watch, rows);
 }
 
 template <int BINS>
diff --git a/ex4dgs_amd/csrc/ex4d_internal.h b/ex4dgs_amd/csrc/ex4d_internal.h
--- a/ex4dgs_amd/csrc/ex4d_internal.h
+++ b/ex4dgs_amd/csrc/ex4d_internal.h
@@ -34,6 +34,7 @@
     uint32_t *total;
     uint32_t *block_totals;
     uint32_t *row_hist;
+    uint32_t *row_blocks;
     float *sh_dsums;
 };
 struct BinState {
@@ -95,8 +96,16 @@
 size_t ex4d_tile_sort_rows_hist_words(uint32_t R);
 void ex4d_set_rows_probe(int v);
 hipError_t ex4d_rows_prof(unsigned long long *out8, int reset);
+#define EX4D_ROWS_PATH_NONE 0u
+#define EX4D_ROWS_PATH_LDS 1u
+#define EX4D_ROWS_PATH_MEMORY 2u
+static inline uint32_t ex4d_rows_fused_blocks(uint32_t P, int msd_bits) { return (P + 255u) / 256u + (1u << msd_bits); }
+static inline size_t ex4d_rows_fused_path_offset(uint32_t P) { return 2 + (size_t)2 * ex4d_rows_fused_blocks(P, EX4D_DLS_MSD_BITS); }
+static inline size_t ex4d_rows_fused_table_words(uint32_t P) { return ex4d_rows_fused_path_offset(P) + ((size_t)1 << EX4D_DLS_MSD_BITS); }
+struct Ex4dRowsFused { uint32_t *hist, *table; uint32_t nblocks, path_offset; int NR; };
 hipError_t ex4d_tile_sort_rows(int P, int gx, int gy, const uint32_t *order, const uint32_t *r4, const uint2 *r8, uint32_t *words,
-    uint32_t *point_list, uint32_t *tile_ids_out, uint32_t cap, uint32_t S, uint32_t *histA, uint32_t *histB, uint2 *ranges, uint32_t *frame_total, hipStream_t stream);
+    uint32_t *point_list, uint32_t *tile_ids_out, uint32_t cap, uint32_t S, uint32_t *histA, uint32_t *histB, uint2 *ranges, uint32_t *frame_total, hipStream_t stream,
+    const uint32_t *blocks = nullptr, uint32_t nblocks = 0);
 
 hipError_t ex4d_launch_scan_tiles(int P, const uint2 *rects, const uint32_t *rects4, const uint32_t *order, uint2 *sorted_rects, uint32_t *sorted_offsets,
     uint32_t *block_sums, int T, uint2 *ranges, uint32_t *frame_total, hipStream_t stream);
@@ -112,7 +121,8 @@
     uint32_t *flags, const uint2 *wave_ranges, uint32_t *hist, uint32_t *starts, uint32_t local_cap, hipStream_t stream,
     uint32_t *local_incl, uint32_t *bucket_sums, int T, uint2 *ranges, int local_threads,
     uint32_t *watch = nullptr,
-    int msd_bits = EX4D_DLS_MSD_BITS);
+    int msd_bits = EX4D_DLS_MSD_BITS,
+    const struct Ex4dRowsFused *rows = nullptr);
 int ex4d_depth_sort_msd_bits(uint32_t n, int key_bits);
 hipError_t ex4d_depth_sort_sample(uint32_t *ka, uint32_t *va, uint32_t *ra, uint32_t *kb, uint32_t *vb, uint32_t *rb, uint32_t n, uint32_t inv_key, int key_bits,
     uint32_t *hist, uint32_t *starts, uint32_t *table, uint32_t local_cap, hipStream_t stream, int T, uint2 *ranges, int local_threads, bool census);
diff --git a/ex4dgs_amd/csrc/ex4d_rowsort.hip b/ex4dgs_amd/csrc/ex4d_rowsort.hip
--- a/ex4dgs_amd/csrc/ex4d_rowsort.hip
+++ b/ex4dgs_amd/csrc/ex4d_rowsort.hip
@@ -103,11 +103,13 @@
     (void)inst; (void)frame_total;
 }
 
-__global__ __launch_bounds__(256) void rows_scan_kernel(uint32_t len, uint32_t *__restrict__ hist, uint32_t nrows, uint32_t *__restrict__ frame_total, uint32_t first_total_row)
+__global__ __launch_bounds__(256) void rows_scan_kernel(uint32_t stride, uint32_t *__restrict__ hist, uint32_t nrows, uint32_t *__restrict__ frame_total, uint32_t first_total_row,
+    const uint32_t *__restrict__ blocks)
 {
     __shared__ uint32_t wave_sums[4];
     __shared__ uint32_t carry_s;
-    uint32_t *row = hist + (size_t)blockIdx.x * len;
+    uint32_t *row = hist + (size_t)blockIdx.x * stride;
+    const uint32_t len = blocks ? (blocks[0] < stride ? blocks[0] : stride) : stride;
     const int lane = threadIdx.x & 63, wave = threadIdx.x >> 6;
     const bool vec = ((((uintptr_t)row) & 15) == 0);
     if (threadIdx.x == 0) carry_s = 0;
@@ -143,7 +145,7 @@
         __syncthreads();
     }
     if (threadIdx.x == 0) {
-        hist[(size_t)nrows * len + blockIdx.x] = carry_s;
+        hist[(size_t)nrows * stride + blockIdx.x] = carry_s;
         if (frame_total && blockIdx.x >= first_total_row && carry_s != 0u) atomicAdd(frame_total, carry_s);
     }
 }
@@ -179,7 +181,8 @@
 template <int NRP, int CAP>
 __global__ __launch_bounds__(ROW_THREADS) void rows_seg_scatter_kernel(uint32_t P, int NR, const uint32_t *__restrict__ order,
     const uint32_t *__restrict__ r4, const uint2 *__restrict__ r8, const uint32_t *__restrict__ hist, uint32_t nblocks,
-    uint32_t *__restrict__ words, uint32_t cap, int shift, int probe, Ex4dTsBlock *__restrict__ block_table, uint32_t table_blocks)
+    uint32_t *__restrict__ words, uint32_t cap, int shift, int probe, Ex4dTsBlock *__restrict__ block_table, uint32_t table_blocks,
+    const uint32_t *__restrict__ blocks)
 {
     constexpr int PAD = NRP + 4;
     __shared__ __attribute__((aligned(16))) uint32_t wave_cnt[4][PAD];
@@ -194,10 +197,16 @@
     unsigned long long ts[8];
 #define ROWS_TS(i) do { if (probe) ts[i] = __builtin_amdgcn_s_memtime(); } while (0)
     ROWS_TS(0);
-    const uint32_t k = blockIdx.x * ROWA_GAUSS + tid;
+    uint32_t first = blockIdx.x * ROWA_GAUSS, count = ROWA_GAUSS;
+    if (blocks) {
+        const uint2 rec = reinterpret_cast<const uint2 *>(blocks)[1 + blockIdx.x];
+        first = rec.x; count = rec.y;
+        if (count == 0u && blockIdx.x != 0) return;
+    }
+    const uint32_t k = first + tid;
     RectU rc = { 0u, 0u, 0u, 0u };
     uint32_t id = 0u;
-    if (k < P) { rc = rect_at(r4, r8, k); id = order[k]; }
+    if ((uint32_t)tid < count && k < P) { rc = rect_at(r4, r8, k); id = order[k]; }
     if (rc.w * rc.h == 0u) rc.h = 0u;
     const uint32_t it = tid < NR ? hist[(size_t)2 * NR * nblocks + NR + tid] : 0u;
     const uint32_t ipre = tid < NR ? hist[(size_t)(NR + tid) * nblocks + blockIdx.x] : 0u;
@@ -347,23 +356,24 @@
     return e;
 }
 bool ex4d_tile_sort_rows_applies(int P, int gx, int gy) { return gx <= 255 && gy <= 255 && (uint32_t)P <= (1u << 24); }
-size_t ex4d_tile_sort_rows_geom_words(uint32_t P) { return (size_t)2 * 255 * ((P + 255) / 256 + 1) + 64; }
+size_t ex4d_tile_sort_rows_geom_words(uint32_t P) { return (size_t)2 * 255 * (ex4d_rows_fused_blocks(P, EX4D_DLS_MSD_BITS) + 1) + 64; }
 size_t ex4d_tile_sort_rows_hist_words(uint32_t R) { return ex4d_tile_sort_pass_b_hist_words(R); }
 
 hipError_t ex4d_tile_sort_rows(int P, int gx, int gy, const uint32_t *order, const uint32_t *r4, const uint2 *r8, uint32_t *words,
-    uint32_t *point_list, uint32_t *tile_ids_out, uint32_t cap, uint32_t S, uint32_t *histA, uint32_t *histB, uint2 *ranges, uint32_t *frame_total, hipStream_t stream)
+    uint32_t *point_list, uint32_t *tile_ids_out, uint32_t cap, uint32_t S, uint32_t *histA, uint32_t *histB, uint2 *ranges, uint32_t *frame_total, hipStream_t stream,
+    const uint32_t *blocks, uint32_t nblocks)
 {
     if (P <= 0 || cap == 0) return hipSuccess;
-    const uint32_t nbA = ((uint32_t)P + ROWA_GAUSS - 1) / ROWA_GAUSS;
+    const uint32_t nbA = blocks ? nblocks : ((uint32_t)P + ROWA_GAUSS - 1) / ROWA_GAUSS;
     uint32_t *totA = histA + (size_t)2 * gy * nbA;
     const int bx = bits_for(gx);
-    hipLaunchKernelGGL(rows_seg_hist_kernel, dim3((nbA + 3) / 4), dim3(ROW_THREADS), 0, stream, (uint32_t)P, gy, r4, r8, histA, nbA, frame_total);
-    hipLaunchKernelGGL(rows_scan_kernel, dim3(2 * gy), dim3(256), 0, stream, nbA, histA, (uint32_t)(2 * gy), frame_total, (uint32_t)gy);
+    if (!blocks) hipLaunchKernelGGL(rows_seg_hist_kernel, dim3((nbA + 3) / 4), dim3(ROW_THREADS), 0, stream, (uint32_t)P, gy, r4, r8, histA, nbA, frame_total);
+    hipLaunchKernelGGL(rows_scan_kernel, dim3(2 * gy), dim3(256), 0, stream, nbA, histA, (uint32_t)(2 * gy), frame_total, (uint32_t)gy, blocks);
     const bool big = S == 0 ? (uint64_t)cap > 20ull * (uint32_t)P : 2ull * S > 7ull * (uint32_t)P;
     Ex4dTsBlock *block_table = reinterpret_cast<Ex4dTsBlock *>(histB + ex4d_tile_sort_pass_b_table_offset(cap));
     const uint32_t table_blocks = ex4d_tile_sort_pass_b_blocks(cap, gy);
 #define ROWS_A(NRP, CAP) hipLaunchKernelGGL((rows_seg_scatter_kernel<NRP, CAP>), dim3(nbA), dim3(ROW_THREADS), 0, stream, (uint32_t)P, gy, order, r4, r8, (const uint32_t *)histA, nbA, \
-        words, cap, 32 - bx, g_rows_probe, block_table, table_blocks)
+        words, cap, 32 - bx, g_rows_probe, block_table, table_blocks, blocks)
     if (gy <= 64) { if (big) ROWS_A(64, 2048); else ROWS_A(64, 1024); }
     else if (gy <= 128) { if (big) ROWS_A(128, 2048); else ROWS_A(128, 1024); }
     else { if (big) ROWS_A(256, 2048); else ROWS_A(256, 1024); }
diff --git a/include/ex4d_rasterizer.h b/include/ex4d_rasterizer.h
--- a/include/ex4d_rasterizer.h
+++ b/include/ex4d_rasterizer.h
@@ -153,6 +153,7 @@
 int ex4d_debug_bwd_stats16(unsigned long long *out16, int reset);
 int ex4d_debug_rows_prof(unsigned long long *out8, int reset);
 int ex4d_debug_sample_sort(unsigned long long *out8, int reset);
+int ex4d_debug_rows_fused_layout(int32_t P, size_t *out4);
 
 void ex4d_profile_enable(int on);
 int ex4d_profile_read(int which, float *ms, const char **names, int max_stages);
```

Result: no change. 0.6493 ms/frame, median of 3 (-0.2%).
